# geloescht/mxnet-maintenance

Hardware: AMD Instinct MI355X
Metric: images/sec (whole node) ResNet-50 fp16 batch 256/GPU at 1/2/4/8 MI355X (higher is better)
Workload: dtype fp16; 1 GPU; model=ResNet-50 v1b, global_batch=256, per_gpu_batch=256, image_size=224, parallelism=dp1, layout=NHWC, optimizer=mp-SGD momentum 0.9, lr 0.1 (linear warm-up 40 steps), hip_graph=True, deterministic=True

## Files before the change

### mxnet_maintenance_amd/_state.py

```python
import threading


class _State(threading.local):
    def __init__(self):
        super().__init__()
        self.recording = False
        self.training = False
        self.np_shape = False
        self.np_array = False
        self.tape_leaves = {}


STATE = _State()

DIRECT_GRAD = [0]


def is_recording():
    return STATE.recording


def is_training():
    return STATE.training

GRAPH_RNG = [None]


GRAD_TOUCHED = set()
```

### mxnet_maintenance_amd/autograd.py

```python
from contextlib import contextmanager


import torch

from . import _state
from .base import MXNetError

__all__ = ['record', 'pause', 'train_mode', 'predict_mode', 'is_recording', 'is_training',
           'set_recording', 'set_training', 'mark_variables', 'backward', 'grad', 'Function',
           'get_symbol']


def set_recording(is_recording):
    prev = _state.STATE.recording
    _state.STATE.recording = bool(is_recording)
    return prev


def set_training(train_mode):
    prev = _state.STATE.training
    _state.STATE.training = bool(train_mode)
    return prev


# ... 41 lines not shown
def predict_mode():
    return _RecordingStateScope(None, False)


def mark_variables(variables, gradients, grad_reqs='write'):
    from .ndarray.ndarray import NDArray
    if isinstance(variables, NDArray):
        variables, gradients = [variables], [gradients]
    if isinstance(grad_reqs, str):
        grad_reqs = [grad_reqs] * len(variables)
    for v, g, r in zip(variables, gradients, grad_reqs):
        if r == 'null':
            v._grad_req = None
            continue
        if not v._data.is_floating_point() or getattr(v, '_idt', None) is not None:
            import torch
            idt = getattr(v, '_idt', None) or v._data.dtype
            if not v._data.is_floating_point():
                v._data = v._data.detach().to(torch.float64)
                v._idt = idt
            if not g._data.is_floating_point():
                gidt = g._data.dtype
                g._data = g._data.to(torch.float64)
                g._idt = gidt
        v._set_grad_buffer(g._data, r)
        v._grad = g


_RELEASED_ATTR = '_mxamd_graph_released'


def _collect_leaves(retain):
    leaves = list(_state.STATE.tape_leaves.values())
    if not retain:
        _state.STATE.tape_leaves = {}
    return leaves


def _add_touch_hook(v, t):
    import weakref
    ref = weakref.ref(v)

    def touched(_t, ref=ref):
        a = ref()
        if a is not None:
            _state.GRAD_TOUCHED.add(id(a))
    t.register_post_accumulate_grad_hook(touched)
    t._mxamd_touch_hook = True


def _zero_marked_grads():
    leaves = _collect_leaves(False)
    _prepare_leaves(leaves)
    for v in leaves:
        if v._grad is not None:
            v._fresh_grad = True


def _prepare_leaves(leaves):
    zero = []
    arenas = {}
    for v in leaves:
        t = v._data
        if not t.requires_grad or v._grad is None:
            continue
        if not getattr(t, '_mxamd_touch_hook', False):
            _add_touch_hook(v, t)
        gbuf = v._grad._data
        if t.grad is not gbuf:
            t.grad = gbuf
        if v._grad_req == 'write':
            a = v._arena
            if a is not None and a.all_write:
                arenas.setdefault(id(a), (a, []))[1].append(gbuf)
            else:
                zero.append(gbuf)
    with torch.no_grad():
        for a, bufs in arenas.values():
            if len(bufs) == len(a.params):
                a.g.zero_()
            else:
                zero.extend(bufs)
        if zero:
            torch._foreach_zero_(zero)


def _finish_leaves(leaves):
    touched = _state.GRAD_TOUCHED
    for v in leaves:
        t = v._data
        if v._grad is None:
            continue
        g = t.grad
        if g is not None and g is not v._grad._data:
            v._grad._data = g
            t.grad = g
        if id(v) in touched or not getattr(t, '_mxamd_touch_hook', False):
            v._fresh_grad = True
        else:
            _state.STATE.tape_leaves.setdefault(id(v), v)
    touched.clear()


def _head_grad(g, t):
    if g.shape == t.shape:
        return g
    if g.numel() == t.numel() or (g.numel() > t.numel() and g.dim() == t.dim()
                                  and g.shape[1:] == t.shape[1:]):
        return g.reshape(-1)[:t.numel()].reshape(t.shape)
    try:
        return g.expand(t.shape)
    except RuntimeError:
        pass
    raise MXNetError(f'head gradient of shape {tuple(g.shape)} does not match output shape {tuple(t.shape)}')


def backward(heads, head_grads=None, retain_graph=False, train_mode=True, create_graph=False):
    from .ndarray.ndarray import NDArray
    if isinstance(heads, NDArray):
        heads = [heads]
    if head_grads is not None and isinstance(head_grads, NDArray):
        head_grads = [head_grads]
    tensors, grads = [], []
    for i, h in enumerate(heads):
        t = h._data
        if not t.requires_grad:
            continue
        tensors.append(t)
        hg = None if head_grads is None else head_grads[i]
        grads.append(torch.ones_like(t) if hg is None else _head_grad(hg._data.to(t.dtype), t))
    if not tensors and heads and all(getattr(h, '_recorded', False) for h in heads):
        _zero_marked_grads()
        return
    if not tensors:
        raise MXNetError('Cannot differentiate node because it is not in a computational graph. '
                         'You need to set is_recording to true or use autograd.record() to save '
                         'computational graphs for backward.')
    for h in heads:
        if getattr(getattr(h, '_data', None), _RELEASED_ATTR, False):
            raise MXNetError('Check failed: the graph of this output was already freed by a backward pass '
                             'without retain_graph=True; record it again or pass retain_graph=True')
    if not (retain_graph or create_graph):
        for h in heads:
            if getattr(h, '_data', None) is not None and h._data.grad_fn is not None:
                setattr(h._data, _RELEASED_ATTR, True)
    leaves = _collect_leaves(retain_graph)
    _prepare_leaves(leaves)
    prev_train = set_training(train_mode)
    prev_rec = set_recording(False)
    direct = not create_graph
    if direct:
        _state.DIRECT_GRAD[0] += 1
    try:
        with torch.enable_grad() if create_graph else torch.no_grad():
            torch.autograd.backward(tensors, grads, retain_graph=retain_graph or create_graph,
                                    create_graph=create_graph)
    finally:
        set_training(prev_train)
        set_recording(prev_rec)
        if direct:
            _state.DIRECT_GRAD[0] -= 1
    _finish_leaves(leaves)


def grad(heads, variables, head_grads=None, retain_graph=None, create_graph=False, train_mode=True):
    from .ndarray.ndarray import NDArray
    if isinstance(heads, NDArray):
        heads = [heads]
    if isinstance(variables, NDArray):
        variables = [variables]
    if head_grads is not None and isinstance(head_grads, NDArray):
        head_grads = [head_grads]
    hts = [h._data for h in heads]
    if head_grads is None:
        hgs = [torch.ones_like(h) for h in hts]
    else:
        hgs = [torch.ones_like(h) if g is None else g._data for h, g in zip(hts, head_grads)]
    if retain_graph is None:
        retain_graph = create_graph
    live = [(h, g) for h, g in zip(hts, hgs) if h.requires_grad]
    gs = [None] * len(variables)
    if live:
        prev_train = set_training(train_mode)
        prev_rec = set_recording(create_graph)
        try:
            with torch.enable_grad():
                gs = torch.autograd.grad([h for h, _ in live], [v._data for v in variables],
                                         grad_outputs=[g for _, g in live], retain_graph=retain_graph,
                                         create_graph=create_graph, allow_unused=True)
        finally:
            set_training(prev_train)
            set_recording(prev_rec)

    def dense(g, v):
        if g is None or g._is_zerotensor():
            return torch.zeros_like(v._data)
        return g
    return [NDArray(dense(g, v)) for g, v in zip(gs, variables)]


def get_symbol(x):
    sym = getattr(x, '_symbol', None)
    if isinstance(sym, tuple):
        block, i = sym
        return block._recorded_symbols()[i]
    if sym is not None:
        return sym
    if getattr(x, '_hist', None) is None:
        raise MXNetError('get_symbol: the array was not produced by a recorded operator')
    from .symbol.symbol import _op_func, var
    memo, nvars = {}, [0]

    def build(a):
        key = id(a)
        if key in memo:
            return memo[key]
        h = getattr(a, '_hist', None)
        if h is None:
            s = var('var%d' % nvars[0])
            nvars[0] += 1
        else:
            (opname, attrs, ins), i = h
            kw = {k: v for k, v in attrs.items() if v is not None}
            node = _op_func(opname)(*[build(b) for b in ins if b is not None], **kw)
            s = node[i] if len(node.list_outputs()) > 1 else node
        memo[key] = s
        return s
    return build(x)


class Function:

    def __init__(self):
        self._saved = ()
        self._used = False

    def save_for_backward(self, *args):
        self._saved = args

    @property
    def saved_tensors(self):
        return self._saved

    def __call__(self, *inputs):
        from .ndarray.ndarray import NDArray
        if self._used:
            raise MXNetError('Each Function instance can only be called once.')
        self._used = True
        fself = self
        nin = len(inputs)

        class _Bridge(torch.autograd.Function):
            @staticmethod
            def forward(ctx, *tins):
                with pause():
                    outs = fself.forward(*[NDArray(t.detach()) for t in tins])
                single = isinstance(outs, NDArray)
                ctx.single = single
                outs = [outs] if single else list(outs)
                return tuple(o._data for o in outs)

            @staticmethod
            def backward(ctx, *gouts):
                with pause():
                    gins = fself.backward(*[NDArray(g) for g in gouts])
                if isinstance(gins, NDArray):
                    gins = [gins]
                return tuple(None if g is None else g._data for g in gins)

        from .ndarray.register import _note_leaves
        _note_leaves(inputs)
        tins = [x._data for x in inputs]
        if _state.STATE.recording:
            with torch.enable_grad():
                res = _Bridge.apply(*tins)
        else:
            with torch.no_grad():
                res = _Bridge.apply(*tins)
        outs = [NDArray(r) for r in res]
        return outs[0] if len(outs) == 1 else outs

    def forward(self, *inputs):
        raise NotImplementedError

    def backward(self, *output_grads):
        raise NotImplementedError
```

### mxnet_maintenance_amd/executor.py

```python
import os

import numpy as np
import torch

from . import _state
from . import profiler as _profiler
from .ops import amp_dispatch as _amp
from .base import MXNetError, AsyncOpError
from .ops import registry


def _call_monitor(cb, name, arr):
    from .base import _HANDLES, NDArrayHandle
    key = id(arr)
    _HANDLES[key] = arr
    try:
        cb(name, NDArrayHandle(key))
    finally:
        _HANDLES.pop(key, None)


class GraphProgram:

    def __init__(self, sym):
# ... 372 lines not shown
            return []
        if not out_shapes or any(s is None for s in out_shapes):
            return []
        return [nd.zeros(tuple(s), ctx=self._ctx, dtype=t if t is not None else 'float32')
                for s, t in zip(out_shapes, out_types or [None] * len(out_shapes))]

    @property
    def arg_dict(self):
        return dict(zip(self._symbol.list_arguments(), self.arg_arrays))

    @property
    def grad_dict(self):
        return dict(zip(self._symbol.list_arguments(), self.grad_arrays))

    @property
    def aux_dict(self):
        return dict(zip(self._symbol.list_auxiliary_states(), self.aux_arrays))

    @property
    def output_dict(self):
        return dict(zip(self._symbol.list_outputs(), self.outputs))

    def forward(self, is_train=False, **kwargs):
        from .ndarray.ndarray import NDArray
        for k, v in kwargs.items():
            ad = self.arg_dict
            if k not in ad:
                raise MXNetError('forward: unknown argument %s' % k)
            src = v._data if isinstance(v, NDArray) else torch.as_tensor(np.asarray(v))
            with torch.no_grad():
                ad[k]._data.copy_(src.reshape(ad[k].shape))
        need_grad = is_train and any(r != 'null' for r in self._grad_req.values())
        self._last_is_train = bool(is_train)
        return self._run(is_train, need_grad)

    def _run(self, is_train, need_grad):
        from . import engine as _eng
        _eng.join_workers()
        from .ndarray.ndarray import NDArray
        arg_names = self._symbol.list_arguments()
        feed = {}
        leaves = []
        int_dtypes = None
        for n, a in zip(arg_names, self.arg_arrays):
            t = a._data.detach()
            if need_grad and self._grad_req[n] != 'null':
                if not (t.is_floating_point() or t.is_complex()):
                    int_dtypes = int_dtypes or {}
                    int_dtypes[n] = t.dtype
                    t = t.to(torch.float64)
                t = t.requires_grad_(True)
                leaves.append((n, t))
            feed[n] = t
        for n, a in zip(self._symbol.list_auxiliary_states(), self.aux_arrays):
            feed[n] = a._data
        prev_train = _state.STATE.training
        _state.STATE.training = bool(is_train)
        try:
            mon = None
            if self._monitor_cb is not None:
                cb = self._monitor_cb

                def mon(name, t):
                    _call_monitor(cb, name, NDArray(t.detach()))
            record = [] if (mon is not None and need_grad) else None
            with torch.set_grad_enabled(need_grad):
                outs = self._prog.run(feed, mon, self._monitor_all, record, int_dtypes=int_dtypes)
            self._mon_record = record
            self._mon_grads = {}
            if record:
                for _name, args in record:
                    for t in args:
                        if isinstance(t, torch.Tensor) and t.requires_grad and id(t) not in self._mon_grads:
                            self._mon_grads[id(t)] = None

                            def hook(g, key=id(t)):
                                self._mon_grads[key] = g.detach()
                            t.register_hook(hook)
        finally:
            _state.STATE.training = prev_train
        self._leaves = leaves
        self._out_tensors = outs
        idts = getattr(self._prog, 'out_idts', None) or [None] * len(outs)
        vals = [o.detach().to(d) if d is not None else o.detach() for o, d in zip(outs, idts)]
        if len(self.outputs) == len(vals) and all(
                b.shape == tuple(o.shape) and b._data.dtype == o.dtype for b, o in zip(self.outputs, vals)):
            with torch.no_grad():
                for b, o in zip(self.outputs, vals):
                    b._data.copy_(o)
        else:
            self.outputs = [NDArray(o) for o in vals]
        st = self._output_stypes()
        if st is not None:
            from .ndarray import sparse
            self.outputs = [sparse.cast_storage(o, t) if t != 'default' else o for o, t in zip(self.outputs, st)]
        self._failure = getattr(self._prog, 'failure', None)
        self._failure_box = None
        if self._failure is not None:
            from . import engine
            box = self._failure_box = engine.record_failure(self._failure)
            for o in self.outputs:
                o._exc = box
        return self.outputs

    def _output_stypes(self):
        cached = getattr(self, '_stype_cache', False)
        if cached is not False:
            return cached
        from .ndarray.register import _kept_stype, _check_storage
        args = dict(zip(self._symbol.list_arguments(), self.arg_arrays))
        if all(getattr(a, 'stype', 'default') == 'default' for a in args.values()):
            self._stype_cache = None
            return None

        class _S:
            __slots__ = ('stype',)

            def __init__(self, st):
                self.stype = st
        memo = {}
        for n in self._symbol._topo():
            if n.op is None:
                memo[(id(n), 0)] = getattr(args.get(n.name), 'stype', 'default')
                continue
            ins = [memo.get((id(i), j), 'default') for i, j in n.inputs]
            attrs = registry_parse(n)
            _check_storage(n.op, ins, attrs)
            st = _binary_stype(n.op, ins)
            if st is None:
                st = _kept_stype(n.op, [_S(t) for t in ins], attrs) if ins else None

            memo[(id(n), 0)] = st or 'default'
        self._stype_cache = [memo.get((id(n), i), 'default') for n, i in self._symbol._outputs]
        return self._stype_cache

    def backward(self, out_grads=None, is_train=True):
        from .ndarray.ndarray import NDArray
        if not self._leaves:
            if not any(r != 'null' for r in self._grad_req.values()) or not self.grad_arrays:
                return
            self._run(getattr(self, '_last_is_train', False), True)
        if out_grads is None:
            out_grads = [None] * len(self._out_tensors)
        elif isinstance(out_grads, NDArray):
            out_grads = [out_grads]
        heads, hgs = [], []
        for o, g in zip(self._out_tensors, out_grads):
            if not o.requires_grad:
                continue
            heads.append(o)
            hgs.append(torch.ones_like(o) if g is None else g._data.to(o.dtype).reshape(o.shape))
        names = [n for n, _ in self._leaves]
        ts = [t for _, t in self._leaves]
        grads = (torch.autograd.grad(heads, ts, hgs, allow_unused=True, retain_graph=False)
                 if heads and ts else [None] * len(ts))
        gd = self.grad_dict
        with torch.no_grad():
            for n, g in zip(names, grads):
                buf = gd[n]
                if g is None:
                    if self._grad_req[n] == 'write':
                        buf._data.zero_()
                    continue
                if self._grad_req[n] == 'add':
                    buf._data.add_(g.to(buf._data.dtype))
                else:
                    buf._data.copy_(g)
            got = set(names)
            for n, buf in gd.items():
                if n not in got and buf is not None and self._grad_req.get(n) == 'write':
                    buf._data.zero_()
        record = getattr(self, '_mon_record', None)
        if record and self._monitor_cb is not None:
            for name, args in reversed(record):
                for i, t in enumerate(args):
                    if not isinstance(t, torch.Tensor):
                        continue
                    g = self._mon_grads.get(id(t))
                    _call_monitor(self._monitor_cb, '%s_backward_in%d' % (name, i),
                                  NDArray(g if g is not None else torch.zeros_like(t)))
            self._mon_record = None
        box = getattr(self, '_failure_box', None)
        if box is not None and box[0] is not None:
            for n in names:
                gd[n]._exc = box
        self._leaves = None

    def set_monitor_callback(self, callback, monitor_all=False):
        self._monitor_cb = callback
        self._monitor_all = monitor_all

    def copy_params_from(self, arg_params, aux_params=None, allow_extra_params=False):
        for name, array in arg_params.items():
            if name in self.arg_dict:
                self.arg_dict[name][:] = array.as_in_context(self.arg_dict[name].context)
            elif not allow_extra_params:
                raise ValueError('Find name "%s" that is not in the arguments' % name)
        if aux_params is not None:
            for name, array in aux_params.items():
                if name in self.aux_dict:
                    self.aux_dict[name][:] = array.as_in_context(self.aux_dict[name].context)
                elif not allow_extra_params:
                    raise ValueError('Find name %s that is not in the auxiliary states' % name)

    def reshape(self, partial_shaping=False, allow_up_sizing=False, **kwargs):
        from .ndarray.ndarray import NDArray
        from . import ndarray as nd
        sym = self._symbol
        known = {n: a.shape for n, a in zip(sym.list_arguments(), self.arg_arrays)}
        for k in kwargs:
            if k not in known:
                raise MXNetError('reshape: %s is not an argument of the symbol' % k)
        if not partial_shaping:
            known = {k: v for k, v in known.items() if k not in kwargs}
            known.update(kwargs)
        else:
            known.update(kwargs)
        arg_shapes, out_shapes, aux_shapes = sym.infer_shape(**known)

        def fit(old, shape, what):
            if old is None:
                return None
            shape = tuple(shape)
            if shape == tuple(old.shape):
                return old
            n = 1
            for d in shape:
                n *= d
            if n <= old.size:
                return NDArray(old._data.reshape(-1)[:n].view(shape))
            if not allow_up_sizing:
                raise MXNetError('reshape: %s grows from %s to %s; pass allow_up_sizing=True'
                                 % (what, old.shape, shape))
            return nd.zeros(shape, ctx=old.context, dtype=old.dtype)

        names = sym.list_arguments()
        args = [fit(a, s, n) for a, s, n in zip(self.arg_arrays, arg_shapes, names)]
        grads = [fit(g, s, n + '_grad') for g, s, n in zip(self.grad_arrays, arg_shapes, names)]
        auxs = [fit(a, s, n) for a, s, n in zip(self.aux_arrays, aux_shapes, sym.list_auxiliary_states())]
        exe = Executor(sym, self._ctx, args, grads if any(g is not None for g in grads) else None,
                       dict(self._grad_req), auxs)
        if len(self.outputs) == len(out_shapes):
            try:
                exe.outputs = [fit(o, s, 'output') for o, s in zip(self.outputs, out_shapes)]
            except MXNetError:
                pass
        exe._monitor_cb, exe._monitor_all = self._monitor_cb, self._monitor_all
        return exe

    def get_optimized_symbol(self):
        return self._opt_symbol

    def debug_str(self):
        from .symbol import passes as _passes
        names = self._symbol.list_arguments()
        wanting = [n for n in names if self._grad_req.get(n, 'null') != 'null']
        grad = bool(_passes.grad_reachable(self._opt_symbol, set(wanting)))
        shapes = {n: a.shape for n, a in zip(names, self.arg_arrays)}
        dtypes = {n: a.dtype for n, a in zip(names, self.arg_arrays)}
        nbytes = _passes.memory_plan(self._opt_symbol, shapes, dtypes, grad)
        return '%s\nTotal %d MB allocated\n' % (self._opt_symbol.debug_str(), nbytes // (1 << 20))
```

### mxnet_maintenance_amd/gluon/graph_step.py

```python
import gc
import os

import torch

from .. import _state
from ..ndarray.ndarray import NDArray

__all__ = ['GraphStep']


def _tensor_of(x):
    return x._data if isinstance(x, NDArray) else x


class GraphStep:

    def __init__(self, fn, trainer=None, warmup=3, fallback=False):
        if warmup < 1:
            raise ValueError('GraphStep needs at least one eager warm-up call')
        self._fn = fn
        self._trainer = trainer
        self._warmup = int(warmup)
        self._calls = 0
        self._graph = None
        self._static_in = None
        self._static_out = None
        self._stream = None
        self._rng = None
        self._fallback = fallback
        self._eager_only = False

    @property
    def captured(self):
        return self._graph is not None

    def _side_stream(self, device):
        if self._stream is None:
            self._stream = torch.cuda.Stream(device=device)
        return self._stream

    @staticmethod
    def _device(inputs):
        dev = next((_tensor_of(x).device for x in inputs if torch.is_tensor(_tensor_of(x))), None)
        if dev is None and torch.cuda.is_available():
            dev = torch.device('cuda', torch.cuda.current_device())
        return dev

    def _run_eager(self, inputs):
        dev = self._device(inputs)
        if dev is None or dev.type != 'cuda':
            return self._fn(*inputs)
        s = self._side_stream(dev)
        s.wait_stream(torch.cuda.current_stream(dev))
        with torch.cuda.stream(s):
            out = self._fn(*inputs)
        torch.cuda.current_stream(dev).wait_stream(s)
        return out

    def _capture(self, inputs):
        tin = [_tensor_of(x) for x in inputs]
        dev = self._device(inputs)
        if dev is None or dev.type != 'cuda':
            raise RuntimeError('GraphStep captures HIP work: inputs must live on a GPU context')
        self._static_in = [NDArray(t.clone()) if isinstance(x, NDArray) else (t.clone() if torch.is_tensor(t) else x)
                           for x, t in zip(inputs, tin)]
        self._rng = torch.zeros(1, dtype=torch.int64, device=dev)
        if self._trainer is not None:
            self._trainer._enter_graph_mode()
        s = self._side_stream(dev)
        if os.environ.get('MXAMD_GRAPH_GC', '1') == '1':
            gc.collect()
        torch.cuda.synchronize(dev)
        graph = torch.cuda.CUDAGraph()
        _state.GRAPH_RNG[0] = self._rng
        try:
            with torch.cuda.graph(graph, stream=s):
                self._static_out = self._fn(*self._static_in)
        except Exception:
            if self._trainer is not None:
                self._trainer._exit_graph_mode()
            raise
        finally:
            _state.GRAPH_RNG[0] = None
        self._graph = graph

    def _load_inputs(self, inputs):
        if len(inputs) != len(self._static_in):
            raise ValueError('GraphStep: expected %d inputs, got %d' % (len(self._static_in), len(inputs)))
        for dst, src in zip(self._static_in, inputs):
            d, t = _tensor_of(dst), _tensor_of(src)
            if not torch.is_tensor(d):
                if d != t:
                    raise ValueError('GraphStep: non-tensor argument %r differs from the captured %r' % (t, d))
                continue
            if d.shape != t.shape or d.dtype != t.dtype:
                raise ValueError('GraphStep: input %s/%s differs from the captured %s/%s'
                                 % (tuple(t.shape), t.dtype, tuple(d.shape), d.dtype))
            if d.data_ptr() != t.data_ptr():
                d.copy_(t, non_blocking=True)

    @property
    def static_inputs(self):
        return self._static_in

    def __call__(self, *inputs):
        self._calls += 1
        if self._eager_only:
            return self._run_eager(inputs)
        if self._graph is None:
            if self._calls <= self._warmup:
                return self._run_eager(inputs)
            err = None
            try:
                self._capture(inputs)
            except Exception as e:
                err = e
            if not self._all_ranks_ok(err is None):
                if self._graph is not None:
                    self._drop_graph()
                if not self._fallback:
                    raise err if err is not None else RuntimeError('GraphStep: capture failed on another rank')
                import warnings
                warnings.warn('GraphStep: capture failed (%s); running the step eagerly on every rank'
                              % (err if err is not None else 'on another rank'))
                self._eager_only = True
                if torch.cuda.is_available():
                    torch.cuda.synchronize()
                return self._run_eager(inputs)
        else:
            self._load_inputs(inputs)
        if self._trainer is not None:
            self._trainer._stage_hyper()
        self._rng.add_(1)
        self._graph.replay()
        return self._static_out

    @staticmethod
    def _all_ranks_ok(ok):
        from ..parallel import dist
        if dist.world_size() <= 1:
            return ok
        t = torch.tensor([1 if ok else 0], dtype=torch.int32)
        dist.all_reduce(t, op='min')
        return bool(t.item())

    def _drop_graph(self):
        if self._trainer is not None:
            self._trainer._exit_graph_mode()
        self._graph = None
        self._static_out = None

    def reset(self):
        if self._trainer is not None and self._graph is not None:
            self._trainer._exit_graph_mode()
        self._graph = None
        self._static_out = None
        self._static_in = None
        self._calls = self._warmup
```

### mxnet_maintenance_amd/ops/kernel_fns.py

```python
import os

import torch

from . import kernels as _K
from .. import _state
from ..utils import env as _env

__all__ = ['BatchNormNHWC', 'BatchNormDualTailNHWC', 'SoftmaxCE', 'GlobalAvgPoolNHWC', 'flat_sgd']

_DT = {torch.float32: 0, torch.float16: 1, torch.bfloat16: 2}


def _stream():
    return torch.cuda.current_stream().cuda_stream


def _p(t):
    return 0 if t is None else t.data_ptr()


def _f32(t):
    if t.dtype == torch.float32 and t.is_contiguous():
        return t
    m = getattr(t, '_mxamd_master', None)
# ... 115 lines not shown
            ctx.pool = (N, H, W, C, Ho, Wo, kh, kw, sh, sw, ph, pw, 1)
            lib.pool_nhwc_forward_bnrelu(_DT[x.dtype], x.data_ptr(), y.data_ptr(), arg.data_ptr(), *ctx.pool,
                                         _stream(), scale.data_ptr(), shift.data_ptr())
            mask = arg
        relu_mode = 0 if not relu else (1 if not _RELU_FROM_X[0] else (3 if addend is not None else 2))
        if pool is not None:
            relu_mode = 2
        ctx.save_for_backward(x, y if relu_mode == 1 else mask, g, mean, invstd,
                              scale if relu_mode == 2 else None, shift if relu_mode == 2 else None)
        ctx.cfg = (relu_mode, bool(training), addend is not None, gamma.dtype, beta.dtype)
        ctx.tee_key = getattr(addend, '_mxamd_tee_key', None) if (addend is not None and relu_mode == 3) else None
        ctx.bn_token = None
        if training and relu_mode in (0, 2, 3) and _BN_BWD_FUSE[0] and pool is None:
            ctx.bn_token = _BnToken()
            y._mxamd_bn_src = (x, mean, scale if relu_mode == 2 else None, shift if relu_mode == 2 else None,
                               mask if relu_mode == 3 else None, relu_mode, ctx.bn_token)
        ctx.refs = (gamma, beta)
        ctx.add_src = None
        if relu_mode == 3 and training and _BN_BWD_FUSE[0] and _BN_TAIL_DS[0]:
            src = getattr(addend, '_mxamd_bn_src', None)
            if (src is not None and src[5] == 0 and tuple(src[0].shape) == tuple(x.shape)
                    and src[0].dtype == x.dtype and src[0].is_contiguous()):
                ctx.add_src = src
        third = invstd if (invstd_out and training) else var
        ctx.mark_non_differentiable(mean, third)
        ctx.set_materialize_grads(False)
        return y, mean, third

    @staticmethod
    def backward(ctx, gy, _gm, _gv):
        lib = _K.lib()
        x, y, g, mean, invstd, fscale, fshift = ctx.saved_tensors
        relu_mode, training, has_add, gdt, bdt = ctx.cfg
        gamma_ref, beta_ref = ctx.refs
        if gy is None:
            return (None,) * 12
        gy = gy.contiguous()
        C = x.shape[-1]
        R = x.numel() // C
        dev = x.device
        fused_pool = False
        if ctx.pool is not None:
            fused_pool = (x.dtype in (torch.float16, torch.bfloat16) and 256 % (C // 8) == 0
                          and hasattr(lib, 'bn_pool_backward') and _BN_POOL_BWD[0])
            if not fused_pool:
                gyd = torch.empty_like(x)
                lib.pool_nhwc_backward(_DT[x.dtype], 1, gy.data_ptr(), y.data_ptr(), gyd.data_ptr(), *ctx.pool,
                                       _stream())
                gy, y = gyd, None
        lazy_mask = None
        tok = ctx.bn_token
        if tok is not None and tok.lazy is not None:
            dy_l, mask_l, ver_l = tok.lazy
            tok.lazy = None
            if gy is dy_l and gy._version == ver_l and relu_mode == 0 and not has_add and ctx.pool is None:
                lazy_mask = mask_l
            else:
                gy = (gy - dy_l + _materialize_dz(dy_l, mask_l)).contiguous()
        dx = torch.empty_like(x)
        dz = torch.empty_like(x) if has_add else None
        ext = getattr(gy, '_mxamd_bn_bwd', None)
        ext_nblk = 0
        if (ext is not None and ctx.bn_token is not None and ext[2] is ctx.bn_token
                and ext[3] == gy._version):
            part, ext_nblk = ext[0], ext[1]
        else:
            nblk = lib.bn_partials_rows(R, C)
            part = torch.empty(2 * nblk * C, dtype=torch.float32, device=dev)
        out = torch.empty(5, C, dtype=torch.float32, device=dev)
        need_g, need_b = ctx.needs_input_grad[1], ctx.needs_input_grad[2]
        tg = _leaf_grad(gamma_ref, C) if need_g else None
        tb = _leaf_grad(beta_ref, C) if need_b else None
        direct = tb is not None and (tg is not None or not need_g) and (tg is not None or tb is not None)
        if direct:
            dg_buf = tg if tg is not None else torch.zeros(C, dtype=torch.float32, device=dev)
            dg_ptr, db_ptr, accum = dg_buf.data_ptr(), tb.data_ptr(), 1
        else:
            dg_ptr, db_ptr, accum = out[0].data_ptr(), out[1].data_ptr(), 0
        if fused_pool:
            N_, H_, W_, C_, Ho_, Wo_, kh, kw, sh, sw, ph, pw, _ = ctx.pool
            ppart = torch.empty(2 * lib.bn_pool_bwd_blocks() * C, dtype=torch.float32, device=dev)
            lib.bn_pool_backward(_DT[x.dtype], x.data_ptr(), gy.data_ptr(), y.data_ptr(), dx.data_ptr(), g.data_ptr(),
                                 mean.data_ptr(), invstd.data_ptr(), fscale.data_ptr(), fshift.data_ptr(),
                                 ppart.data_ptr(), dg_ptr, db_ptr, out[2].data_ptr(), N_, H_, W_, C_, Ho_, Wo_, kh, kw,
                                 sh, sw, ph, pw, 0, int(training), accum, _stream())
            if direct:
                return dx, None, None, None, None, None, None, None, None, None, None, None
            return (dx, out[0].to(gdt) if need_g else None, out[1].to(bdt) if need_b else None,
                    None, None, None, None, None, None, None, None, None)
        ymask = y if relu_mode == 3 else None
        y = y if relu_mode == 1 else None
        ds = ctx.add_src if dz is not None else None
        lazy = (dz is not None and ds is None and ymask is not None and ctx.tee_key is not None
                and lazy_shortcut_ok(ctx.tee_key))
        lazy_ds = (dz is not None and ds is not None and ymask is not None and _LAZY_DZ[0]
                   and isinstance(ds[6], _BnToken))
        if lazy or lazy_ds:
            dz = None
        kmode = relu_mode
        if lazy_mask is not None:
            kmode, ymask = 3, lazy_mask
        dkw = {}
        if ds is not None:
            ds_nblk = lib.bn_tail_ds_rows(R, C)
            ds_part = torch.empty(2 * ds_nblk * C, dtype=torch.float32, device=dev)
            dkw = dict(ds_z=ds[0].data_ptr(), ds_mean=ds[1].data_ptr(), ds_part=ds_part.data_ptr())
        lib.bn_nhwc_backward(_DT[x.dtype], x.data_ptr(), gy.data_ptr(), _p(y), _p(ymask), dx.data_ptr(), _p(dz),
                             g.data_ptr(),
                             mean.data_ptr(), invstd.data_ptr(), _p(fscale), _p(fshift), part.data_ptr(), dg_ptr,
                             db_ptr, out[2].data_ptr(), R, C, kmode, 0, int(training), accum, _stream(),
                             ext_nblk, **dkw)
        if ds is not None:
            if lazy_ds:
                gy._mxamd_bn_bwd = (ds_part, ds_nblk, ds[6], gy._version)
                ds[6].lazy = (gy, ymask, gy._version)
                dz = gy
            else:
                dz._mxamd_bn_bwd = (ds_part, ds_nblk, ds[6], dz._version)
        if lazy:
            gy._mxamd_lazy_mask = (ymask, gy._version)
            dz = gy
        if direct:
            dgamma = None
            dbeta = None
        else:
            dgamma = out[0].to(gdt) if need_g else None
            dbeta = out[1].to(bdt) if need_b else None
        return dx, dgamma, dbeta, dz, None, None, None, None, None, None, None, None


_DUAL_TAIL_USED = [0]


def _bn_param_grad_dst(gamma_ref, beta_ref, need_g, need_b, out, C, dev):
    tg = _leaf_grad(gamma_ref, C) if need_g else None
    tb = _leaf_grad(beta_ref, C) if need_b else None
    if tb is not None and (tg is not None or not need_g):
        dg_buf = tg if tg is not None else torch.zeros(C, dtype=torch.float32, device=dev)
        return dg_buf.data_ptr(), tb.data_ptr(), 1, True, dg_buf
    return out[0].data_ptr(), out[1].data_ptr(), 0, False, None


class BatchNormDualTailNHWC(torch.autograd.Function):

    @staticmethod
    def forward(ctx, x, z, gamma, beta, zgamma, zbeta, eps, training, moving_mean, moving_var, zmoving_mean,
                zmoving_var, momentum=None):
        lib = _K.lib()
        assert z.shape == x.shape and z.dtype == x.dtype and z.is_contiguous()
        dev = x.device
        dt = _DT[x.dtype]
        zg, zmean, zinvstd, _zvar, zscale, zshift, zargs, zhost = _bn_fwd_stats(
            lib, z, zgamma, zbeta, zmoving_mean, zmoving_var, eps, training, momentum)
        if training:
            lib.bn_nhwc_forward(dt, z.data_ptr(), 0, 0, 0, *zargs(False))
        g, mean, invstd, var, scale, shift, args, host = _bn_fwd_stats(
            lib, x, gamma, beta, moving_mean, moving_var, eps, training, momentum)
        y = torch.empty_like(x)
        mask = torch.empty(x.numel() // 8, dtype=torch.uint8, device=dev)
        lib.bn_nhwc_forward(dt, x.data_ptr(), z.data_ptr(), y.data_ptr(), mask.data_ptr(), *args(True),
                            zscale.data_ptr(), zshift.data_ptr())
        for h in (zhost, host):
            if h is not None:
                h()
        _DUAL_TAIL_USED[0] += 1
        ctx.save_for_backward(x, z, mask, g, mean, invstd, zg, zmean, zinvstd)
        ctx.cfg = (bool(training), gamma.dtype, beta.dtype, zgamma.dtype, zbeta.dtype)
        ctx.refs = (gamma, beta, zgamma, zbeta)
        ctx.bn_token = None
        if training and _BN_BWD_FUSE[0]:
            ctx.bn_token = _BnToken()
            y._mxamd_bn_src = (x, mean, None, None, mask, 3, ctx.bn_token)
        ctx.mark_non_differentiable(mean, var)
        ctx.set_materialize_grads(False)
        return y, mean, var

    @staticmethod
    def backward(ctx, gy, _gm, _gv):
        lib = _K.lib()
        x, z, mask, g, mean, invstd, zg, zmean, zinvstd = ctx.saved_tensors
        training, gdt, bdt, zgdt, zbdt = ctx.cfg
        gamma_ref, beta_ref, zgamma_ref, zbeta_ref = ctx.refs
        if gy is None:
            return (None,) * 13
        gy = gy.contiguous()
        C = x.shape[-1]
        R = x.numel() // C
        dev = x.device
        dt = _DT[x.dtype]
        need = ctx.needs_input_grad
        dx = torch.empty_like(x)
        dzs = torch.empty_like(z)
        ext = getattr(gy, '_mxamd_bn_bwd', None)
        ext_nblk = 0
        if ext is not None and ctx.bn_token is not None and ext[2] is ctx.bn_token and ext[3] == gy._version:
            part, ext_nblk = ext[0], ext[1]
        else:
            part = torch.empty(2 * lib.bn_partials_rows(R, C) * C, dtype=torch.float32, device=dev)
        out = torch.empty(5, C, dtype=torch.float32, device=dev)
        zout = torch.empty(5, C, dtype=torch.float32, device=dev)
        dg_ptr, db_ptr, accum, direct, _k1 = _bn_param_grad_dst(gamma_ref, beta_ref, need[2], need[3], out, C, dev)
        zdg_ptr, zdb_ptr, zaccum, zdirect, _k2 = _bn_param_grad_dst(zgamma_ref, zbeta_ref, need[4], need[5], zout, C,
                                                                    dev)
        ride = training and _BN_TAIL_DS[0]
        dkw, zpart, znblk = {}, None, 0
        if ride:
            znblk = lib.bn_tail_ds_rows(R, C)
            zpart = torch.empty(2 * znblk * C, dtype=torch.float32, device=dev)
            dkw = dict(ds_z=z.data_ptr(), ds_mean=zmean.data_ptr(), ds_part=zpart.data_ptr())
        else:
            zpart = torch.empty(2 * lib.bn_partials_rows(R, C) * C, dtype=torch.float32, device=dev)
        lib.bn_nhwc_backward(dt, x.data_ptr(), gy.data_ptr(), 0, mask.data_ptr(), dx.data_ptr(), 0, g.data_ptr(),
                             mean.data_ptr(), invstd.data_ptr(), 0, 0, part.data_ptr(), dg_ptr, db_ptr,
                             out[2].data_ptr(), R, C, 3, 0, int(training), accum, _stream(), ext_nblk, **dkw)
        lib.bn_nhwc_backward(dt, z.data_ptr(), gy.data_ptr(), 0, mask.data_ptr(), dzs.data_ptr(), 0, zg.data_ptr(),
                             zmean.data_ptr(), zinvstd.data_ptr(), 0, 0, zpart.data_ptr(), zdg_ptr, zdb_ptr,
                             zout[2].data_ptr(), R, C, 3, 0, int(training), zaccum, _stream(), znblk)
        dgamma = None if direct or not need[2] else out[0].to(gdt)
        dbeta = None if direct or not need[3] else out[1].to(bdt)
        zdgamma = None if zdirect or not need[4] else zout[0].to(zgdt)
        zdbeta = None if zdirect or not need[5] else zout[1].to(zbdt)
        return dx, dzs, dgamma, dbeta, zdgamma, zdbeta, None, None, None, None, None, None, None


def bnrelu_pool_ok(x, kernel, stride, pad):
    return (bn_ok(x) and tuple(kernel) == (3, 3) and pool_ok(x, kernel, stride, pad)
            and x.numel() + 256 * 32 * 256 * 8 < 2 ** 31 and hasattr(_K.lib(), 'pool_nhwc_forward_bnrelu'))


class SoftmaxCE(torch.autograd.Function):

    @staticmethod
    def forward(ctx, logits, label):
        lib = _K.lib()
        N, K = logits.shape
        lab = label.reshape(-1)
        is_int = not lab.is_floating_point()
        lab = lab.to(torch.int64).contiguous() if is_int else lab.float().contiguous()
        loss = torch.empty(N, dtype=torch.float32, device=logits.device)
        lse = torch.empty(N, dtype=torch.float32, device=logits.device)
        lib.softmax_ce_forward(_DT[logits.dtype], int(is_int), logits.data_ptr(), lab.data_ptr(), loss.data_ptr(),
                               lse.data_ptr(), N, K, _stream())
        ctx.save_for_backward(logits, lab, lse)
        ctx.is_int = is_int
        return loss

    @staticmethod
    def backward(ctx, gout):
        lib = _K.lib()
        logits, lab, lse = ctx.saved_tensors
        N, K = logits.shape
        g = gout.float().contiguous()
        dl = torch.empty_like(logits)
        lib.softmax_ce_backward(_DT[logits.dtype], int(ctx.is_int), logits.data_ptr(), lab.data_ptr(),
                                lse.data_ptr(), g.data_ptr(), dl.data_ptr(), N, K, _stream())
        return dl, None


class GlobalAvgPoolNHWC(torch.autograd.Function):
    @staticmethod
    def forward(ctx, x):
        lib = _K.lib()
        x = x.contiguous()
        N, C = x.shape[0], x.shape[-1]
        HW = x.numel() // (N * C)
        y = torch.empty((N,) + (1,) * (x.dim() - 2) + (C,), dtype=x.dtype, device=x.device)
        lib.gap_nhwc_forward(_DT[x.dtype], x.data_ptr(), y.data_ptr(), N, HW, C, _stream())
        ctx.shape = x.shape
        return y

    @staticmethod
    def backward(ctx, gy):
        lib = _K.lib()
        shape = ctx.shape
        N, C = shape[0], shape[-1]
        HW = int(torch.tensor(shape[1:-1]).prod())
        gy = gy.contiguous()
        dx = torch.empty(shape, dtype=gy.dtype, device=gy.device)
        lib.gap_nhwc_backward(_DT[gy.dtype], gy.data_ptr(), dx.data_ptr(), N, HW, C, _stream())
        return dx


def gap_ok(x):
    return x.dtype in _DT and x.is_contiguous() and x.shape[-1] % 8 == 0


class ReluHip(torch.autograd.Function):

    @staticmethod
    def forward(ctx, x):
        x = x.contiguous()
        y = torch.empty_like(x)
        _K.lib().relu_forward(_DT[x.dtype], x.data_ptr(), y.data_ptr(), x.numel(), _stream())
        ctx.save_for_backward(y)
        return y

    @staticmethod
    def backward(ctx, gy):
        y, = ctx.saved_tensors
        gy = gy.contiguous()
        dx = torch.empty_like(y)
        _K.lib().relu_backward(_DT[y.dtype], y.data_ptr(), gy.data_ptr(), dx.data_ptr(), y.numel(), _stream())
        return dx


def relu_ok(x):
    return x.dtype in _DT and x.is_cuda and x.numel() > 0 and x.data_ptr() % 16 == 0 and x.is_contiguous()


_PW_OPS = {'add': 0, 'sub': 1, 'mul': 2, 'div': 3, 'maximum': 4, 'minimum': 5}


def _bcast_strides(t, shape):
    lead = len(shape) - t.dim()
# ... 226 lines not shown
        if bn_bwd is not None:
            z, bmean, bscale, bshift, bmask, bmode, token = bn_bwd
            assert z.shape == y.shape and z.dtype == y.dtype and z.is_contiguous()
            bnp = lib.conv_nhwc_fwd_big_bwd_nparts(N, H, W, R, S, stride[0], stride[1], pad[0], pad[1], v)
            bpart = torch.empty(2 * K * bnp, dtype=torch.float32, device=x.device)
            bkw = dict(bn_z=z.data_ptr(), bn_mean=bmean.data_ptr(), bn_scale=_p(bscale), bn_shift=_p(bshift),
                       bn_mask=_p(bmask), bn_mode=int(bmode), bn_part=bpart.data_ptr(), bn_nparts=bnp)
        lib.conv_nhwc_fwd_big(_DT[x.dtype], x.data_ptr(), w.data_ptr(), _p(b), y.data_ptr(),
                              _zero_page(x.device).data_ptr(), N, H, W, C, K, R, S, stride[0], stride[1],
                              pad[0], pad[1], v, _p(part), nparts, _p(addend), _stream(), up=int(up), dh=dil[0],
                              dw=dil[1], **bkw)
        if bkw:
            y._mxamd_bn_bwd = (bpart, bnp, bn_bwd[6], y._version)
        if part is not None:
            y._mxamd_bn_part = (part, nparts)
        return y
    if variant in (5, 6):
        lib = _K.lib()
        bco = 128 if variant == 5 else 64
        bkw = _glds_bnb(bn_bwd, y, lib.conv_glds_bwd_nparts(N * Ho * Wo, bco))
        part = bkw.pop('_part', None)
        lib.conv_nhwc_fwd_glds(_DT[x.dtype], x.data_ptr(), w.data_ptr(), _p(b), y.data_ptr(),
                               _zero_page(x.device).data_ptr(), N, H, W, C, K, R, S, stride[0], stride[1],
                               pad[0], pad[1], bco, _stream(), **bkw)
        if part is not None:
            y._mxamd_bn_bwd = (part, bkw['bn_nparts'], bn_bwd[6], y._version)
        return y
    _K.lib().conv_nhwc_fwd(_DT[x.dtype], x.data_ptr(), w.data_ptr(), _p(b), y.data_ptr(), N, H, W, C, K, R, S,
                           stride[0], stride[1], pad[0], pad[1], int(variant), _stream())
    return y


def halo_ok(x, w, stride, pad):
    K, R, S, C = w.shape
    return (_CONV_HIP and x.is_cuda and x.dtype in (torch.float16, torch.bfloat16) and x.dim() == 4
            and x.is_contiguous() and w.is_contiguous() and x.data_ptr() % 16 == 0 and w.data_ptr() % 16 == 0
            and hasattr(_K.lib(), 'conv3x3_halo')
            and bool(_K.lib().conv3x3_halo_ok(C, K, R, S, stride[0], stride[1], pad[0], pad[1], x.shape[2])))


def conv_halo(x, w, bn_stats=False, bn_bwd=None):
    N, H, W, C = x.shape
    K = w.shape[0]
    lib = _K.lib()
    y = torch.empty((N, H, W, K), dtype=x.dtype, device=x.device)
    nparts = lib.conv3x3_halo_nparts(N, H)
    part = torch.empty(2 * K * nparts, dtype=torch.float32, device=x.device) if (bn_stats or bn_bwd) else None
    kw = {}
    if bn_bwd is not None:
        z, bmean, bscale, bshift, _bmask, bmode, _token = bn_bwd
        assert int(bmode) in (0, 2) and z.shape == y.shape and z.dtype == y.dtype and z.is_contiguous()
        kw = dict(bn_z=z.data_ptr(), bn_mean=bmean.data_ptr(), bn_scale=_p(bscale), bn_shift=_p(bshift),
                  bn_mode=int(bmode), bn_part=part.data_ptr())
    lib.conv3x3_halo(_DT[x.dtype], x.data_ptr(), w.data_ptr(), y.data_ptr(), _zero_page(x.device).data_ptr(), N, H,
                     W, C, K, _p(part) if bn_bwd is None else 0, nparts if bn_bwd is None else 0, s=_stream(), **kw)
    if bn_bwd is not None:
        y._mxamd_bn_bwd = (part, nparts, bn_bwd[6], y._version)
    elif part is not None:
        y._mxamd_bn_part = (part, nparts)
    return y


def glds_bnb_ok(bn_src):
    return bn_src is not None and int(bn_src[5]) in (0, 2) and hasattr(_K.lib(), 'conv_glds_bwd_nparts')


def _glds_bnb(bn_bwd, y, nparts):
    if bn_bwd is None:
        return {}
    z, bmean, bscale, bshift, _bmask, bmode, _token = bn_bwd
    assert int(bmode) in (0, 2) and z.shape == y.shape and z.dtype == y.dtype and z.is_contiguous()
    part = torch.empty(2 * y.shape[-1] * nparts, dtype=torch.float32, device=y.device)
    return dict(bn_z=z.data_ptr(), bn_mean=bmean.data_ptr(), bn_scale=_p(bscale), bn_shift=_p(bshift),
                bn_part=part.data_ptr(), bn_nparts=nparts, _part=part)


_ZERO = {}


def _zero_page(dev):
    z = _ZERO.get(dev)
    if z is None:
        z = _ZERO[dev] = torch.zeros(128, dtype=torch.float16, device=dev)
    return z


def _fwd_variants(C, K, bias=False, ktot=None):
    v = []
    if C % 64 == 0 and not bias:
        v.extend(b for b, (bco, _bpix) in sorted(_RING_VARIANTS.items()) if K % bco == 0)
    if C % 64 == 0:
        v.extend(b for b, (bco, _bpix) in sorted(_BIG_VARIANTS.items())
                 if K % bco == 0 and (b not in _BIG_SKINNY or (_SKINNY_ON and ktot == 64)))
    if C % 64 == 0 and K % 128 == 0:
        v.append(5)
    if C % 64 == 0:
        v.append(6)
    if K % 128 == 0 and C % 64 == 0:
        v.append(1)
    if K % 128 == 0:
        v.append(2)
    if C % 64 == 0:
        v.append(3)
    v.append(4)
    return v


def conv_wgrad_ok(x, w):
    return (_CONV_HIP and x.dim() == 4 and w.dim() == 4 and x.dtype in (torch.float16, torch.bfloat16)
            and x.is_contiguous() and x.shape[3] % 64 == 0 and w.shape[0] % 64 == 0 and w.shape[3] == x.shape[3]
            and x.numel() < 2 ** 31 and x.data_ptr() % 16 == 0)


def conv_wgrad(x, dy, wshape, stride, pad, out=None, accum=False, dma=True, ring=0, dil=(1, 1)):
    N, H, W, C = x.shape
    K, R, S, _ = wshape
    dy = dy.contiguous()
    assert dy.dtype == x.dtype and dy.shape[0] == N and dy.shape[3] == K
    dh, dw = dil
    Ho = (H + 2 * pad[0] - dh * (R - 1) - 1) // stride[0] + 1
    Wo = (W + 2 * pad[1] - dw * (S - 1) - 1) // stride[1] + 1
    assert tuple(dy.shape[1:3]) == (Ho, Wo), 'conv_wgrad: dy shape does not match the conv geometry'
    assert dy.numel() < 2 ** 31 and dy.data_ptr() % 16 == 0
    lib = _K.lib()
    if ring:
        ws = lib.conv_nhwc_wgrad_ring_workspace(N, H, W, C, K, R, S, stride[0], stride[1], pad[0], pad[1], ring,
                                                dh=dh, dw=dw)
    else:
        ws = lib.conv_nhwc_wgrad_workspace(N, H, W, C, K, R, S, stride[0], stride[1], pad[0], pad[1], dh=dh, dw=dw)
    slab = torch.empty(ws, dtype=torch.float32, device=x.device)
    if out is None:
        out = torch.empty((K, R, S, C), dtype=x.dtype, device=x.device)
        accum = False
    assert out.is_contiguous() and out.numel() == K * R * S * C and out.dtype in _DT
    if ring:
        lib.conv_nhwc_wgrad_ring(_DT[x.dtype], x.data_ptr(), dy.data_ptr(), slab.data_ptr(), _DT[out.dtype],
                                 out.data_ptr(), int(bool(accum)), N, H, W, C, K, R, S, stride[0], stride[1], pad[0],
                                 pad[1], _zero_page(x.device).data_ptr(), int(ring), _stream(), dh=dh, dw=dw)
        return out
    lib.conv_nhwc_wgrad(_DT[x.dtype], x.data_ptr(), dy.data_ptr(), slab.data_ptr(), _DT[out.dtype], out.data_ptr(),
                        int(bool(accum)), N, H, W, C, K, R, S, stride[0], stride[1], pad[0], pad[1],
                        _zero_page(x.device).data_ptr() if dma else 0, _stream(), dh=dh, dw=dw)
    return out


def _taps_t(w, out, src, base, rstride):
    K, R, S, C = w.shape
    for i in range(0, len(src), 32):
        _K.lib().weight_taps_t(w.element_size(), w.data_ptr(), out.data_ptr(), K, R * S, C, src[i:i + 32],
                               base[i:i + 32], rstride[i:i + 32], _stream())
    return out


def _dgrad_weight(w):
    K, R, S, C = w.shape
    if not (w.is_cuda and w.is_contiguous() and w.element_size() in (2, 4) and _K.available()):
        return w.flip(1, 2).permute(3, 1, 2, 0).contiguous()
    T = R * S
    out = torch.empty((C, R, S, K), dtype=w.dtype, device=w.device)
    return _taps_t(w, out, [T - 1 - t for t in range(T)], [t * K for t in range(T)], [T * K] * T)


def transpose2d(w):
    R, C = w.shape
    if w.is_cuda and w.is_contiguous() and w.element_size() in (2, 4) and R % 8 == 0 and C % 8 == 0:
        return _dgrad_weight(w.view(R, 1, 1, C)).view(C, R)
    return w.t().contiguous()


def _phase_taps(R, P, s, ph):
    return sorted(((ph + P - r) // s, r) for r in range(R) if (ph + P - r) % s == 0)


def conv_dgrad_strided_ok(dy, w, stride, pad, xshape, bco=128):
    K, R, S, C = w.shape
    s = tuple(stride)
    return (_CONV_HIP and s != (1, 1) and s[0] == s[1] and s[0] <= 2 and dy.dtype in (torch.float16, torch.bfloat16)
            and dy.dim() == 4 and K % 64 == 0 and C % bco == 0 and xshape[1] % s[0] == 0 and xshape[2] % s[1] == 0
            and dy.is_cuda and all(0 <= p < k for p, k in zip(pad, (R, S))))


_PHASE_PLANS = {}


def _phase_plan(wshape, stride, pad, device):
    key = (tuple(wshape), tuple(stride), tuple(pad), device)
    plan = _PHASE_PLANS.get(key)
    if plan is not None:
        return plan
    K, R, S, C = wshape
    st = stride[0]
    phases, empty, idx, off = [], [], [], 0
    for ph in range(st):
        th = _phase_taps(R, pad[0], st, ph)
        for pw in range(st):
            tw = _phase_taps(S, pad[1], st, pw)
            if not th or not tw:
                empty.append((ph, pw))
                continue
            dh = [d for d, _ in th]
            dw = [d for d, _ in tw]
            if dh != list(range(dh[0], dh[0] + len(dh))) or dw != list(range(dw[0], dw[0] + len(dw))):
                raise ValueError('conv_dgrad_strided: non-contiguous phase taps')
            nt = len(th) * len(tw)
            for i, (_, r) in enumerate(th):
                for j, (_, c) in enumerate(tw):
                    idx.append((r * S + c, off + (i * len(tw) + j) * K, nt * K))
            phases.append((ph, pw, len(th), len(tw), -dh[0], -dw[0], off))
            off += C * nt * K
    plan = (phases, empty, (idx, off))
    _PHASE_PLANS[key] = plan
    return plan


def conv_dgrad_strided(dy, w, stride, pad, xshape, bco=128, bn_bwd=None):
    K, R, S, C = w.shape
    N, H, W, _ = xshape
    st = stride[0]
    Ho, Wo = H // st, W // st
    dy = dy.contiguous()
    phases, empty, gidx = _phase_plan(w.shape, stride, pad, w.device)
    if len(phases) > 4:
        raise ValueError('conv_dgrad_strided: at most 4 phases per launch')
    dx = torch.empty((N, H, W, C), dtype=dy.dtype, device=dy.device)
    if len(empty) > 3:
        raise ValueError('conv_dgrad_strided: at most 3 phases without taps')
    slots, total = gidx
    wsub = _taps_t(w.contiguous(), torch.empty(total, dtype=w.dtype, device=w.device), [t[0] for t in slots],
                   [t[1] for t in slots], [t[2] for t in slots])
    cols = list(zip(*phases))
    lib = _K.lib()
    bkw = _glds_bnb(bn_bwd, dx, len(phases) * lib.conv_glds_bwd_nparts(N * Ho * Wo, bco)) if bn_bwd else {}
    part = bkw.pop('_part', None)
    lib.conv_nhwc_dgrad_phases_glds(_DT[dy.dtype], dy.data_ptr(), wsub.data_ptr(), dx.data_ptr(),
                                    _zero_page(dy.device).data_ptr(), N, dy.shape[1], dy.shape[2], K, C, Ho, Wo,
                                    st, list(cols[0]), list(cols[1]), list(cols[2]), list(cols[3]),
                                    list(cols[4]), list(cols[5]), list(cols[6]), [e[0] for e in empty],
                                    [e[1] for e in empty], bco, _stream(), **bkw)
    if part is not None:
        dx._mxamd_bn_bwd = (part, bkw['bn_nparts'], bn_bwd[6], dx._version)
    return dx


def _conv_bwd_torch(dy, x, w, stride, pad, mask):
    xc = x.permute(0, 3, 1, 2)
    wc = w.permute(0, 3, 1, 2)
    dyc = dy.permute(0, 3, 1, 2)
    dx, dw, _ = torch.ops.aten.convolution_backward(dyc, xc, wc, None, list(stride), list(pad), [1, 1], False,
                                                    [0, 0], 1, [mask[0], mask[1], False])
    if dx is not None:
        dx = dx.permute(0, 2, 3, 1)
    if dw is not None:
        dw = dw.permute(0, 2, 3, 1)
    return dx, dw



_AUTOTUNE = _env.get('MXNET_CUDNN_AUTOTUNE_DEFAULT') > 0
_ALGO = {}
_TIMES = {}


_REJECTED = {}


def _rel_err(a, b):
    a = a.float()
    b = b.float()
    return float((a - b).abs().max() / (b.abs().max() + 1e-6))


_VENDOR = ('mm', 'miopen')
_VENDOR_PREFIX = ('splitk', 'blaslt', 'sk')
_VENDOR_MARGIN = float(os.environ.get('MXAMD_VENDOR_MARGIN', '0.03'))


def _is_vendor(name):
    return name in _VENDOR or name.startswith(_VENDOR_PREFIX)
_TUNE_ROUNDS = int(os.environ.get('MXAMD_TUNE_ROUNDS', '2'))


def _time_candidates(cands, reps=3, key=None, tol=2e-2):
    ref = None
    ref_name = next((n for n, _ in cands if n in ('mm', 'miopen')), None)
    if ref_name is not None:
        ref = dict(cands)[ref_name]()
        if isinstance(ref, torch.Tensor):
            ref = ref.detach().clone()
        else:
            ref = None
    ok = []
    for name, fn in cands:
        if ref is not None and name != ref_name:
            r = fn()
            if isinstance(r, torch.Tensor) and r.shape == ref.shape:
                err = _rel_err(r, ref)
                if not err <= tol:
                    _REJECTED.setdefault(key, {})[name] = err
                    continue
        ok.append((name, fn))
    times, outs = {}, {}
    for _ in range(_TUNE_ROUNDS):
        for name, fn in ok:
            fn()
            t, r = _measure(fn, reps)
            if name not in times or t < times[name]:
                times[name] = t
                outs[name] = r
    names = [n for n, _ in cands]
    agreed = _agree_times([times.get(n, float('inf')) for n in names])
    best, best_t = None, None
    for name, t in zip(names, agreed):
        if t == float('inf'):
            continue
        if key is not None:
            _TIMES.setdefault(key, {})[name] = t / reps
        if _is_vendor(name):
            t *= 1.0 + _VENDOR_MARGIN
        if best_t is None or t < best_t:
            best, best_t = name, t
    if best is not None and best not in outs:
        best = None
    return best, (outs[best] if best is not None else None)


def _measure(fn, reps):
    if torch.cuda.is_available():
        s, e = torch.cuda.Event(enable_timing=True), torch.cuda.Event(enable_timing=True)
        s.record()
        for _ in range(reps):
            r = fn()
        e.record()
        e.synchronize()
        return s.elapsed_time(e), r
    import time
    t0 = time.perf_counter()
    for _ in range(reps):
        r = fn()
    return (time.perf_counter() - t0) * 1e3, r


def _agree_times(vals):
    from ..parallel import dist
    if dist.world_size() <= 1 or not vals:
        return vals
    t = torch.tensor(vals, dtype=torch.float64)
    dist.all_reduce(t, op='max')
    return [float(v) for v in t.tolist()]


_DETERMINISTIC = [_env.get('MXNET_ENFORCE_DETERMINISM') != 0]
_NONDET = ('mm', 'miopen', 'sk', 'splitk', 'bmm', 'blaslt')


def _apply_torch_determinism(flag):
    torch.backends.cudnn.deterministic = bool(flag)
    if flag:
        torch.backends.cudnn.benchmark = False
    try:
        torch.use_deterministic_algorithms(bool(flag), warn_only=True)
    except Exception:
        pass


def set_deterministic(flag):
    _DETERMINISTIC[0] = bool(flag)
    _apply_torch_determinism(flag)


def deterministic():
    return _DETERMINISTIC[0]


if _DETERMINISTIC[0]:
    _apply_torch_determinism(True)


def _det_filter(cands):
    if not _DETERMINISTIC[0] or cands is None:
        return cands
    keep = [(n, f) for n, f in cands if not n.startswith(_NONDET)]
    return keep or cands


def _akey(key):
    return key + ('det',) if _DETERMINISTIC[0] else key


_FILE_ALGO = {}
_FILE_STATE = {'loaded': False}


def _tuning_file():
    return os.environ.get('MXAMD_AUTOTUNE_FILE', '')


def _load_tuning_file():
    if _FILE_STATE['loaded']:
        return
    _FILE_STATE['loaded'] = True
    path = _tuning_file()
    if path and os.path.exists(path):
        import json
        try:
            with open(path) as f:
                _FILE_ALGO.update(json.load(f))
        except (OSError, ValueError):
            pass


def _save_tuning_file(key, name):
    path = _tuning_file()
    if not path or name is None:
        return
    from ..parallel import dist
    if dist.rank() != 0:
        return
    import json
    _FILE_ALGO[repr(key)] = name
    tmp = path + '.tmp'
    try:
        with open(tmp, 'w') as f:
            json.dump(_FILE_ALGO, f, indent=0, sort_keys=True)
        os.replace(tmp, path)
    except OSError:
        pass


def _select(key, cands, default, timing=None):
    key = _akey(key)
    cands = _det_filter(cands)
    timing = _det_filter(timing)
    _load_tuning_file()
    name = _ALGO.get(key)
    if name is None:
# ... 681 lines not shown
```

### src/kernels/bindings.cc

```cpp
#include <hip/hip_runtime.h>
#include <pybind11/pybind11.h>
#include <pybind11/stl.h>

#include <cstdint>
#include <stdexcept>
#include <vector>

namespace py = pybind11;

namespace mxamd {
void bn_nhwc_forward(int dtype, const void* x, const void* addend, void* y, uint8_t* mask, const float* gamma,
                     const float* beta,
                     const float* center, float* part, float* mean, float* invstd, float* var, float* scale,
                     float* shift, int64_t R, int C, float eps, int training, int relu, int fix_gamma,
                     float momentum, float* mm_upd, float* mv_upd, int ext_nblk, hipStream_t s, const float* ascale,
                     const float* ashift);
void bn_nhwc_backward(int dtype, const void* x, const void* dy, const void* y, const uint8_t* mask, void* dx,
                      void* dz,
                      const float* gamma, const float* mean, const float* invstd, const float* fscale,
                      const float* fshift, float* part, float* dgamma, float* dbeta, float* coef, int64_t R, int C,
                      int relu_mode, int fix_gamma, int training, int accum, hipStream_t s, int ext_nblk, const void* ds_z, const float* ds_mean, float* ds_part);
int bn_partials_rows(int64_t R, int C);
int bn_tail_ds_rows(int64_t R, int C);
void gemm_nt(int dtype, const void* a, const void* b, const void* bias, const void* addend, void* c, int out_f32,
             int M, int N, int K, int lda, int ldb, int ldc, int act, int cfg, int splits, float* ws, hipStream_t s,
             int bias_lowp);
int gemm_nt_tile_n(int cfg);
int gemm_nt_tile_m(int cfg);
void int8_gemm(const int8_t* A, const int8_t* B, int32_t* C, int M, int N, int K, hipStream_t s);
void csr_dot_dense(int dtype, const int64_t* indptr, const int64_t* indices, const void* vals, const void* rhs,
                   void* out, int64_t M, int64_t K, int N, hipStream_t s);
void csrT_dot_dense(int dtype, const int64_t* indptr, const int64_t* indices, const void* vals, const void* rhs,
                    const int64_t* slot, float* out32, int64_t M, int64_t K, int N, hipStream_t s);
void embedding_forward(int dtype, int itype, const void* idx, const void* w, void* y, int64_t n, int V, int C,
                       hipStream_t s);
void embedding_backward(int dtype, int itype, const void* idx, const void* dy, float* acc, uint8_t* touched,
                        int out_dtype, void* grad, int accum, int64_t n, int V, int C, hipStream_t s);
int bn_nhwc_stats(int dtype, const void* x, const float* center, float* part, int64_t R, int C, hipStream_t s,
                  int total_blocks);
int64_t colsum_partials(int64_t R, int C);
void colsum_rows(int dtype, const void* x, const float* zeros, float* part, int64_t R, int C, int out_dtype,
                 void* out, int accum, hipStream_t s);
void softmax_ce_forward(int dtype, int label_is_int, const void* logits, const void* label, float* loss, float* lse,
                        int N, int K, hipStream_t s);
void softmax_ce_backward(int dtype, int label_is_int, const void* logits, const void* label, const float* lse,
                         const float* gout, void* dlogits, int N, int K, hipStream_t s);
void gap_nhwc_forward(int dtype, const void* x, void* y, int N, int HW, int C, hipStream_t s);
void relu_forward(int dtype, const void* x, void* y, int64_t n, hipStream_t s);
void relu_backward(int dtype, const void* y, const void* dy, void* dx, int64_t n, hipStream_t s);
void pointwise_binary(int dtype, int op, const void* a, const void* b, void* out, int64_t n, int mode, int64_t row,
                      int ndim, const int64_t* shape, const int64_t* astride, const int64_t* bstride, hipStream_t s);
void gap_nhwc_backward(int dtype, const void* dy, void* dx, int N, int HW, int C, hipStream_t s);
void flat_sgd(int dtype, void* w, const void* g, float* mom, float* w32, int64_t n, float lr, float wd,
              float momentum, float rescale, float clip, const float* hp, hipStream_t s);
void conv_nhwc_fwd(int dtype, const void* x, const void* w, const float* bias, void* y, int N, int H, int W, int C,
                   int K, int R, int S, int sh, int sw, int ph, int pw, int variant, hipStream_t s);
int conv_nhwc_fwd_big_nparts(int N, int H, int W, int R, int S, int sh, int sw, int ph, int pw, int variant);
void conv_nhwc_fwd_big(int dtype, const void* x, const void* w, const float* bias, void* y, const void* zero, int N,
                       int H, int W, int C, int K, int R, int S, int sh, int sw, int ph, int pw, int variant,
                       float* part, int nparts, const void* addend, hipStream_t s, const void* bn_z,
                       const float* bn_mean, const float* bn_scale, const float* bn_shift, const uint8_t* bn_mask,
                       int bn_mode, float* bn_part, int bn_nparts, int up, int dh, int dw);
int conv_nhwc_fwd_big_bwd_nparts(int N, int H, int W, int R, int S, int sh, int sw, int ph, int pw, int variant);
void conv_nhwc_fwd_glds(int dtype, const void* x, const void* w, const float* bias, void* y, const void* zero, int N,
                        int H, int W, int C, int K, int R, int S, int sh, int sw, int ph, int pw, int bco,
                        hipStream_t s, const void* bn_z, const float* bn_mean, const float* bn_scale,
                        const float* bn_shift, float* bn_part, int bn_nparts);
int conv_glds_bwd_nparts(int M, int bco);
void conv_nhwc_dgrad_phases_glds(int dtype, const void* dy, const void* w, void* dx, const void* zero, int N, int Hi,
                                 int Wi, int Cin, int Cout, int Ho, int Wo, int stride, int nph, const int* ph,
                                 const int* pw, const int* R, const int* S, const int* pad_h, const int* pad_w,
                                 const int64_t* w_off, int nzero, const int* zph, const int* zpw, int bco,
                                 hipStream_t s, const void* bn_z, const float* bn_mean, const float* bn_scale,
                                 const float* bn_shift, float* bn_part, int bn_nparts);
int conv_nhwc_fwd_ring_nparts(int N, int H, int W, int R, int S, int sh, int sw, int ph, int pw, int variant);
void conv_nhwc_fwd_ring(int dtype, const void* x, const void* w, void* y, const void* zero, int N, int H, int W, int C,
                        int K, int R, int S, int sh, int sw, int ph, int pw, int variant, float* part, int nparts,
                        hipStream_t s);
bool conv3x3_halo_ok(int C, int K, int R, int S, int sh, int sw, int ph, int pw, int W);
int conv3x3_halo_nparts(int N, int H);
void conv3x3_halo(int dtype, const void* x, const void* w, void* y, const void* zero, int N, int H, int W, int C, int K,
                  float* part, int nparts, const void* bn_z, const float* bn_mean, const float* bn_scale,
                  const float* bn_shift, int bn_mode, float* bn_part, hipStream_t s);
int conv_nhwc_wgrad_ring_ok(int C, int K, int R, int S, int variant);
int64_t conv_nhwc_wgrad_ring_workspace(int N, int H, int W, int C, int K, int R, int S, int sh, int sw, int ph, int pw,
                                       int variant, int dh, int dw);
void conv_nhwc_wgrad_ring(int dtype, const void* x, const void* dy, float* slab, int out_dtype, void* out, int accum,
                          int N, int H, int W, int C, int K, int R, int S, int sh, int sw, int ph, int pw,
                          const void* zero, int variant, hipStream_t s, int dh, int dw);
int64_t conv_nhwc_wgrad_workspace(int N, int H, int W, int C, int K, int R, int S, int sh, int sw, int ph, int pw,
                                  int dh, int dw);
void conv_nhwc_wgrad(int dtype, const void* x, const void* dy, float* slab, int out_dtype, void* out, int accum, int N,
                     int H, int W, int C, int K, int R, int S, int sh, int sw, int ph, int pw, const void* zero,
                     hipStream_t s, int dh, int dw);
int conv_stem_grid(int N, int H, int W, int R, int S, int ph, int pw);
void conv_stem_fwd(int dtype, const void* x, const void* w, void* y, int N, int H, int W, int C, int K, int R, int S,
                   int sh, int sw, int ph, int pw, float* part, int nparts, hipStream_t s);
int64_t conv_stem_wgrad_workspace(int N, int H, int W, int R, int S, int ph, int pw);
void conv_stem_wgrad(int dtype, const void* x, const void* dy, float* slab, int out_dtype, void* out, int accum, int N,
                     int H, int W, int C, int K, int R, int S, int sh, int sw, int ph, int pw, hipStream_t s);
int layernorm_bwd_partials(int M);
void layernorm_forward(int dtype, const void* x, const void* gamma, const void* beta, int pt, void* y, float* mean,
                       float* rstd, int M, int D, float eps, hipStream_t s);
void layernorm_backward(int dtype, const void* x, const void* dy, const void* gamma, int pt, const float* mean,
                        const float* rstd, void* dx, float* part, void* dgamma, void* dbeta, int gdtype, int accum,
                        int M, int D, hipStream_t s);
void add_dropout_ln_forward(int dtype, const void* x, const void* h, const void* gamma, const void* beta, int pt,
                            void* y, void* s_out, uint8_t* mask, float* mean, float* rstd, int M, int D, float eps,
                            float p, uint64_t seed, const uint64_t* seed_base, hipStream_t s);
void add_dropout_ln_backward(int dtype, const void* s_in, const void* dy, const void* gamma, int pt, const float* mean,
                             const float* rstd, const uint8_t* mask, float p, void* ds, void* dh, float* part,
                             float* hpart, void* dgamma, void* dbeta, int gdtype, int accum, int M, int D,
                             hipStream_t s);
void column_sum_partials(int gdtype, const float* part, int nb, int ncol, void* out, int accum, hipStream_t s);
void gelu_forward(int dtype, const void* x, void* y, int64_t n, hipStream_t s);
void gelu_backward(int dtype, const void* x, const void* dy, void* dx, int64_t n, hipStream_t s);
void gelu_backward_colpart(int dtype, const void* x, const void* dy, void* dx, float* part, int M, int N,
                           hipStream_t s);
int gelu_colpart_blocks(int M, int N);
void softmax_forward(int dtype, int log, const void* x, void* y, int M, int L, float scale, hipStream_t s);
void softmax_backward(int dtype, int log, const void* y, const void* dy, void* dx, int M, int L, float scale,
                      hipStream_t s);
void dropout_forward(int dtype, const void* x, void* y, uint8_t* mask, int64_t n, float p, uint64_t seed,
                     const uint64_t* seed_base, hipStream_t s);
void dropout_backward(int dtype, const void* dy, const uint8_t* mask, void* dx, int64_t n, float p, hipStream_t s);
int attention_max_seq();
void attention_forward(int dtype, const void* qkv, const float* kmask, void* out, float* lse, int S, int B, int H,
                       int D, float scale, float p, uint64_t seed, const uint64_t* seed_base, hipStream_t s);
void attention_backward(int dtype, const void* qkv, const float* kmask, const void* out, const void* dout,
                        const float* lse, float* delta, void* dqkv, int S, int B, int H, int D, float scale, float p,
                        uint64_t seed, const uint64_t* seed_base, hipStream_t s);
void flat_adam(int dtype, int mode, void* w, const void* g, float* mean, float* var, float* w32, int64_t n, float lr,
               float beta1, float beta2, float eps, float wd, float eta, float rescale, float clip, const float* hp,
               hipStream_t s);
void lamb_update(int dtype, void* w, const void* g, float* mean, float* var, float* w32, float* upd,
                 const void* chunks, int nchunks, float* nrm, int nseg, float lr, float beta1, float beta2, float eps,
                 float bc1, float bc2, float wd, float rescale, float clip, float lb, float ub, const float* hp,
                 hipStream_t s);
void seg_sumsq(int dtype, const void* x, const void* chunks, int nchunks, float* out, int nseg, hipStream_t s);
void all_finite(int dtype, const void* x, int64_t n, float scale, int* flag, int init, hipStream_t s);
void pool_nhwc_forward(int dtype, int is_max, const void* x, void* y, uint8_t* arg, int N, int H, int W, int C,
                       int Ho, int Wo, int kh, int kw, int sh, int sw, int ph, int pw, int cip, hipStream_t s,
                       const float* scale, const float* shift);
int bn_pool_bwd_blocks();
void bn_pool_backward(int dtype, const void* x, const void* dy, const uint8_t* arg, void* dx, const float* gamma,
                      const float* mean, const float* invstd, const float* fscale, const float* fshift, float* part,
                      float* dgamma, float* dbeta, float* coef, int N, int H, int W, int C, int Ho, int Wo, int kh,
                      int kw, int sh, int sw, int ph, int pw, int fix_gamma, int training, int accum,
                      hipStream_t s);
void pool_nhwc_backward(int dtype, int is_max, const void* dy, const uint8_t* arg, void* dx, int N, int H, int W,
                        int C, int Ho, int Wo, int kh, int kw, int sh, int sw, int ph, int pw, int cip,
                        hipStream_t s);
void deform_im2col(int dtype, const void* x, const void* off, const void* msk, void* cols, int N, int C, int H, int W,
                   int Ho, int Wo, int kh, int kw, int sh, int sw, int ph, int pw, int dh, int dw, int dg,
                   int rows, hipStream_t s);
void deform_col2im(int dtype, const void* off, const void* msk, const void* gcols, float* gx, int N, int C, int H,
                   int W, int Ho, int Wo, int kh, int kw, int sh, int sw, int ph, int pw, int dh, int dw, int dg,
                   int rows, hipStream_t s);
void deform_col2im_coord(int dtype, const void* x, const void* off, const void* msk, const void* gcols, void* goff,
                         void* gmsk, int N, int C, int H, int W, int Ho, int Wo, int kh, int kw, int sh, int sw,
                         int ph, int pw, int dh, int dw, int dg, int rows, hipStream_t s);
void deform_im2col_nhwc(int dtype, const void* x, const void* off, const void* msk, void* cols, const int* g,
                        int ld_off, int ld_msk, hipStream_t s);
void deform_bwd_nhwc(int dtype, const void* x, const void* off, const void* msk, const void* gcols, float* gx,
                     void* goff, void* gmsk, const int* g, int ld_off, int ld_msk, hipStream_t s);
void conv_dw_fwd(int dtype, const void* x, const void* wt, const float* bias, void* y, const int* gm, hipStream_t s);
void conv_dw_dgrad(int dtype, const void* dy, const void* wt, void* dx, const int* gm, hipStream_t s);
void conv_dw_wgrad(int dtype, const void* x, const void* dy, float* slab, int nslice, int out_dtype, void* out,
                   int accum, const int* gm, hipStream_t s);
int ssd_loss_blocks(int rows);
void ssd_loss_fwd(int dtype, const void* cls, const void* loc, const float* cls_t, const float* loc_t,
                  const float* loc_m, int rows, int C1, float lambd, float* part, float* out, hipStream_t s);
void ssd_loss_bwd(int dtype, const void* cls, const void* loc, const float* cls_t, const float* loc_t,
                  const float* loc_m, const float* stats, const float* gout, int rows, int C1, float lambd, void* dcls,
                  void* dloc, hipStream_t s);
void multibox_target(int dtype, const float* anchors, const float* labels, const void* cls_pred, float* loc_target,
                     float* loc_mask, float* cls_target, float* match_iou, int* match_gt, uint32_t* key, int B, int A,
                     int L, int W, int C, float thr, float ignore_label, float neg_ratio, float neg_thresh,
                     int min_neg, float v0, float v1, float v2, float v3, hipStream_t s);
void slab_reduce(int out_dtype, float* slab, int splits, int64_t n, void* out, int accum, hipStream_t s);
void twobit_quantize(int dtype, const void* g, float* res, void* packed, int64_t n, float thr, hipStream_t s);
void twobit_dequantize_sum(const void* packed, int64_t row_bytes, int nrows, int64_t n, float thr, float* out,
                           hipStream_t s);
int conv_pw_stream_ok(int kin, int nout);
int conv_pw_stream_grid(int M, int kin, int nout, int ncu, int add);
int conv_pw_stream_slices(int kin, int nout);
void weight_taps_t(int elem_bytes, const void* w, void* out, int K, int RS, int C, int n, const int* src,
                   const int64_t* base, const int64_t* rstride, hipStream_t s);
void conv_pw_stream(int dtype, const void* x, const void* w, void* y, const void* zero, int M, int kin, int nout,
                    float* part, int grid, hipStream_t s, const void* addend, int wt, const void* bn_z,
                    const uint8_t* bn_mask, const float* bn_mean, const float* bn_scale, const float* bn_shift,
                    int bn_mode, const uint8_t* addend_mask);
int conv_pw_stream_bnb_ok(int kin, int nout, int add, int mode);
void conv_gen(int dtype, int mode, const void* src, const void* wsrc, const float* bias, void* dst, const int* geom,
              int splits, hipStream_t s);
void rnn_fwd_seq(int dtype, int mode, const float* gx, const void* h0, const float* c0, const void* whh,
                 const float* bhh, void* out, int ldo, float* cseq, float* save, int Tn, int N, int H, int reverse,
                 hipStream_t s);
void rnn_bwd_seq(int dtype, int mode, const void* whhT, const void* dy, int ldy, const float* dhT,
                 const float* save, const float* cseq, const float* c0, const void* h0, const void* out, int ldo,
                 void* dgh, void* dgx, float* dc, float* dhd, float* dh0, int Tn, int N, int H, int reverse,
                 hipStream_t s);
}

using namespace mxamd;

template <typename T>
static inline T* P(uintptr_t p) {
  return reinterpret_cast<T*>(p);
}
static inline hipStream_t S(uintptr_t s) { return reinterpret_cast<hipStream_t>(s); }
static inline hipStream_t S_(uintptr_t s) { return reinterpret_cast<hipStream_t>(s); }

static void check_launch(const char* name) {
  hipError_t e = hipGetLastError();
  if (e != hipSuccess) throw std::runtime_error(std::string(name) + ": " + hipGetErrorString(e));
}

PYBIND11_MODULE(_hip_kernels, m) {
  m.doc() = "gfx950 HIP kernels for mxnet_maintenance_amd";
  m.attr("arch") = "gfx950";

  m.def("bn_partials_rows", &bn_partials_rows);
  m.def("bn_tail_ds_rows", &bn_tail_ds_rows);
  m.def("bn_nhwc_stats", [](int dt, uintptr_t x, uintptr_t center, uintptr_t part, int64_t R, int C, uintptr_t s) {
    int nblk = bn_nhwc_stats(dt, P<const void>(x), P<const float>(center), P<float>(part), R, C, S(s), 512);
    check_launch("bn_nhwc_stats");
    return nblk;
  });
  m.def("embedding_forward", [](int dt, int it, uintptr_t idx, uintptr_t w, uintptr_t y, int64_t n, int V, int C,
                                uintptr_t s) {
    embedding_forward(dt, it, P<const void>(idx), P<const void>(w), P<void>(y), n, V, C, S(s));
    check_launch("embedding_forward");
  });
  m.def("embedding_backward", [](int dt, int it, uintptr_t idx, uintptr_t dy, uintptr_t acc, uintptr_t touched,
                                 int odt, uintptr_t grad, int accum, int64_t n, int V, int C, uintptr_t s) {
    embedding_backward(dt, it, P<const void>(idx), P<const void>(dy), P<float>(acc), P<uint8_t>(touched), odt,
                       P<void>(grad), accum, n, V, C, S(s));
    check_launch("embedding_backward");
  });
  m.def("csr_dot_dense", [](int dt, uintptr_t indptr, uintptr_t indices, uintptr_t vals, uintptr_t rhs, uintptr_t out,
                            int64_t M, int64_t K, int N, uintptr_t s) {
    csr_dot_dense(dt, P<const int64_t>(indptr), P<const int64_t>(indices), P<const void>(vals), P<const void>(rhs),
                  P<void>(out), M, K, N, S(s));
    check_launch("csr_dot_dense");
  });
  m.def("csrT_dot_dense", [](int dt, uintptr_t indptr, uintptr_t indices, uintptr_t vals, uintptr_t rhs,
                             uintptr_t slot, uintptr_t out32, int64_t M, int64_t K, int N, uintptr_t s) {
    csrT_dot_dense(dt, P<const int64_t>(indptr), P<const int64_t>(indices), P<const void>(vals), P<const void>(rhs),
                   P<const int64_t>(slot), P<float>(out32), M, K, N, S(s));
    check_launch("csrT_dot_dense");
  });
  m.def("int8_gemm", [](uintptr_t a, uintptr_t b, uintptr_t c, int M, int N, int K, uintptr_t s) {
    int8_gemm(P<const int8_t>(a), P<const int8_t>(b), P<int32_t>(c), M, N, K, S(s));
    check_launch("int8_gemm");
  });
  m.def("colsum_partials", [](int64_t R, int C) { return colsum_partials(R, C); });
  m.def("colsum_rows", [](int dt, uintptr_t x, uintptr_t zeros, uintptr_t part, int64_t R, int C, int odt,
                          uintptr_t out, int accum, uintptr_t s) {
    colsum_rows(dt, P<const void>(x), P<const float>(zeros), P<float>(part), R, C, odt, P<void>(out), accum, S(s));
    check_launch("colsum_rows");
  });
  m.def("twobit_quantize", [](int dt, uintptr_t g, uintptr_t res, uintptr_t packed, int64_t n, float thr,
                              uintptr_t s) {
    twobit_quantize(dt, P<void>(g), P<float>(res), P<void>(packed), n, thr, S(s));
    check_launch("twobit_quantize");
  });
  m.def("twobit_dequantize_sum", [](uintptr_t packed, int64_t row_bytes, int nrows, int64_t n, float thr,
                                    uintptr_t out, uintptr_t s) {
    twobit_dequantize_sum(P<void>(packed), row_bytes, nrows, n, thr, P<float>(out), S(s));
    check_launch("twobit_dequantize_sum");
  });
  m.def("gemm_nt", [](int dt, uintptr_t a, uintptr_t b, uintptr_t bias, uintptr_t addend, uintptr_t c, int out_f32,
                      int M, int N, int K, int lda, int ldb, int ldc, int act, int cfg, int splits, uintptr_t ws,
                      uintptr_t s, int bias_lowp) {
    gemm_nt(dt, P<void>(a), P<void>(b), P<void>(bias), P<void>(addend), P<void>(c), out_f32, M, N, K, lda, ldb, ldc,
            act, cfg, splits, P<float>(ws), S(s), bias_lowp);
    check_launch("gemm_nt");
  }, py::arg("dt"), py::arg("a"), py::arg("b"), py::arg("bias"), py::arg("addend"), py::arg("c"), py::arg("out_f32"),
     py::arg("M"), py::arg("N"), py::arg("K"), py::arg("lda"), py::arg("ldb"), py::arg("ldc"), py::arg("act"),
     py::arg("cfg"), py::arg("splits"), py::arg("ws"), py::arg("s"), py::arg("bias_lowp") = 0);
  m.def("weight_taps_t", [](int eb, uintptr_t w, uintptr_t out, int K, int RS, int C, std::vector<int> src,
                            std::vector<int64_t> base, std::vector<int64_t> rstride, uintptr_t s) {
    if (src.size() != base.size() || src.size() != rstride.size()) throw std::runtime_error("weight_taps_t: table sizes");
    weight_taps_t(eb, P<const void>(w), P<void>(out), K, RS, C, static_cast<int>(src.size()), src.data(), base.data(),
                  rstride.data(), S(s));
    check_launch("weight_taps_t");
  });
  m.def("conv_pw_stream_ok", &conv_pw_stream_ok);
  m.def("conv_pw_stream_slices", &conv_pw_stream_slices);
  m.def("conv_pw_stream_grid", [](int M, int kin, int nout, int ncu, int add) {
    return conv_pw_stream_grid(M, kin, nout, ncu, add);
  }, pybind11::arg("M"), pybind11::arg("kin"), pybind11::arg("nout"), pybind11::arg("ncu"), pybind11::arg("add") = 0);
  m.def("conv_pw_stream", [](int dt, uintptr_t x, uintptr_t w, uintptr_t y, uintptr_t zero, int M, int kin, int nout,
                             uintptr_t part, int grid, uintptr_t s, uintptr_t addend, int wt, uintptr_t bn_z,
                             uintptr_t bn_mask, uintptr_t bn_mean, uintptr_t bn_scale, uintptr_t bn_shift, int bn_mode,
                             uintptr_t addend_mask) {
    conv_pw_stream(dt, P<const void>(x), P<const void>(w), P<void>(y), P<const void>(zero), M, kin, nout,
                   P<float>(part), grid, S(s), P<const void>(addend), wt, P<const void>(bn_z), P<const uint8_t>(bn_mask),
                   P<const float>(bn_mean), P<const float>(bn_scale), P<const float>(bn_shift), bn_mode,
                   P<const uint8_t>(addend_mask));
    check_launch("conv_pw_stream");
  }, pybind11::arg("dt"), pybind11::arg("x"), pybind11::arg("w"), pybind11::arg("y"), pybind11::arg("zero"),
     pybind11::arg("M"), pybind11::arg("kin"), pybind11::arg("nout"), pybind11::arg("part"), pybind11::arg("grid"),
     pybind11::arg("s"), pybind11::arg("addend"), pybind11::arg("wt") = 0, pybind11::arg("bn_z") = 0,
     pybind11::arg("bn_mask") = 0, pybind11::arg("bn_mean") = 0, pybind11::arg("bn_scale") = 0,
     pybind11::arg("bn_shift") = 0, pybind11::arg("bn_mode") = 0, pybind11::arg("addend_mask") = 0);
  m.def("conv_pw_stream_bnb_ok", &conv_pw_stream_bnb_ok);
  m.def("conv_gen", [](int dt, int mode, uintptr_t src, uintptr_t wsrc, uintptr_t bias, uintptr_t dst,
                       std::vector<int> geom, int splits, uintptr_t s) {
    if (geom.size() != 22) throw std::runtime_error("conv_gen: geometry needs 22 ints");
    conv_gen(dt, mode, P<const void>(src), P<const void>(wsrc), P<const float>(bias), P<void>(dst), geom.data(),
             splits, S(s));
    check_launch("conv_gen");
  });
  m.def("rnn_fwd_seq", [](int dt, int mode, uintptr_t gx, uintptr_t h0, uintptr_t c0, uintptr_t whh, uintptr_t bhh,
                          uintptr_t out, int ldo, uintptr_t cseq, uintptr_t save, int T, int N, int H, int reverse,
                          uintptr_t s) {
    rnn_fwd_seq(dt, mode, P<const float>(gx), P<const void>(h0), P<const float>(c0), P<const void>(whh),
                P<const float>(bhh), P<void>(out), ldo, P<float>(cseq), P<float>(save), T, N, H, reverse, S(s));
    check_launch("rnn_fwd_seq");
  });
  m.def("rnn_bwd_seq", [](int dt, int mode, uintptr_t whhT, uintptr_t dy, int ldy, uintptr_t dhT, uintptr_t save,
                          uintptr_t cseq, uintptr_t c0, uintptr_t h0, uintptr_t out, int ldo, uintptr_t dgh,
                          uintptr_t dgx, uintptr_t dc, uintptr_t dhd, uintptr_t dh0, int T, int N, int H, int reverse,
                          uintptr_t s) {
    rnn_bwd_seq(dt, mode, P<const void>(whhT), P<const void>(dy), ldy, P<const float>(dhT), P<const float>(save),
                P<const float>(cseq), P<const float>(c0), P<const void>(h0), P<const void>(out), ldo, P<void>(dgh),
                P<void>(dgx), P<float>(dc), P<float>(dhd), P<float>(dh0), T, N, H, reverse, S(s));
    check_launch("rnn_bwd_seq");
  });
  m.def("gemm_nt_tile_n", &gemm_nt_tile_n);
  m.def("gemm_nt_tile_m", &gemm_nt_tile_m);
  m.def("slab_reduce", [](int odt, uintptr_t slab, int splits, int64_t n, uintptr_t out, int accum, uintptr_t s) {
    slab_reduce(odt, P<float>(slab), splits, n, P<void>(out), accum, S(s));
    check_launch("slab_reduce");
  });
  m.def("deform_im2col", [](int dt, uintptr_t x, uintptr_t off, uintptr_t msk, uintptr_t cols, std::vector<int> g,
                            uintptr_t s) {
    if (g.size() != 15 && g.size() != 16) throw std::runtime_error("deform_im2col: geometry needs 15 or 16 ints");
    const int rows = g.size() == 16 ? g[15] : 0;
    deform_im2col(dt, P<void>(x), P<void>(off), P<void>(msk), P<void>(cols), g[0], g[1], g[2], g[3], g[4], g[5], g[6],
                  g[7], g[8], g[9], g[10], g[11], g[12], g[13], g[14], rows, S(s));
    check_launch("deform_im2col");
  });
  m.def("deform_col2im", [](int dt, uintptr_t off, uintptr_t msk, uintptr_t gcols, uintptr_t gx, std::vector<int> g,
                            uintptr_t s) {
    if (g.size() != 15 && g.size() != 16) throw std::runtime_error("deform_col2im: geometry needs 15 or 16 ints");
    const int rows = g.size() == 16 ? g[15] : 0;
    deform_col2im(dt, P<void>(off), P<void>(msk), P<void>(gcols), P<float>(gx), g[0], g[1], g[2], g[3], g[4], g[5],
                  g[6], g[7], g[8], g[9], g[10], g[11], g[12], g[13], g[14], rows, S(s));
    check_launch("deform_col2im");
  });
  m.def("deform_col2im_coord", [](int dt, uintptr_t x, uintptr_t off, uintptr_t msk, uintptr_t gcols, uintptr_t goff,
                                  uintptr_t gmsk, std::vector<int> g, uintptr_t s) {
    if (g.size() != 15 && g.size() != 16) throw std::runtime_error("deform_col2im_coord: geometry needs 15 or 16 ints");
    const int rows = g.size() == 16 ? g[15] : 0;
    deform_col2im_coord(dt, P<void>(x), P<void>(off), P<void>(msk), P<void>(gcols), P<void>(goff), P<void>(gmsk),
                        g[0], g[1], g[2], g[3], g[4], g[5], g[6], g[7], g[8], g[9], g[10], g[11], g[12], g[13], g[14],
                        rows, S(s));
    check_launch("deform_col2im_coord");
  });
  m.def("deform_im2col_nhwc", [](int dt, uintptr_t x, uintptr_t off, uintptr_t msk, uintptr_t cols, std::vector<int> g,
                                 int ld_off, int ld_msk, uintptr_t s) {
    if (g.size() != 15) throw std::runtime_error("deform_im2col_nhwc: geometry needs 15 ints");
    deform_im2col_nhwc(dt, P<void>(x), P<void>(off), P<void>(msk), P<void>(cols), g.data(), ld_off, ld_msk, S(s));
    check_launch("deform_im2col_nhwc");
  });
  m.def("deform_bwd_nhwc", [](int dt, uintptr_t x, uintptr_t off, uintptr_t msk, uintptr_t gcols, uintptr_t gx,
                              uintptr_t goff, uintptr_t gmsk, std::vector<int> g, int ld_off, int ld_msk, uintptr_t s) {
    if (g.size() != 15) throw std::runtime_error("deform_bwd_nhwc: geometry needs 15 ints");
    deform_bwd_nhwc(dt, P<void>(x), P<void>(off), P<void>(msk), P<void>(gcols), P<float>(gx), P<void>(goff),
                    P<void>(gmsk), g.data(), ld_off, ld_msk, S(s));
    check_launch("deform_bwd_nhwc");
  });
  m.def("conv_dw_fwd", [](int dt, uintptr_t x, uintptr_t wt, uintptr_t bias, uintptr_t y, std::vector<int> g,
                          uintptr_t s) {
    if (g.size() != 14) throw std::runtime_error("conv_dw_fwd: geometry needs 14 ints");
    conv_dw_fwd(dt, P<void>(x), P<void>(wt), P<float>(bias), P<void>(y), g.data(), S(s));
    check_launch("conv_dw_fwd");
  });
  m.def("conv_dw_dgrad", [](int dt, uintptr_t dy, uintptr_t wt, uintptr_t dx, std::vector<int> g, uintptr_t s) {
    if (g.size() != 14) throw std::runtime_error("conv_dw_dgrad: geometry needs 14 ints");
    conv_dw_dgrad(dt, P<void>(dy), P<void>(wt), P<void>(dx), g.data(), S(s));
    check_launch("conv_dw_dgrad");
  });
  m.def("conv_dw_wgrad", [](int dt, uintptr_t x, uintptr_t dy, uintptr_t slab, int nslice, int out_dt, uintptr_t out,
                            int accum, std::vector<int> g, uintptr_t s) {
    if (g.size() != 14) throw std::runtime_error("conv_dw_wgrad: geometry needs 14 ints");
    conv_dw_wgrad(dt, P<void>(x), P<void>(dy), P<float>(slab), nslice, out_dt, P<void>(out), accum, g.data(), S(s));
    check_launch("conv_dw_wgrad");
  });
  m.def("ssd_loss_blocks", &ssd_loss_blocks);
  m.def("ssd_loss_fwd", [](int dt, uintptr_t cls, uintptr_t loc, uintptr_t ct, uintptr_t lt, uintptr_t lm, int rows,
                           int C1, float lambd, uintptr_t part, uintptr_t out, uintptr_t s) {
    ssd_loss_fwd(dt, P<void>(cls), P<void>(loc), P<float>(ct), P<float>(lt), P<float>(lm), rows, C1, lambd,
                 P<float>(part), P<float>(out), S(s));
    check_launch("ssd_loss_fwd");
  });
  m.def("ssd_loss_bwd", [](int dt, uintptr_t cls, uintptr_t loc, uintptr_t ct, uintptr_t lt, uintptr_t lm,
                           uintptr_t stats, uintptr_t gout, int rows, int C1, float lambd, uintptr_t dcls, uintptr_t dloc,
                           uintptr_t s) {
    ssd_loss_bwd(dt, P<void>(cls), P<void>(loc), P<float>(ct), P<float>(lt), P<float>(lm), P<float>(stats),
                 P<float>(gout), rows, C1, lambd, P<void>(dcls), P<void>(dloc), S(s));
    check_launch("ssd_loss_bwd");
  });
  m.def("multibox_target", [](int dt, uintptr_t anchors, uintptr_t labels, uintptr_t cls_pred, uintptr_t loc_target,
                              uintptr_t loc_mask, uintptr_t cls_target, uintptr_t match_iou, uintptr_t match_gt,
                              uintptr_t key, int B, int A, int L, int W, int C, float thr, float ignore_label,
                              float neg_ratio, float neg_thresh, int min_neg, float v0, float v1, float v2, float v3,
                              uintptr_t s) {
    multibox_target(dt, P<float>(anchors), P<float>(labels), P<void>(cls_pred), P<float>(loc_target),
                    P<float>(loc_mask), P<float>(cls_target), P<float>(match_iou), P<int>(match_gt),
                    P<uint32_t>(key), B, A, L, W, C, thr, ignore_label, neg_ratio, neg_thresh, min_neg, v0, v1, v2,
                    v3, S(s));
    check_launch("multibox_target");
  });
  m.def("bn_nhwc_forward", [](int dt, uintptr_t x, uintptr_t add, uintptr_t y, uintptr_t mask, uintptr_t g, uintptr_t b,
                              uintptr_t center, uintptr_t part, uintptr_t mean, uintptr_t inv, uintptr_t var,
                              uintptr_t scale, uintptr_t shift, int64_t R, int C, float eps, int training, int relu,
                              int fix_gamma, float momentum, uintptr_t mm_upd, uintptr_t mv_upd, int ext_nblk,
                              uintptr_t s, uintptr_t ascale, uintptr_t ashift) {
    bn_nhwc_forward(dt, P<void>(x), P<void>(add), P<void>(y), P<uint8_t>(mask), P<float>(g), P<float>(b), P<float>(center),
                    P<float>(part), P<float>(mean), P<float>(inv), P<float>(var), P<float>(scale), P<float>(shift), R,
                    C, eps, training, relu, fix_gamma, momentum, P<float>(mm_upd), P<float>(mv_upd), ext_nblk, S(s),
                    P<const float>(ascale), P<const float>(ashift));
    check_launch("bn_nhwc_forward");
  }, py::arg("dt"), py::arg("x"), py::arg("add"), py::arg("y"), py::arg("mask"), py::arg("g"), py::arg("b"),
     py::arg("center"), py::arg("part"), py::arg("mean"), py::arg("inv"), py::arg("var"), py::arg("scale"),
     py::arg("shift"), py::arg("R"), py::arg("C"), py::arg("eps"), py::arg("training"), py::arg("relu"),
     py::arg("fix_gamma"), py::arg("momentum"), py::arg("mm_upd"), py::arg("mv_upd"), py::arg("ext_nblk"),
     py::arg("stream"), py::arg("ascale") = 0, py::arg("ashift") = 0);
  m.def("bn_nhwc_backward", [](int dt, uintptr_t x, uintptr_t dy, uintptr_t y, uintptr_t mask, uintptr_t dx,
                               uintptr_t dz,
                               uintptr_t g, uintptr_t mean, uintptr_t inv, uintptr_t fscale, uintptr_t fshift,
                               uintptr_t part, uintptr_t dgamma, uintptr_t dbeta, uintptr_t coef, int64_t R, int C,
                               int relu_mode, int fix_gamma, int training, int accum, uintptr_t s, int ext_nblk,
                               uintptr_t ds_z, uintptr_t ds_mean, uintptr_t ds_part) {
    bn_nhwc_backward(dt, P<void>(x), P<void>(dy), P<void>(y), P<uint8_t>(mask), P<void>(dx), P<void>(dz), P<float>(g), P<float>(mean),
                     P<float>(inv), P<float>(fscale), P<float>(fshift), P<float>(part), P<float>(dgamma),
                     P<float>(dbeta), P<float>(coef), R, C, relu_mode, fix_gamma, training, accum, S(s), ext_nblk,
                     P<const void>(ds_z), P<const float>(ds_mean), P<float>(ds_part));
    check_launch("bn_nhwc_backward");
  }, py::arg("dt"), py::arg("x"), py::arg("dy"), py::arg("y"), py::arg("mask"), py::arg("dx"), py::arg("dz"),
     py::arg("g"), py::arg("mean"), py::arg("inv"), py::arg("fscale"), py::arg("fshift"), py::arg("part"),
     py::arg("dgamma"), py::arg("dbeta"), py::arg("coef"), py::arg("R"), py::arg("C"), py::arg("relu_mode"),
     py::arg("fix_gamma"), py::arg("training"), py::arg("accum"), py::arg("stream"), py::arg("ext_nblk") = 0,
     py::arg("ds_z") = 0, py::arg("ds_mean") = 0, py::arg("ds_part") = 0);
  m.def("softmax_ce_forward", [](int dt, int li, uintptr_t logits, uintptr_t label, uintptr_t loss, uintptr_t lse,
                                 int N, int K, uintptr_t s) {
    softmax_ce_forward(dt, li, P<void>(logits), P<void>(label), P<float>(loss), P<float>(lse), N, K, S(s));
    check_launch("softmax_ce_forward");
  });
  m.def("softmax_ce_backward", [](int dt, int li, uintptr_t logits, uintptr_t label, uintptr_t lse, uintptr_t gout,
                                  uintptr_t dlogits, int N, int K, uintptr_t s) {
    softmax_ce_backward(dt, li, P<void>(logits), P<void>(label), P<float>(lse), P<float>(gout), P<void>(dlogits), N,
                        K, S(s));
    check_launch("softmax_ce_backward");
  });
  m.def("relu_forward", [](int dt, uintptr_t x, uintptr_t y, int64_t n, uintptr_t s) {
    relu_forward(dt, P<void>(x), P<void>(y), n, S(s));
    check_launch("relu_forward");
  });
  m.def("relu_backward", [](int dt, uintptr_t y, uintptr_t dy, uintptr_t dx, int64_t n, uintptr_t s) {
    relu_backward(dt, P<void>(y), P<void>(dy), P<void>(dx), n, S(s));
    check_launch("relu_backward");
  });
  m.def("pointwise_binary", [](int dt, int op, uintptr_t a, uintptr_t b, uintptr_t out, int64_t n, int mode,
                               int64_t row, std::vector<int64_t> shape, std::vector<int64_t> sa,
                               std::vector<int64_t> sb, uintptr_t s) {
    if (shape.size() != sa.size() || shape.size() != sb.size()) throw std::runtime_error("pointwise_binary: rank");
    pointwise_binary(dt, op, P<void>(a), P<void>(b), P<void>(out), n, mode, row, static_cast<int>(shape.size()),
                     shape.data(), sa.data(), sb.data(), S(s));
    check_launch("pointwise_binary");
  });
  m.def("gap_nhwc_forward", [](int dt, uintptr_t x, uintptr_t y, int N, int HW, int C, uintptr_t s) {
    gap_nhwc_forward(dt, P<void>(x), P<void>(y), N, HW, C, S(s));
    check_launch("gap_nhwc_forward");
  });
  m.def("gap_nhwc_backward", [](int dt, uintptr_t dy, uintptr_t dx, int N, int HW, int C, uintptr_t s) {
    gap_nhwc_backward(dt, P<void>(dy), P<void>(dx), N, HW, C, S(s));
    check_launch("gap_nhwc_backward");
  });
  m.def("flat_sgd", [](int dt, uintptr_t w, uintptr_t g, uintptr_t mom, uintptr_t w32, int64_t n, float lr,
                       float wd, float momentum, float rescale, float clip, uintptr_t s) {
    flat_sgd(dt, P<void>(w), P<void>(g), P<float>(mom), P<float>(w32), n, lr, wd, momentum, rescale, clip, nullptr,
             S(s));
    check_launch("flat_sgd");
  });
  m.def("flat_sgd", [](int dt, uintptr_t w, uintptr_t g, uintptr_t mom, uintptr_t w32, int64_t n, float lr,
                       float wd, float momentum, float rescale, float clip, uintptr_t s, uintptr_t hp) {
    flat_sgd(dt, P<void>(w), P<void>(g), P<float>(mom), P<float>(w32), n, lr, wd, momentum, rescale, clip,
             P<float>(hp), S(s));
    check_launch("flat_sgd");
  });
  m.def("conv_nhwc_fwd", [](int dt, uintptr_t x, uintptr_t w, uintptr_t bias, uintptr_t y, int N, int H, int W,
                            int C, int K, int R, int Sf, int sh, int sw, int ph, int pw, int variant, uintptr_t s) {
    conv_nhwc_fwd(dt, P<void>(x), P<void>(w), P<float>(bias), P<void>(y), N, H, W, C, K, R, Sf, sh, sw, ph, pw,
                  variant, S(s));
    check_launch("conv_nhwc_fwd");
  });
  m.def("conv_nhwc_fwd_glds", [](int dt, uintptr_t x, uintptr_t w, uintptr_t bias, uintptr_t y, uintptr_t zero, int N,
                                 int H, int W, int C, int K, int R, int Sf, int sh, int sw, int ph, int pw, int bco,
                                 uintptr_t s, uintptr_t bn_z, uintptr_t bn_mean, uintptr_t bn_scale,
                                 uintptr_t bn_shift, uintptr_t bn_part, int bn_nparts) {
    conv_nhwc_fwd_glds(dt, P<void>(x), P<void>(w), P<float>(bias), P<void>(y), P<void>(zero), N, H, W, C, K, R, Sf,
                       sh, sw, ph, pw, bco, S(s), P<void>(bn_z), P<float>(bn_mean), P<float>(bn_scale),
                       P<float>(bn_shift), P<float>(bn_part), bn_nparts);
    check_launch("conv_nhwc_fwd_glds");
  }, py::arg("dtype"), py::arg("x"), py::arg("w"), py::arg("bias"), py::arg("y"), py::arg("zero"), py::arg("N"),
     py::arg("H"), py::arg("W"), py::arg("C"), py::arg("K"), py::arg("R"), py::arg("S"), py::arg("sh"),
     py::arg("sw"), py::arg("ph"), py::arg("pw"), py::arg("bco"), py::arg("stream"), py::arg("bn_z") = 0,
     py::arg("bn_mean") = 0, py::arg("bn_scale") = 0, py::arg("bn_shift") = 0, py::arg("bn_part") = 0,
     py::arg("bn_nparts") = 0);
  m.def("conv_glds_bwd_nparts", &conv_glds_bwd_nparts);
  m.def("conv_nhwc_dgrad_phases_glds",
        [](int dt, uintptr_t dy, uintptr_t w, uintptr_t dx, uintptr_t zero, int N, int Hi, int Wi, int Cin, int Cout,
           int Ho, int Wo, int stride, std::vector<int> ph, std::vector<int> pw, std::vector<int> R,
           std::vector<int> Sf, std::vector<int> pad_h, std::vector<int> pad_w, std::vector<int64_t> w_off,
           std::vector<int> zph, std::vector<int> zpw, int bco, uintptr_t s, uintptr_t bn_z, uintptr_t bn_mean,
           uintptr_t bn_scale, uintptr_t bn_shift, uintptr_t bn_part, int bn_nparts) {
          const size_t n = ph.size();
          if (pw.size() != n || R.size() != n || Sf.size() != n || pad_h.size() != n || pad_w.size() != n ||
              w_off.size() != n || zph.size() != zpw.size())
            throw std::runtime_error("conv_nhwc_dgrad_phases_glds: per-phase lists differ in length");
          conv_nhwc_dgrad_phases_glds(dt, P<void>(dy), P<void>(w), P<void>(dx), P<void>(zero), N, Hi, Wi, Cin, Cout,
                                      Ho, Wo, stride, (int)n, ph.data(), pw.data(), R.data(), Sf.data(),
                                      pad_h.data(), pad_w.data(), w_off.data(), (int)zph.size(), zph.data(),
                                      zpw.data(), bco, S(s), P<void>(bn_z), P<float>(bn_mean), P<float>(bn_scale),
                                      P<float>(bn_shift), P<float>(bn_part), bn_nparts);
          check_launch("conv_nhwc_dgrad_phases_glds");
        },
        py::arg("dtype"), py::arg("dy"), py::arg("w"), py::arg("dx"), py::arg("zero"), py::arg("N"), py::arg("Hi"),
        py::arg("Wi"), py::arg("Cin"), py::arg("Cout"), py::arg("Ho"), py::arg("Wo"), py::arg("stride"),
        py::arg("ph"), py::arg("pw"), py::arg("R"), py::arg("S"), py::arg("pad_h"), py::arg("pad_w"),
        py::arg("w_off"), py::arg("zph"), py::arg("zpw"), py::arg("bco"), py::arg("stream"), py::arg("bn_z") = 0,
        py::arg("bn_mean") = 0, py::arg("bn_scale") = 0, py::arg("bn_shift") = 0, py::arg("bn_part") = 0,
        py::arg("bn_nparts") = 0);
  m.def("conv_stem_grid", &conv_stem_grid);
  m.def("conv_stem_wgrad_workspace", &conv_stem_wgrad_workspace);
  m.def("conv_stem_fwd", [](int dt, uintptr_t x, uintptr_t w, uintptr_t y, int N, int H, int W, int C, int K, int R,
                            int Sf, int sh, int sw, int ph, int pw, uintptr_t part, int nparts, uintptr_t s) {
    conv_stem_fwd(dt, P<void>(x), P<void>(w), P<void>(y), N, H, W, C, K, R, Sf, sh, sw, ph, pw, P<float>(part),
                  nparts, S(s));
    check_launch("conv_stem_fwd");
  });
  m.def("conv_stem_wgrad", [](int dt, uintptr_t x, uintptr_t dy, uintptr_t slab, int odt, uintptr_t out, int accum,
                              int N, int H, int W, int C, int K, int R, int Sf, int sh, int sw, int ph, int pw,
                              uintptr_t s) {
    conv_stem_wgrad(dt, P<void>(x), P<void>(dy), P<float>(slab), odt, P<void>(out), accum, N, H, W, C, K, R, Sf, sh,
                    sw, ph, pw, S(s));
    check_launch("conv_stem_wgrad");
  });
  m.def("conv_nhwc_fwd_big_nparts", &conv_nhwc_fwd_big_nparts);
  m.def("conv_nhwc_fwd_big_bwd_nparts", &conv_nhwc_fwd_big_bwd_nparts);
  m.def("conv_nhwc_fwd_big", [](int dt, uintptr_t x, uintptr_t w, uintptr_t bias, uintptr_t y, uintptr_t zero, int N,
                                int H, int W, int C, int K, int R, int Sf, int sh, int sw, int ph, int pw, int variant,
                                uintptr_t part, int nparts, uintptr_t addend, uintptr_t s, uintptr_t bz,
                                uintptr_t bmean, uintptr_t bscale, uintptr_t bshift, uintptr_t bmask, int bmode,
                                uintptr_t bpart, int bnparts, int up, int dh, int dw) {
    conv_nhwc_fwd_big(dt, P<void>(x), P<void>(w), P<float>(bias), P<void>(y), P<void>(zero), N, H, W, C, K, R, Sf, sh,
                      sw, ph, pw, variant, P<float>(part), nparts, P<void>(addend), S(s), P<void>(bz), P<float>(bmean),
                      P<float>(bscale), P<float>(bshift), P<uint8_t>(bmask), bmode, P<float>(bpart), bnparts, up, dh,
                      dw);
    check_launch("conv_nhwc_fwd_big");
  }, py::arg("dt"), py::arg("x"), py::arg("w"), py::arg("bias"), py::arg("y"), py::arg("zero"), py::arg("N"),
     py::arg("H"), py::arg("W"), py::arg("C"), py::arg("K"), py::arg("R"), py::arg("S"), py::arg("sh"),
     py::arg("sw"), py::arg("ph"), py::arg("pw"), py::arg("variant"), py::arg("part"), py::arg("nparts"),
     py::arg("addend"), py::arg("stream"), py::arg("bn_z") = 0, py::arg("bn_mean") = 0, py::arg("bn_scale") = 0,
     py::arg("bn_shift") = 0, py::arg("bn_mask") = 0, py::arg("bn_mode") = 0, py::arg("bn_part") = 0,
     py::arg("bn_nparts") = 0, py::arg("up") = 0, py::arg("dh") = 1, py::arg("dw") = 1);
  m.def("conv_nhwc_fwd_ring_nparts", &conv_nhwc_fwd_ring_nparts);
  m.def("conv_nhwc_fwd_ring", [](int dt, uintptr_t x, uintptr_t w, uintptr_t y, uintptr_t zero, int N, int H, int W,
                                 int C, int K, int R, int Sf, int sh, int sw, int ph, int pw, int variant, uintptr_t part,
                                 int nparts, uintptr_t s) {
    conv_nhwc_fwd_ring(dt, P<void>(x), P<void>(w), P<void>(y), P<void>(zero), N, H, W, C, K, R, Sf, sh, sw, ph, pw,
                       variant, P<float>(part), nparts, S(s));
    check_launch("conv_nhwc_fwd_ring");
  });
  m.def("conv3x3_halo_ok", &conv3x3_halo_ok);
  m.def("conv3x3_halo_nparts", &conv3x3_halo_nparts);
  m.def("conv3x3_halo", [](int dt, uintptr_t x, uintptr_t w, uintptr_t y, uintptr_t zero, int N, int H, int W, int C,
                           int K, uintptr_t part, int nparts, uintptr_t bn_z, uintptr_t bn_mean, uintptr_t bn_scale,
                           uintptr_t bn_shift, int bn_mode, uintptr_t bn_part, uintptr_t s) {
    conv3x3_halo(dt, P<void>(x), P<void>(w), P<void>(y), P<void>(zero), N, H, W, C, K, P<float>(part), nparts,
// ... 199 lines not shown
```

### src/kernels/bn_nhwc.hip

```cpp
#include <cstdlib>
#include <stdexcept>

#include <algorithm>

#include "common.h"

namespace mxamd {

constexpr int kBnThreads = 256;

struct BnGeom {
  int tpr;
  int cb;
  int rpi;
};

static inline BnGeom bn_geom(int C) {
  BnGeom g;
  int v = C / 8;
  g.tpr = v;
  if (v > kBnThreads)
    for (g.tpr = kBnThreads; v % g.tpr != 0; --g.tpr) {
    }
  g.cb = g.tpr * 8;
  g.rpi = kBnThreads / g.tpr;
  return g;
}

constexpr int kReluNone = 0;
constexpr int kReluFromY = 1;
constexpr int kReluFromX = 2;
constexpr int kReluFromMask = 3;

template <typename T, int MODE, int RELU>
__global__ void __launch_bounds__(kBnThreads) bn_reduce_kernel(
    const T* __restrict__ x, const T* __restrict__ dy, const T* __restrict__ y, const uint8_t* __restrict__ mask,
    const float* __restrict__ center, const float* __restrict__ fscale, const float* __restrict__ fshift,
    float* __restrict__ part1, float* __restrict__ part2, int64_t R, int C, int tpr, int rpi,
    int64_t rows_per_block) {
  const int tid = threadIdx.x;
  const int lane_c = tid % tpr;
  const int lane_r = tid / tpr;
  const int cbase = blockIdx.y * tpr * 8 + lane_c * 8;
  float s1[8], s2[8], k[8], fs[8], fh[8];
#pragma unroll
  for (int i = 0; i < 8; ++i) {
    s1[i] = 0.f;
    s2[i] = 0.f;
    k[i] = center[cbase + i];
    if (RELU == kReluFromX) {
      fs[i] = fscale[cbase + i];
      fh[i] = fshift[cbase + i];
    }
  }
  const int64_t r0 = static_cast<int64_t>(blockIdx.x) * rows_per_block;
  int64_t r1 = r0 + rows_per_block;
  if (r1 > R) r1 = R;
  const bool spare = lane_r >= rpi;
  if (spare) r1 = r0;
  constexpr int UNR = 4;
  auto accum = [&](const Vec8<T>& vx, const Vec8<T>& vdy, const Vec8<T>& vy, uint32_t mb) {
#pragma unroll
    for (int i = 0; i < 8; ++i) {
      if (MODE == 0) {
        float d = vx.get(i) - k[i];
        s1[i] += d;
        s2[i] += d * d;
      } else {
        float dz = vdy.get(i);
        const float xi = vx.get(i);
        if (RELU == kReluFromY) dz = vy.get(i) > 0.f ? dz : 0.f;
        if (RELU == kReluFromX) dz = fmaf(xi, fs[i], fh[i]) > 0.f ? dz : 0.f;
        if (RELU == kReluFromMask) dz = ((mb >> i) & 1u) ? dz : 0.f;
        s1[i] += dz;
        s2[i] += dz * (xi - k[i]);
      }
    }
  };
  int64_t r = r0 + lane_r;
  for (; r + (UNR - 1) * rpi < r1; r += UNR * rpi) {
    Vec8<T> vx[UNR], vdy[UNR], vy[UNR];
    uint32_t vm[UNR];
#pragma unroll
    for (int u = 0; u < UNR; ++u) {
      const int64_t off = (r + u * rpi) * C + cbase;
      vx[u].load(x + off);
      if (MODE == 1) vdy[u].load(dy + off);
      if (MODE == 1 && RELU == kReluFromY) vy[u].load(y + off);
      vm[u] = (MODE == 1 && RELU == kReluFromMask) ? mask[off >> 3] : 0u;
    }
#pragma unroll
    for (int u = 0; u < UNR; ++u) accum(vx[u], vdy[u], vy[u], vm[u]);
  }
  for (; r < r1; r += rpi) {
    const int64_t off = r * C + cbase;
    Vec8<T> vx, vdy, vy;
    vx.load(x + off);
    if (MODE == 1) vdy.load(dy + off);
    if (MODE == 1 && RELU == kReluFromY) vy.load(y + off);
    accum(vx, vdy, vy, (MODE == 1 && RELU == kReluFromMask) ? mask[off >> 3] : 0u);
  }
  __shared__ float sh1[kBnThreads * 8];
  __shared__ float sh2[kBnThreads * 8];
  const int cb = tpr * 8;
  if (!spare) {
#pragma unroll
    for (int i = 0; i < 8; ++i) {
      sh1[lane_r * cb + lane_c * 8 + i] = s1[i];
      sh2[lane_r * cb + lane_c * 8 + i] = s2[i];
    }
  }
  __syncthreads();
  for (int c = tid; c < cb; c += kBnThreads) {
    float a = 0.f, b = 0.f;
    for (int rr = 0; rr < rpi; ++rr) {
      a += sh1[rr * cb + c];
      b += sh2[rr * cb + c];
    }
    const int64_t o = static_cast<int64_t>(blockIdx.y * cb + c) * gridDim.x + blockIdx.x;
    part1[o] = a;
    part2[o] = b;
  }
}

constexpr int kFinThreads = 256;
constexpr int kFinPerBlock = kFinThreads / 64;
template <int MODE>
__global__ void __launch_bounds__(kFinThreads) bn_finalize_kernel(
    const float* __restrict__ part1, const float* __restrict__ part2, int nblk, int C, int64_t R,
    const float* __restrict__ center, const float* __restrict__ gamma, const float* __restrict__ beta,
    const float* __restrict__ invstd_in, float eps, float* __restrict__ o0, float* __restrict__ o1,
    float* __restrict__ o2, float* __restrict__ o3, float* __restrict__ o4, float* __restrict__ o5,
    int fix_gamma, int training, float momentum, float* __restrict__ mm_upd, float* __restrict__ mv_upd,
    int accum) {
  const int lane = threadIdx.x & 63;
  const int c = blockIdx.x * kFinPerBlock + (threadIdx.x >> 6);
  if (c >= C) return;
  const float* p1 = part1 + static_cast<int64_t>(c) * nblk;
  const float* p2 = part2 + static_cast<int64_t>(c) * nblk;
  double a = 0.0, b = 0.0;
  const int nv = ((reinterpret_cast<uintptr_t>(p1) | reinterpret_cast<uintptr_t>(p2)) & 15) == 0 ? nblk / 4 : 0;
  for (int i = lane; i < nv; i += 64) {
    const float4 x = reinterpret_cast<const float4*>(p1)[i];
    const float4 y = reinterpret_cast<const float4*>(p2)[i];
    a += static_cast<double>(x.x) + static_cast<double>(x.y) + static_cast<double>(x.z) + static_cast<double>(x.w);
    b += static_cast<double>(y.x) + static_cast<double>(y.y) + static_cast<double>(y.z) + static_cast<double>(y.w);
  }
  for (int i = nv * 4 + lane; i < nblk; i += 64) {
    a += p1[i];
    b += p2[i];
  }
#pragma unroll
  for (int o = 32; o > 0; o >>= 1) {
    a += __shfl_xor(a, o, 64);
    b += __shfl_xor(b, o, 64);
  }
  if (lane != 0) return;
  const double n = static_cast<double>(R);
  const float g = fix_gamma ? 1.f : gamma[c];
  if (MODE == 0) {
    double m1 = a / n;
    double var = b / n - m1 * m1;
    if (var < 0) var = 0;
    double mean = center[c] + m1;
    float inv = static_cast<float>(1.0 / sqrt(var + eps));
    o0[c] = static_cast<float>(mean);
    o1[c] = inv;
    o2[c] = static_cast<float>(var);
    float sc = g * inv;
    o3[c] = sc;
    o4[c] = beta[c] - static_cast<float>(mean) * sc;
    if (mm_upd) mm_upd[c] = mm_upd[c] * momentum + static_cast<float>(mean) * (1.f - momentum);
    if (mv_upd) mv_upd[c] = mv_upd[c] * momentum + static_cast<float>(var) * (1.f - momentum);
  } else {
    const float inv = invstd_in[c];
    const double dbeta = a;
    const double dgamma = b * inv;
    if (accum) {
      o0[c] += static_cast<float>(dgamma);
      o1[c] += static_cast<float>(dbeta);
    } else {
      o0[c] = static_cast<float>(dgamma);
      o1[c] = static_cast<float>(dbeta);
    }
    const double A = static_cast<double>(g) * inv;
    const double B = training ? -A * inv * dgamma / n : 0.0;
    const double Cc = training ? A * (static_cast<double>(center[c]) * inv * dgamma / n - dbeta / n) : 0.0;
    o2[c] = static_cast<float>(A);
    o3[c] = static_cast<float>(B);
    o4[c] = static_cast<float>(Cc);
  }
}

typedef unsigned int bn_u32x4 __attribute__((ext_vector_type(4)));

template <typename T>
__device__ __forceinline__ void vload(Vec8<T>& v, const T* p, int nt) {
  if constexpr (sizeof(T) == 2) {
    if (nt) {
      const bn_u32x4 r = __builtin_nontemporal_load(reinterpret_cast<const bn_u32x4*>(p));
      v.raw = make_uint4(r.x, r.y, r.z, r.w);
      return;
    }
  }
  v.load(p);
}

template <typename T>
__device__ __forceinline__ void vstore(const Vec8<T>& v, T* p, int nt) {
  if constexpr (sizeof(T) == 2) {
    if (nt > 1) {
      const bn_u32x4 r = {v.raw.x, v.raw.y, v.raw.z, v.raw.w};
      __builtin_nontemporal_store(r, reinterpret_cast<bn_u32x4*>(p));
      return;
    }
  }
  v.store(p);
}

__device__ __forceinline__ void load8f(const float* __restrict__ p, float* o) {
  const float4 a = *reinterpret_cast<const float4*>(p);
  const float4 b = *reinterpret_cast<const float4*>(p + 4);
  o[0] = a.x; o[1] = a.y; o[2] = a.z; o[3] = a.w; o[4] = b.x; o[5] = b.y; o[6] = b.z; o[7] = b.w;
}


template <typename T, bool ADD, bool RELU, bool MASK, bool AFF = false>
__global__ void __launch_bounds__(kBnThreads) bn_apply_kernel(
    const T* __restrict__ x, const T* __restrict__ addend, const float* __restrict__ scale,
    const float* __restrict__ shift, T* __restrict__ y, uint8_t* __restrict__ mask, int64_t nvec, int C, int nt,
    const float* __restrict__ ascale, const float* __restrict__ ashift) {
  static_assert(ADD || !AFF, "an affine addend needs the add");
  const int64_t stride = static_cast<int64_t>(gridDim.x) * blockDim.x;
  int64_t v = static_cast<int64_t>(blockIdx.x) * blockDim.x + threadIdx.x;
  int c = static_cast<int>((v * 8) % C);
  const int cstep = static_cast<int>((stride * 8) % C);
  float sc[8], sh[8], asc[8], ash[8];
  auto coef = [&](int cc) {
    load8f(scale + cc, sc);
    load8f(shift + cc, sh);
    if (AFF) {
      load8f(ascale + cc, asc);
      load8f(ashift + cc, ash);
    }
  };
  auto compute = [&](const Vec8<T>& vx, Vec8<T> va, int64_t vv) {
    Vec8<T> out;
    uint32_t bits = 0;
    if (AFF) {
#pragma unroll
      for (int i = 0; i < 8; ++i) va.set(i, va.get(i) * asc[i] + ash[i]);
    }
#pragma unroll
    for (int i = 0; i < 8; ++i) {
      float r = vx.get(i) * sc[i] + sh[i];
      if (ADD) r += va.get(i);
      if (MASK) bits |= (r > 0.f ? 1u : 0u) << i;
      if (RELU) r = r > 0.f ? r : 0.f;
      out.set(i, r);
    }
    vstore(out, y + vv * 8, nt == 2 ? 2 : 0);
    if (MASK) mask[vv] = static_cast<uint8_t>(bits);
  };
  if (cstep == 0) {
    coef(c);
    for (; v + stride < nvec; v += 2 * stride) {
      Vec8<T> vx0, vx1, va0, va1;
      vload(vx0, x + v * 8, nt);
      vload(vx1, x + (v + stride) * 8, nt);
      if (ADD) {
        vload(va0, addend + v * 8, nt);
        vload(va1, addend + (v + stride) * 8, nt);
      }
      compute(vx0, va0, v);
      compute(vx1, va1, v + stride);
    }
    if (v < nvec) {
      Vec8<T> vx, va;
      vload(vx, x + v * 8, nt);
      if (ADD) vload(va, addend + v * 8, nt);
      compute(vx, va, v);
    }
    return;
  }
  for (; v < nvec; v += stride, c = (c + cstep >= C) ? c + cstep - C : c + cstep) {
    Vec8<T> vx, va;
    vload(vx, x + v * 8, nt);
    if (ADD) vload(va, addend + v * 8, nt);
    coef(c);
    compute(vx, va, v);
  }
}

template <typename T, int RELU, bool WRITE_DZ>
__global__ void __launch_bounds__(kBnThreads) bn_bwd_apply_kernel(
    const T* __restrict__ x, const T* __restrict__ dy, const T* __restrict__ y, const uint8_t* __restrict__ mask,
    const float* __restrict__ A, const float* __restrict__ B, const float* __restrict__ Cc,
    const float* __restrict__ fscale, const float* __restrict__ fshift,
    T* __restrict__ dx, T* __restrict__ dz_out, int64_t nvec, int C, int nt) {
  const int64_t stride = static_cast<int64_t>(gridDim.x) * blockDim.x;
  int64_t v = static_cast<int64_t>(blockIdx.x) * blockDim.x + threadIdx.x;
  int c = static_cast<int>((v * 8) % C);
  const int cstep = static_cast<int>((stride * 8) % C);
  float fs[8], fh[8], ka[8], kb[8], kc[8];
  auto coef = [&](int cc) {
    if (RELU == kReluFromX) {
      load8f(fscale + cc, fs);
      load8f(fshift + cc, fh);
    }
    load8f(A + cc, ka);
    load8f(B + cc, kb);
    load8f(Cc + cc, kc);
  };
  struct In {
    Vec8<T> x, dy, y;
    uint32_t mb;
  };
  auto load = [&](In& in, int64_t vv) {
    vload(in.x, x + vv * 8, nt);
    vload(in.dy, dy + vv * 8, nt);
    if (RELU == kReluFromY) vload(in.y, y + vv * 8, nt);
    in.mb = RELU == kReluFromMask ? mask[vv] : 0u;
  };
  auto compute = [&](const In& in, int64_t vv) {
    Vec8<T> out, dz;
#pragma unroll
    for (int i = 0; i < 8; ++i) {
      float d = in.dy.get(i);
      if (RELU == kReluFromY) d = in.y.get(i) > 0.f ? d : 0.f;
      if (RELU == kReluFromX) d = fmaf(in.x.get(i), fs[i], fh[i]) > 0.f ? d : 0.f;
      if (RELU == kReluFromMask) d = ((in.mb >> i) & 1u) ? d : 0.f;
      if (WRITE_DZ) dz.set(i, d);
      out.set(i, ka[i] * d + kb[i] * in.x.get(i) + kc[i]);
    }
    vstore(out, dx + vv * 8, nt == 2 ? 2 : 0);
    if (WRITE_DZ) vstore(dz, dz_out + vv * 8, nt >= 2 ? 2 : 0);
  };
  if (cstep == 0) {
    coef(c);
    for (; v + stride < nvec; v += 2 * stride) {
      In i0, i1;
      load(i0, v);
      load(i1, v + stride);
      compute(i0, v);
      compute(i1, v + stride);
    }
    if (v < nvec) {
      In i0;
      load(i0, v);
      compute(i0, v);
    }
    return;
  }
  for (; v < nvec; v += stride, c = (c + cstep >= C) ? c + cstep - C : c + cstep) {
    In i0;
    load(i0, v);
    coef(c);
    compute(i0, v);
  }
}

template <typename T>
__global__ void __launch_bounds__(kBnThreads) bn_tail_bwd_ds_kernel(
    const T* __restrict__ x, const T* __restrict__ dy, const uint8_t* __restrict__ mask,
    const float* __restrict__ A, const float* __restrict__ B, const float* __restrict__ Cc, T* __restrict__ dx,
    T* __restrict__ dz_out, const T* __restrict__ zds, const float* __restrict__ mean_ds, float* __restrict__ part1,
    float* __restrict__ part2, int64_t R, int C, int tpr, int rpi, int64_t rows_per_block, int nt) {
  const int tid = threadIdx.x;
  const int lane_c = tid % tpr;
  const int lane_r = tid / tpr;
  const int cbase = blockIdx.y * tpr * 8 + lane_c * 8;
  float s1[8], s2[8], ka[8], kb[8], kc[8], km[8];
#pragma unroll
  for (int i = 0; i < 8; ++i) {
    s1[i] = 0.f;
    s2[i] = 0.f;
    ka[i] = A[cbase + i];
    kb[i] = B[cbase + i];
    kc[i] = Cc[cbase + i];
    km[i] = mean_ds[cbase + i];
  }
  const int64_t r0 = static_cast<int64_t>(blockIdx.x) * rows_per_block;
  int64_t r1 = r0 + rows_per_block;
  if (r1 > R) r1 = R;
  const bool spare = lane_r >= rpi;
  if (spare) r1 = r0;
  constexpr int UNR = 2;
  auto body = [&](const Vec8<T>& vx, const Vec8<T>& vdy, const Vec8<T>& vz, uint32_t mb, int64_t off) {
    Vec8<T> out, dz;
#pragma unroll
    for (int i = 0; i < 8; ++i) {
      const float d = ((mb >> i) & 1u) ? vdy.get(i) : 0.f;
      dz.set(i, d);
      out.set(i, ka[i] * d + kb[i] * vx.get(i) + kc[i]);
      s1[i] += d;
      s2[i] += d * (vz.get(i) - km[i]);
    }
    out.store(dx + off);
    if (dz_out != nullptr) vstore(dz, dz_out + off, nt >= 2 ? 2 : 0);
  };
  int64_t r = r0 + lane_r;
  for (; r + (UNR - 1) * rpi < r1; r += UNR * rpi) {
    Vec8<T> vx[UNR], vdy[UNR], vz[UNR];
    uint32_t vm[UNR];
#pragma unroll
    for (int u = 0; u < UNR; ++u) {
      const int64_t off = (r + u * rpi) * C + cbase;
      vload(vx[u], x + off, nt);
      vload(vdy[u], dy + off, nt);
      vload(vz[u], zds + off, nt);
      vm[u] = mask[off >> 3];
    }
#pragma unroll
    for (int u = 0; u < UNR; ++u) body(vx[u], vdy[u], vz[u], vm[u], (r + u * rpi) * C + cbase);
  }
  for (; r < r1; r += rpi) {
    const int64_t off = r * C + cbase;
    Vec8<T> vx, vdy, vz;
    vload(vx, x + off, nt);
    vload(vdy, dy + off, nt);
    vload(vz, zds + off, nt);
    body(vx, vdy, vz, mask[off >> 3], off);
  }
  __shared__ float sh1[kBnThreads * 8];
  __shared__ float sh2[kBnThreads * 8];
  const int cb = tpr * 8;
  if (!spare) {
#pragma unroll
    for (int i = 0; i < 8; ++i) {
      sh1[lane_r * cb + lane_c * 8 + i] = s1[i];
      sh2[lane_r * cb + lane_c * 8 + i] = s2[i];
    }
  }
  __syncthreads();
  for (int c = tid; c < cb; c += kBnThreads) {
    float a = 0.f, b = 0.f;
    for (int rr = 0; rr < rpi; ++rr) {
      a += sh1[rr * cb + c];
      b += sh2[rr * cb + c];
    }
    const int64_t o = static_cast<int64_t>(blockIdx.y * cb + c) * gridDim.x + blockIdx.x;
    part1[o] = a;
    part2[o] = b;
  }
}


static int bn_nt() { return 1; }

static int bn_total_blocks() { return 512; }

static inline int64_t bn_rows_per_block(int64_t R, int C, const BnGeom& g, int* nblk,
                                        int total_blocks = bn_total_blocks(), int min_rows = 0) {
  const int cblocks = C / g.cb;
  int64_t target = total_blocks / cblocks;
  if (target < 8) target = 8;
  int64_t rpb = (R + target - 1) / target;
  rpb = (rpb + g.rpi - 1) / g.rpi * g.rpi;
  if (rpb < g.rpi * 4) rpb = g.rpi * 4;
  if (rpb < min_rows) rpb = (min_rows + g.rpi - 1) / g.rpi * g.rpi;
  *nblk = static_cast<int>((R + rpb - 1) / rpb);
  return rpb;
}

static int bn_tail_blocks() { return 1024; }

int bn_tail_ds_rows(int64_t R, int C) {
  BnGeom g = bn_geom(C);
  int nblk;
  bn_rows_per_block(R, C, g, &nblk, bn_tail_blocks(), 64);
  return nblk;
}

int bn_partials_rows(int64_t R, int C) {
  BnGeom g = bn_geom(C);
  int nblk;
  bn_rows_per_block(R, C, g, &nblk);
  return nblk;
}

template <typename T>
static void bn_forward_impl(const void* x, const void* addend, void* y, uint8_t* mask, const float* gamma,
                            const float* beta, const float* center, float* part, float* mean, float* invstd,
                            float* var, float* scale, float* shift, int64_t R, int C, float eps, int training,
                            int relu, int fix_gamma, float momentum, float* mm_upd, float* mv_upd, int ext_nblk,
                            hipStream_t s, const float* ascale, const float* ashift) {
  MXAMD_HOST_CHECK(C % 8 == 0, "bn_nhwc: channels must be a multiple of 8");
  BnGeom g = bn_geom(C);
  MXAMD_HOST_CHECK(C % g.cb == 0, "bn_nhwc: unsupported channel count");
  if (training) {
    int nblk;
    float* p1 = part;
    if (ext_nblk > 0) {
      nblk = ext_nblk;
    } else {
      int64_t rpb = bn_rows_per_block(R, C, g, &nblk);
      dim3 grid(nblk, C / g.cb);
      float* p2r = part + static_cast<int64_t>(nblk) * C;
      hipLaunchKernelGGL((bn_reduce_kernel<T, 0, kReluNone>), grid, dim3(kBnThreads), 0, s,
                         static_cast<const T*>(x), nullptr, nullptr, nullptr, center, nullptr, nullptr, p1, p2r, R, C,
                         g.tpr, g.rpi, rpb);
    }
    float* p2 = part + static_cast<int64_t>(nblk) * C;
    hipLaunchKernelGGL((bn_finalize_kernel<0>), dim3((C + kFinPerBlock - 1) / kFinPerBlock), dim3(kFinThreads), 0, s, p1, p2, nblk, C, R, center, gamma,
                       beta, nullptr, eps, mean, invstd, var, scale, shift, nullptr, fix_gamma, 1, momentum, mm_upd,
                       mv_upd, 0);
  }
  if (y == nullptr) return;
  const int64_t nvec = R * C / 8;
  int blocks = static_cast<int>((nvec + kBnThreads - 1) / kBnThreads);
  if (blocks > 256 * 16) blocks = 256 * 16;
  const T* xa = static_cast<const T*>(x);
  const T* aa = static_cast<const T*>(addend);
  T* ya = static_cast<T*>(y);
  const float* no_coef = nullptr;
#define APPLY(ADD, RELU, MASK)                                                                              \
  hipLaunchKernelGGL((bn_apply_kernel<T, ADD, RELU, MASK>), dim3(blocks), dim3(kBnThreads), 0, s, xa, aa, scale, \
                     shift, ya, mask, nvec, C, bn_nt(), no_coef, no_coef)
  MXAMD_HOST_CHECK(mask == nullptr || (addend && relu), "bn_nhwc_forward: mask output only for add+relu");
  MXAMD_HOST_CHECK((ascale == nullptr) == (ashift == nullptr) && (ascale == nullptr || addend),
                   "bn_nhwc_forward: an affine addend needs the addend and both of its coefficient vectors");
  if (ascale) {
#define APPLY_AFF(RELU, MASK)                                                                                 \
  hipLaunchKernelGGL((bn_apply_kernel<T, true, RELU, MASK, true>), dim3(blocks), dim3(kBnThreads), 0, s, xa, aa, \
                     scale, shift, ya, mask, nvec, C, bn_nt(), ascale, ashift)
    if (relu) {
      if (mask) APPLY_AFF(true, true); else APPLY_AFF(true, false);
    } else {
      APPLY_AFF(false, false);
    }
#undef APPLY_AFF
  } else if (addend) {
    if (relu) {
      if (mask) APPLY(true, true, true); else APPLY(true, true, false);
    } else {
      APPLY(true, false, false);
    }
  } else {
    if (relu) APPLY(false, true, false); else APPLY(false, false, false);
  }
#undef APPLY
}

template <typename T>
static void bn_backward_impl(const void* x, const void* dy, const void* y, const uint8_t* mask, void* dx, void* dz,
                             const float* gamma, const float* mean, const float* invstd, const float* fscale,
                             const float* fshift, float* part, float* dgamma, float* dbeta, float* coef, int64_t R,
                             int C, int relu_mode, int fix_gamma, int training, int accum, hipStream_t s,
                             int ext_nblk, const void* ds_z, const float* ds_mean, float* ds_part) {
  BnGeom g = bn_geom(C);
  int nblk;
  int64_t rpb = bn_rows_per_block(R, C, g, &nblk);
  if (ext_nblk > 0) nblk = ext_nblk;
  dim3 grid(nblk, C / g.cb);
  float* p1 = part;
  float* p2 = part + static_cast<int64_t>(nblk) * C;
  const T* xa = static_cast<const T*>(x);
  const T* dya = static_cast<const T*>(dy);
  const T* ya = static_cast<const T*>(y);
  MXAMD_HOST_CHECK(relu_mode != kReluFromY || y != nullptr, "bn_nhwc_backward: relu mask from y needs y");
  MXAMD_HOST_CHECK(relu_mode != kReluFromX || (fscale && fshift), "bn_nhwc_backward: relu-from-x needs scale/shift");
  MXAMD_HOST_CHECK(relu_mode != kReluFromMask || mask != nullptr, "bn_nhwc_backward: relu-from-mask needs the mask");
#define RED(RL)                                                                                                \
  hipLaunchKernelGGL((bn_reduce_kernel<T, 1, RL>), grid, dim3(kBnThreads), 0, s, xa, dya, ya, mask, mean, fscale, \
                     fshift,                                                                                         \
                     p1, p2, R, C, g.tpr, g.rpi, rpb)
  if (ext_nblk > 0) {
  } else if (relu_mode == kReluFromY) RED(kReluFromY);
  else if (relu_mode == kReluFromX) RED(kReluFromX);
  else if (relu_mode == kReluFromMask) RED(kReluFromMask);
  else RED(kReluNone);
#undef RED
  float* A = coef;
  float* B = coef + C;
  float* Cc = coef + 2 * C;
  hipLaunchKernelGGL((bn_finalize_kernel<1>), dim3((C + kFinPerBlock - 1) / kFinPerBlock), dim3(kFinThreads), 0, s, p1, p2, nblk, C, R, mean, gamma, nullptr,
                     invstd, 0.f, dgamma, dbeta, A, B, Cc, nullptr, fix_gamma, training, 0.f, nullptr,
                     nullptr, accum);
  const int64_t nvec = R * C / 8;
  int blocks = static_cast<int>((nvec + kBnThreads - 1) / kBnThreads);
  if (blocks > 256 * 16) blocks = 256 * 16;
  T* dxa = static_cast<T*>(dx);
  T* dza = static_cast<T*>(dz);
  if (ds_z) {
    MXAMD_HOST_CHECK(relu_mode == kReluFromMask && ds_mean && ds_part,
                     "bn_nhwc_backward: shortcut statistics need the tail's mask mode and the BN's mean");
    int dnblk;
    const int64_t drpb = bn_rows_per_block(R, C, g, &dnblk, bn_tail_blocks(), 64);
    hipLaunchKernelGGL((bn_tail_bwd_ds_kernel<T>), dim3(dnblk, C / g.cb), dim3(kBnThreads), 0, s, xa, dya, mask, A, B,
                       Cc, dxa, dza, static_cast<const T*>(ds_z), ds_mean, ds_part,
                       ds_part + static_cast<int64_t>(dnblk) * C, R, C, g.tpr, g.rpi, drpb, bn_nt());
    return;
  }
#define BWD(RL, WD)                                                                                      \
  hipLaunchKernelGGL((bn_bwd_apply_kernel<T, RL, WD>), dim3(blocks), dim3(kBnThreads), 0, s, xa, dya, ya, mask, A, B, \
                     Cc, fscale, fshift, dxa, dza, nvec, C, bn_nt())
  if (relu_mode == kReluFromY) {
    if (dz) BWD(kReluFromY, true); else BWD(kReluFromY, false);
  } else if (relu_mode == kReluFromX) {
    if (dz) BWD(kReluFromX, true); else BWD(kReluFromX, false);
  } else if (relu_mode == kReluFromMask) {
    if (dz) BWD(kReluFromMask, true); else BWD(kReluFromMask, false);
  } else {
    if (dz) BWD(kReluNone, true); else BWD(kReluNone, false);
  }
#undef BWD
}

int bn_nhwc_stats(int dtype, const void* x, const float* center, float* part, int64_t R, int C, hipStream_t s,
                  int total_blocks) {
  MXAMD_HOST_CHECK(C % 8 == 0, "bn_nhwc: channels must be a multiple of 8");
  BnGeom g = bn_geom(C);
  MXAMD_HOST_CHECK(C % g.cb == 0, "bn_nhwc: unsupported channel count");
  int nblk;
  int64_t rpb = bn_rows_per_block(R, C, g, &nblk, total_blocks);
  dim3 grid(nblk, C / g.cb);
  float* p2 = part + static_cast<int64_t>(nblk) * C;
#define STATS(T)                                                                                              \
  hipLaunchKernelGGL((bn_reduce_kernel<T, 0, kReluNone>), grid, dim3(kBnThreads), 0, s, static_cast<const T*>(x), \
                     nullptr, nullptr, nullptr, center, nullptr, nullptr, part, p2, R, C, g.tpr, g.rpi, rpb)
  if (dtype == kF16) STATS(__half); else if (dtype == kBF16) STATS(__hip_bfloat16); else STATS(float);
#undef STATS
  return nblk;
}

namespace {
constexpr int kColsumTargetBlocks = 768;

inline void colsum_geom(int64_t R, int C, int* nchunk, int* rows_per) {
  const int strips = (C + 63) / 64;
  int64_t n = (kColsumTargetBlocks + strips - 1) / strips;
  n = std::max<int64_t>(1, std::min<int64_t>(n, (R + 31) / 32));
  int64_t rp = (R + n - 1) / n;
  rp = (rp + 31) / 32 * 32;
  *rows_per = static_cast<int>(rp);
  *nchunk = static_cast<int>((R + rp - 1) / rp);
}

template <typename T>
__global__ void __launch_bounds__(256) colsum_part_kernel(const T* __restrict__ x, int64_t R, int C, int rows_per,
                                                          float* __restrict__ part) {
  __shared__ float red[32][64 + 1];
  const int cv = threadIdx.x & 7, ty = threadIdx.x >> 3;
  const int c0 = (blockIdx.x * 8 + cv) * 8;
  const int64_t r0 = static_cast<int64_t>(blockIdx.y) * rows_per;
  const int64_t r1 = r0 + rows_per < R ? r0 + rows_per : R;
  float a[8] = {0.f, 0.f, 0.f, 0.f, 0.f, 0.f, 0.f, 0.f};
  if (c0 < C) {
    for (int64_t r = r0 + ty; r < r1; r += 32) {
      Vec8<T> v;
      v.load(x + r * C + c0);
#pragma unroll
      for (int i = 0; i < 8; ++i) a[i] += v.get(i);
    }
  }
#pragma unroll
  for (int i = 0; i < 8; ++i) red[ty][cv * 8 + i] = a[i];
  __syncthreads();
  if (threadIdx.x < 64) {
    const int col = threadIdx.x;
    float t = 0.f;
#pragma unroll 8
    for (int j = 0; j < 32; ++j) t += red[j][col];
    const int c = blockIdx.x * 64 + col;
    if (c < C) part[static_cast<int64_t>(blockIdx.y) * C + c] = t;
  }
}

template <typename TO>
__global__ void __launch_bounds__(256) colsum_fin_kernel(const float* __restrict__ part, int nchunk, int C,
                                                         TO* __restrict__ out, int accum) {
  __shared__ float red[16][17];
  const int col = threadIdx.x & 15, l16 = threadIdx.x >> 4;
  const int c = blockIdx.x * 16 + col;
  float t0 = 0.f, t1 = 0.f, t2 = 0.f, t3 = 0.f;
  if (c < C) {
    int i = l16;
    for (; i + 48 < nchunk; i += 64) {
      t0 += part[static_cast<int64_t>(i) * C + c];
      t1 += part[static_cast<int64_t>(i + 16) * C + c];
      t2 += part[static_cast<int64_t>(i + 32) * C + c];
      t3 += part[static_cast<int64_t>(i + 48) * C + c];
    }
    for (; i < nchunk; i += 16) t0 += part[static_cast<int64_t>(i) * C + c];
  }
  red[l16][col] = (t0 + t1) + (t2 + t3);
  __syncthreads();
  if (l16 == 0 && c < C) {
    float t = 0.f;
#pragma unroll
    for (int j = 0; j < 16; ++j) t += red[j][col];
    if (accum) t += static_cast<float>(out[c]);
    out[c] = static_cast<TO>(t);
  }
}
}

int64_t colsum_partials(int64_t R, int C) {
  int nchunk, rows_per;
  colsum_geom(R, C, &nchunk, &rows_per);
  return static_cast<int64_t>(nchunk) * C;
}

void colsum_rows(int dtype, const void* x, const float* zeros, float* part, int64_t R, int C, int out_dtype,
                 void* out, int accum, hipStream_t s) {
  (void)zeros;
  MXAMD_HOST_CHECK(C % 8 == 0, "colsum_rows: columns must be a multiple of 8");
  int nchunk, rows_per;
  colsum_geom(R, C, &nchunk, &rows_per);
  const dim3 grid((C + 63) / 64, nchunk);
  if (dtype == kF16)
    hipLaunchKernelGGL(colsum_part_kernel<__half>, grid, dim3(256), 0, s, static_cast<const __half*>(x), R, C,
                       rows_per, part);
  else if (dtype == kBF16)
    hipLaunchKernelGGL(colsum_part_kernel<__hip_bfloat16>, grid, dim3(256), 0, s,
                       static_cast<const __hip_bfloat16*>(x), R, C, rows_per, part);
  else
    hipLaunchKernelGGL(colsum_part_kernel<float>, grid, dim3(256), 0, s, static_cast<const float*>(x), R, C,
                       rows_per, part);
  const dim3 g2((C + 15) / 16);
  if (out_dtype == kF16)
    hipLaunchKernelGGL(colsum_fin_kernel<__half>, g2, dim3(256), 0, s, part, nchunk, C, static_cast<__half*>(out),
                       accum);
  else if (out_dtype == kBF16)
    hipLaunchKernelGGL(colsum_fin_kernel<__hip_bfloat16>, g2, dim3(256), 0, s, part, nchunk, C,
                       static_cast<__hip_bfloat16*>(out), accum);
  else
    hipLaunchKernelGGL(colsum_fin_kernel<float>, g2, dim3(256), 0, s, part, nchunk, C, static_cast<float*>(out),
                       accum);
}

void bn_nhwc_forward(int dtype, const void* x, const void* addend, void* y, uint8_t* mask, const float* gamma,
                     const float* beta,
                     const float* center, float* part, float* mean, float* invstd, float* var, float* scale,
                     float* shift, int64_t R, int C, float eps, int training, int relu, int fix_gamma,
                     float momentum, float* mm_upd, float* mv_upd, int ext_nblk, hipStream_t s, const float* ascale,
                     const float* ashift) {
  switch (dtype) {
    case kF16:
      bn_forward_impl<__half>(x, addend, y, mask, gamma, beta, center, part, mean, invstd, var, scale, shift, R, C, eps,
                              training, relu, fix_gamma, momentum, mm_upd, mv_upd, ext_nblk, s, ascale, ashift);
      break;
    case kBF16:
      bn_forward_impl<__hip_bfloat16>(x, addend, y, mask, gamma, beta, center, part, mean, invstd, var, scale, shift, R,
                                      C, eps, training, relu, fix_gamma, momentum, mm_upd, mv_upd, ext_nblk, s, ascale,
                                      ashift);
      break;
    default:
      bn_forward_impl<float>(x, addend, y, mask, gamma, beta, center, part, mean, invstd, var, scale, shift, R, C, eps,
                             training, relu, fix_gamma, momentum, mm_upd, mv_upd, ext_nblk, s, ascale, ashift);
  }
}

void bn_finalize_backward(const float* part, int nblk, int C, int64_t R, const float* mean, const float* gamma,
                          const float* invstd, float* dgamma, float* dbeta, float* coef, int fix_gamma, int training,
                          int accum, hipStream_t s) {
  hipLaunchKernelGGL((bn_finalize_kernel<1>), dim3((C + kFinPerBlock - 1) / kFinPerBlock), dim3(kFinThreads), 0, s, part,
                     part + static_cast<int64_t>(nblk) * C, nblk, C, R, mean, gamma, nullptr, invstd, 0.f, dgamma,
                     dbeta, coef, coef + C, coef + 2 * C, nullptr, fix_gamma, training, 0.f, nullptr, nullptr, accum);
}

void bn_nhwc_backward(int dtype, const void* x, const void* dy, const void* y, const uint8_t* mask, void* dx,
                      void* dz,
                      const float* gamma, const float* mean, const float* invstd, const float* fscale,
                      const float* fshift, float* part, float* dgamma, float* dbeta, float* coef, int64_t R, int C,
                      int relu_mode, int fix_gamma, int training, int accum, hipStream_t s, int ext_nblk,
                      const void* ds_z, const float* ds_mean, float* ds_part) {
  switch (dtype) {
    case kF16:
      bn_backward_impl<__half>(x, dy, y, mask, dx, dz, gamma, mean, invstd, fscale, fshift, part, dgamma, dbeta, coef, R,
                               C, relu_mode, fix_gamma, training, accum, s, ext_nblk, ds_z, ds_mean, ds_part);
      break;
    case kBF16:
      bn_backward_impl<__hip_bfloat16>(x, dy, y, mask, dx, dz, gamma, mean, invstd, fscale, fshift, part, dgamma, dbeta,
                                       coef, R, C, relu_mode, fix_gamma, training, accum, s, ext_nblk, ds_z, ds_mean,
                                       ds_part);
      break;
    default:
      bn_backward_impl<float>(x, dy, y, mask, dx, dz, gamma, mean, invstd, fscale, fshift, part, dgamma, dbeta, coef, R,
                              C, relu_mode, fix_gamma, training, accum, s, ext_nblk, ds_z, ds_mean, ds_part);
  }
}

}
```

### src/kernels/pointwise.hip

```cpp
#include <stdexcept>

#include "common.h"

namespace mxamd {

namespace {

constexpr int kPwThreads = 256;
constexpr int kPwMaxDims = 6;

enum PwOp { kAdd = 0, kSub = 1, kMul = 2, kDiv = 3, kMax = 4, kMin = 5 };

template <int OP>
__device__ __forceinline__ float pw_apply(float a, float b) {
  if (OP == kAdd) return a + b;
  if (OP == kSub) return a - b;
  if (OP == kMul) return a * b;
  if (OP == kDiv) return a / b;
  if (OP == kMax) return a >= b ? a : b;
  return a <= b ? a : b;
}

template <typename T>
struct PwVec {
  static constexpr int N = 16 / sizeof(T);
};

template <typename T>
__device__ __forceinline__ float to_f(T v) {
  return static_cast<float>(v);
}
template <>
__device__ __forceinline__ float to_f<__half>(__half v) {
  return __half2float(v);
}
template <>
__device__ __forceinline__ float to_f<__hip_bfloat16>(__hip_bfloat16 v) {
  return __bfloat162float(v);
}

template <typename T>
__device__ __forceinline__ T from_f(float v) {
  return static_cast<T>(v);
}
template <>
__device__ __forceinline__ __half from_f<__half>(float v) {
  return __float2half(v);
}
template <>
__device__ __forceinline__ __hip_bfloat16 from_f<__hip_bfloat16>(float v) {
  return __float2bfloat16(v);
}

template <typename T>
union PwPack {
  uint4 raw;
  T e[PwVec<T>::N];
};

inline unsigned pw_blocks(int64_t work) {
  int64_t b = (work + kPwThreads - 1) / kPwThreads;
  if (b > 256 * 8 * 4) b = 256 * 8 * 4;
  return static_cast<unsigned>(b < 1 ? 1 : b);
}

template <typename T>
__global__ void __launch_bounds__(kPwThreads) relu_fwd_kernel(const T* __restrict__ x, T* __restrict__ y, int64_t n) {
  constexpr int V = PwVec<T>::N;
  const int64_t nv = n / V;
  const int64_t stride = static_cast<int64_t>(gridDim.x) * kPwThreads;
  for (int64_t i = static_cast<int64_t>(blockIdx.x) * kPwThreads + threadIdx.x; i < nv; i += stride) {
    PwPack<T> p;
    p.raw = reinterpret_cast<const uint4*>(x)[i];
#pragma unroll
    for (int k = 0; k < V; ++k) {
      const float v = to_f(p.e[k]);
      p.e[k] = from_f<T>(v > 0.f ? v : 0.f);
    }
    reinterpret_cast<uint4*>(y)[i] = p.raw;
  }
  if (blockIdx.x == 0) {
    for (int64_t i = nv * V + threadIdx.x; i < n; i += kPwThreads) {
      const float v = to_f(x[i]);
      y[i] = from_f<T>(v > 0.f ? v : 0.f);
    }
  }
}

template <typename T>
__global__ void __launch_bounds__(kPwThreads) relu_bwd_kernel(const T* __restrict__ y, const T* __restrict__ dy,
                                                              T* __restrict__ dx, int64_t n) {
  constexpr int V = PwVec<T>::N;
  const int64_t nv = n / V;
  const int64_t stride = static_cast<int64_t>(gridDim.x) * kPwThreads;
  for (int64_t i = static_cast<int64_t>(blockIdx.x) * kPwThreads + threadIdx.x; i < nv; i += stride) {
    PwPack<T> py, pd;
    py.raw = reinterpret_cast<const uint4*>(y)[i];
    pd.raw = reinterpret_cast<const uint4*>(dy)[i];
#pragma unroll
    for (int k = 0; k < V; ++k) pd.e[k] = to_f(py.e[k]) > 0.f ? pd.e[k] : from_f<T>(0.f);
    reinterpret_cast<uint4*>(dx)[i] = pd.raw;
  }
  if (blockIdx.x == 0) {
    for (int64_t i = nv * V + threadIdx.x; i < n; i += kPwThreads) dx[i] = to_f(y[i]) > 0.f ? dy[i] : from_f<T>(0.f);
  }
}

template <typename T, int OP, int ROW, bool SWAP>
__global__ void __launch_bounds__(kPwThreads) binary_vec_kernel(const T* __restrict__ a, const T* __restrict__ b,
                                                                T* __restrict__ out, int64_t n, int64_t row) {
  constexpr int V = PwVec<T>::N;
  const int64_t nv = n / V;
  const int64_t stride = static_cast<int64_t>(gridDim.x) * kPwThreads;
  for (int64_t i = static_cast<int64_t>(blockIdx.x) * kPwThreads + threadIdx.x; i < nv; i += stride) {
    PwPack<T> pa, pb;
    pa.raw = reinterpret_cast<const uint4*>(a)[i];
    const int64_t bi = ROW ? (i * V) % row / V : i;
    pb.raw = reinterpret_cast<const uint4*>(b)[bi];
#pragma unroll
    for (int k = 0; k < V; ++k) {
      const float x = to_f(pa.e[k]), yv = to_f(pb.e[k]);
      pa.e[k] = from_f<T>(SWAP ? pw_apply<OP>(yv, x) : pw_apply<OP>(x, yv));
    }
    reinterpret_cast<uint4*>(out)[i] = pa.raw;
  }
  if (blockIdx.x == 0) {
    for (int64_t i = nv * V + threadIdx.x; i < n; i += kPwThreads) {
      const float x = to_f(a[i]), yv = to_f(b[ROW ? i % row : i]);
      out[i] = from_f<T>(SWAP ? pw_apply<OP>(yv, x) : pw_apply<OP>(x, yv));
    }
  }
}

struct PwGeom {
  int ndim;
  int64_t shape[kPwMaxDims];
  int64_t sa[kPwMaxDims];
  int64_t sb[kPwMaxDims];
};

template <typename T, int OP>
__global__ void __launch_bounds__(kPwThreads) binary_strided_kernel(const T* __restrict__ a, const T* __restrict__ b,
                                                                    T* __restrict__ out, int64_t n, PwGeom g) {
  const int64_t stride = static_cast<int64_t>(gridDim.x) * kPwThreads;
  for (int64_t i = static_cast<int64_t>(blockIdx.x) * kPwThreads + threadIdx.x; i < n; i += stride) {
    int64_t rem = i, oa = 0, ob = 0;
    for (int d = g.ndim - 1; d >= 0; --d) {
      const int64_t q = rem / g.shape[d];
      const int64_t idx = rem - q * g.shape[d];
      rem = q;
      oa += idx * g.sa[d];
      ob += idx * g.sb[d];
    }
    out[i] = from_f<T>(pw_apply<OP>(to_f(a[oa]), to_f(b[ob])));
  }
}

template <typename T, int OP>
void binary_launch(const T* a, const T* b, T* out, int64_t n, int mode, int64_t row, const PwGeom& g,
                   hipStream_t s) {
  constexpr int V = PwVec<T>::N;
  const unsigned vb = pw_blocks(n / V + 1);
  if (mode == 0) {
    hipLaunchKernelGGL((binary_vec_kernel<T, OP, 0, false>), dim3(vb), dim3(kPwThreads), 0, s, a, b, out, n, row);
  } else if (mode == 1) {
    hipLaunchKernelGGL((binary_vec_kernel<T, OP, 1, false>), dim3(vb), dim3(kPwThreads), 0, s, a, b, out, n, row);
  } else if (mode == 2) {
    hipLaunchKernelGGL((binary_vec_kernel<T, OP, 1, true>), dim3(vb), dim3(kPwThreads), 0, s, b, a, out, n, row);
  } else {
    hipLaunchKernelGGL((binary_strided_kernel<T, OP>), dim3(pw_blocks(n)), dim3(kPwThreads), 0, s, a, b, out, n, g);
  }
}

template <typename T>
void binary_dispatch(int op, const T* a, const T* b, T* out, int64_t n, int mode, int64_t row, const PwGeom& g,
                     hipStream_t s) {
  switch (op) {
    case kAdd: binary_launch<T, kAdd>(a, b, out, n, mode, row, g, s); break;
    case kSub: binary_launch<T, kSub>(a, b, out, n, mode, row, g, s); break;
    case kMul: binary_launch<T, kMul>(a, b, out, n, mode, row, g, s); break;
    case kDiv: binary_launch<T, kDiv>(a, b, out, n, mode, row, g, s); break;
    case kMax: binary_launch<T, kMax>(a, b, out, n, mode, row, g, s); break;
    case kMin: binary_launch<T, kMin>(a, b, out, n, mode, row, g, s); break;
    default: throw std::runtime_error("pointwise_binary: unknown op");
  }
}


constexpr int kTapMax = 32;
struct TapTable {
  int src[kTapMax];
  int64_t base[kTapMax];
  int64_t rstride[kTapMax];
};

template <typename E>
__global__ void __launch_bounds__(256) weight_taps_t_kernel(const E* __restrict__ w, E* __restrict__ out, int K, int RS,
                                                            int C, TapTable tt) {
  __shared__ E tile[64][65];
  const int z = blockIdx.z;
  const int k0 = blockIdx.y * 64, c0 = blockIdx.x * 64;
  const int src = tt.src[z];
  for (int i = threadIdx.x; i < 64 * 64; i += 256) {
    const int kk = i >> 6, cc = i & 63;
    const int k = k0 + kk, c = c0 + cc;
    if (k < K && c < C) tile[kk][cc] = w[(static_cast<int64_t>(k) * RS + src) * C + c];
  }
  __syncthreads();
  const int64_t base = tt.base[z], rs = tt.rstride[z];
  for (int i = threadIdx.x; i < 64 * 64; i += 256) {
    const int cc = i >> 6, kk = i & 63;
    const int k = k0 + kk, c = c0 + cc;
    if (k < K && c < C) out[base + static_cast<int64_t>(c) * rs + k] = tile[kk][cc];
  }
}

__global__ void __launch_bounds__(256) weight_taps_t_vec_kernel(const uint16_t* __restrict__ w,
                                                                uint16_t* __restrict__ out, int K, int RS, int C,
                                                                TapTable tt) {
  __shared__ __attribute__((aligned(16))) uint16_t tile[64][72];
  const int z = blockIdx.z;
  const int k0 = blockIdx.y * 64, c0 = blockIdx.x * 64;
  const int src = tt.src[z];
  const int tid = threadIdx.x;
  uint4 r[2];
#pragma unroll
  for (int i = 0; i < 2; ++i) {
    const int v = tid + i * 256;
    const int k = k0 + (v >> 3), c = c0 + (v & 7) * 8;
    r[i] = (k < K && c < C) ? *reinterpret_cast<const uint4*>(w + (static_cast<int64_t>(k) * RS + src) * C + c)
                            : uint4{0u, 0u, 0u, 0u};
  }
#pragma unroll
  for (int i = 0; i < 2; ++i) {
    const int v = tid + i * 256;
    *reinterpret_cast<uint4*>(&tile[v >> 3][(v & 7) * 8]) = r[i];
  }
  __syncthreads();
  const int64_t base = tt.base[z], rs = tt.rstride[z];
#pragma unroll
  for (int i = 0; i < 2; ++i) {
    const int v = tid + i * 256;
    const int cc = v >> 3, kv = (v & 7) * 8;
    const int c = c0 + cc, k = k0 + kv;
    if (c < C && k < K) {
      uint32_t q[4];
#pragma unroll
      for (int j = 0; j < 4; ++j)
        q[j] = static_cast<uint32_t>(tile[kv + 2 * j][cc]) | (static_cast<uint32_t>(tile[kv + 2 * j + 1][cc]) << 16);
      *reinterpret_cast<uint4*>(out + base + static_cast<int64_t>(c) * rs + k) = uint4{q[0], q[1], q[2], q[3]};
    }
  }
}

}

void weight_taps_t(int elem_bytes, const void* w, void* out, int K, int RS, int C, int n, const int* src,
                   const int64_t* base, const int64_t* rstride, hipStream_t s) {
  MXAMD_HOST_CHECK(n >= 1 && n <= kTapMax, "weight_taps_t: 1..32 tap slots");
  TapTable tt{};
  for (int z = 0; z < n; ++z) {
    MXAMD_HOST_CHECK(src[z] >= 0 && src[z] < RS, "weight_taps_t: tap index out of range");
    tt.src[z] = src[z];
    tt.base[z] = base[z];
    tt.rstride[z] = rstride[z];
  }
  const dim3 grid((C + 63) / 64, (K + 63) / 64, n);
  bool vec = elem_bytes == 2 && K % 8 == 0 && C % 8 == 0 && reinterpret_cast<uintptr_t>(w) % 16 == 0 &&
             reinterpret_cast<uintptr_t>(out) % 16 == 0;
  for (int z = 0; z < n && vec; ++z) vec = base[z] % 8 == 0 && rstride[z] % 8 == 0;
  if (vec)
    hipLaunchKernelGGL(weight_taps_t_vec_kernel, grid, dim3(256), 0, s, static_cast<const uint16_t*>(w),
                       static_cast<uint16_t*>(out), K, RS, C, tt);
  else if (elem_bytes == 2)
    hipLaunchKernelGGL(weight_taps_t_kernel<uint16_t>, grid, dim3(256), 0, s, static_cast<const uint16_t*>(w),
                       static_cast<uint16_t*>(out), K, RS, C, tt);
  else if (elem_bytes == 4)
    hipLaunchKernelGGL(weight_taps_t_kernel<uint32_t>, grid, dim3(256), 0, s, static_cast<const uint32_t*>(w),
                       static_cast<uint32_t*>(out), K, RS, C, tt);
  else
    throw std::runtime_error("weight_taps_t: 2- or 4-byte elements");
}

void relu_forward(int dtype, const void* x, void* y, int64_t n, hipStream_t s) {
  const unsigned blocks = pw_blocks(n / 8 + 1);
  if (dtype == kF16)
    hipLaunchKernelGGL(relu_fwd_kernel<__half>, dim3(blocks), dim3(kPwThreads), 0, s, static_cast<const __half*>(x),
                       static_cast<__half*>(y), n);
  else if (dtype == kBF16)
    hipLaunchKernelGGL(relu_fwd_kernel<__hip_bfloat16>, dim3(blocks), dim3(kPwThreads), 0, s,
                       static_cast<const __hip_bfloat16*>(x), static_cast<__hip_bfloat16*>(y), n);
  else
    hipLaunchKernelGGL(relu_fwd_kernel<float>, dim3(blocks), dim3(kPwThreads), 0, s, static_cast<const float*>(x),
                       static_cast<float*>(y), n);
}

void relu_backward(int dtype, const void* y, const void* dy, void* dx, int64_t n, hipStream_t s) {
  const unsigned blocks = pw_blocks(n / 8 + 1);
  if (dtype == kF16)
    hipLaunchKernelGGL(relu_bwd_kernel<__half>, dim3(blocks), dim3(kPwThreads), 0, s, static_cast<const __half*>(y),
                       static_cast<const __half*>(dy), static_cast<__half*>(dx), n);
  else if (dtype == kBF16)
    hipLaunchKernelGGL(relu_bwd_kernel<__hip_bfloat16>, dim3(blocks), dim3(kPwThreads), 0, s,
                       static_cast<const __hip_bfloat16*>(y), static_cast<const __hip_bfloat16*>(dy),
                       static_cast<__hip_bfloat16*>(dx), n);
  else
    hipLaunchKernelGGL(relu_bwd_kernel<float>, dim3(blocks), dim3(kPwThreads), 0, s, static_cast<const float*>(y),
                       static_cast<const float*>(dy), static_cast<float*>(dx), n);
}

void pointwise_binary(int dtype, int op, const void* a, const void* b, void* out, int64_t n, int mode, int64_t row,
                      int ndim, const int64_t* shape, const int64_t* astride, const int64_t* bstride, hipStream_t s) {
  MXAMD_HOST_CHECK(ndim <= kPwMaxDims, "pointwise_binary: at most 6 dimensions");
  MXAMD_HOST_CHECK(mode == 0 || mode == 3 || (row > 0 && row % (dtype == kF32 ? 4 : 8) == 0),
                   "pointwise_binary: row broadcast needs a row length that is a multiple of the vector width");
  PwGeom g{};
  g.ndim = ndim;
  for (int d = 0; d < ndim; ++d) {
    g.shape[d] = shape[d];
    g.sa[d] = astride[d];
    g.sb[d] = bstride[d];
  }
  if (n == 0) return;
  if (dtype == kF16)
    binary_dispatch<__half>(op, static_cast<const __half*>(a), static_cast<const __half*>(b), static_cast<__half*>(out),
                            n, mode, row, g, s);
  else if (dtype == kBF16)
    binary_dispatch<__hip_bfloat16>(op, static_cast<const __hip_bfloat16*>(a), static_cast<const __hip_bfloat16*>(b),
                                    static_cast<__hip_bfloat16*>(out), n, mode, row, g, s);
  else
    binary_dispatch<float>(op, static_cast<const float*>(a), static_cast<const float*>(b), static_cast<float*>(out), n,
                           mode, row, g, s);
}

}
```

Before: 12650 images/sec.

## Batch per-backward weight relayouts into one multi-job launch and fuse dual BN forward

Adds a per-backward-pass relayout plan that collects all dgrad weight flip/transpose jobs seen in the previous backward and launches them together as one table-driven kernel at the start of the next backward, instead of one small kernel per conv. It also fuses the shortcut BatchNorm stats pass and the main BatchNorm forward into a single dual kernel during training. The aim is to cut kernel-launch count and small-kernel tail overhead, particularly inside the captured HIP graph. The cost is added bookkeeping, stream waits, table uploads and graph-lifetime pinning of buffers, with some risk of stale relayouts if weights are reallocated.

```diff
diff --git a/mxnet_maintenance_amd/_state.py b/mxnet_maintenance_amd/_state.py
--- a/mxnet_maintenance_amd/_state.py
+++ b/mxnet_maintenance_amd/_state.py
@@ -16,6 +16,23 @@
 DIRECT_GRAD = [0]
 
 
+BACKWARD_EPOCH = [0]
+BACKWARD_DEPTH = [0]
+
+
+class backward_pass:
+
+    def __enter__(self):
+        if BACKWARD_DEPTH[0] == 0:
+            BACKWARD_EPOCH[0] += 1
+        BACKWARD_DEPTH[0] += 1
+        return self
+
+    def __exit__(self, *exc):
+        BACKWARD_DEPTH[0] -= 1
+        return False
+
+
 def is_recording():
     return STATE.recording
 
@@ -24,6 +41,7 @@
     return STATE.training
 
 GRAPH_RNG = [None]
+GRAPH_KEEP = [None]
 
 
 GRAD_TOUCHED = set()
diff --git a/mxnet_maintenance_amd/autograd.py b/mxnet_maintenance_amd/autograd.py
--- a/mxnet_maintenance_amd/autograd.py
+++ b/mxnet_maintenance_amd/autograd.py
@@ -217,7 +217,7 @@
     if direct:
         _state.DIRECT_GRAD[0] += 1
     try:
-        with torch.enable_grad() if create_graph else torch.no_grad():
+        with (torch.enable_grad() if create_graph else torch.no_grad()), _state.backward_pass():
             torch.autograd.backward(tensors, grads, retain_graph=retain_graph or create_graph,
                                     create_graph=create_graph)
     finally:
@@ -249,7 +249,7 @@
         prev_train = set_training(train_mode)
         prev_rec = set_recording(create_graph)
         try:
-            with torch.enable_grad():
+            with torch.enable_grad(), _state.backward_pass():
                 gs = torch.autograd.grad([h for h, _ in live], [v._data for v in variables],
                                          grad_outputs=[g for _, g in live], retain_graph=retain_graph,
                                          create_graph=create_graph, allow_unused=True)
diff --git a/mxnet_maintenance_amd/executor.py b/mxnet_maintenance_amd/executor.py
--- a/mxnet_maintenance_amd/executor.py
+++ b/mxnet_maintenance_amd/executor.py
@@ -548,8 +548,9 @@
             hgs.append(torch.ones_like(o) if g is None else g._data.to(o.dtype).reshape(o.shape))
         names = [n for n, _ in self._leaves]
         ts = [t for _, t in self._leaves]
-        grads = (torch.autograd.grad(heads, ts, hgs, allow_unused=True, retain_graph=False)
-                 if heads and ts else [None] * len(ts))
+        with _state.backward_pass():
+            grads = (torch.autograd.grad(heads, ts, hgs, allow_unused=True, retain_graph=False)
+                     if heads and ts else [None] * len(ts))
         gd = self.grad_dict
         with torch.no_grad():
             for n, g in zip(names, grads):
diff --git a/mxnet_maintenance_amd/gluon/graph_step.py b/mxnet_maintenance_amd/gluon/graph_step.py
--- a/mxnet_maintenance_amd/gluon/graph_step.py
+++ b/mxnet_maintenance_amd/gluon/graph_step.py
@@ -29,6 +29,7 @@
         self._rng = None
         self._fallback = fallback
         self._eager_only = False
+        self._keep = []
 
     @property
     def captured(self):
@@ -73,6 +74,7 @@
         torch.cuda.synchronize(dev)
         graph = torch.cuda.CUDAGraph()
         _state.GRAPH_RNG[0] = self._rng
+        self._keep = _state.GRAPH_KEEP[0] = []
         try:
             with torch.cuda.graph(graph, stream=s):
                 self._static_out = self._fn(*self._static_in)
@@ -82,6 +84,7 @@
             raise
         finally:
             _state.GRAPH_RNG[0] = None
+            _state.GRAPH_KEEP[0] = None
         self._graph = graph
 
     def _load_inputs(self, inputs):
@@ -149,6 +152,7 @@
             self._trainer._exit_graph_mode()
         self._graph = None
         self._static_out = None
+        self._keep = []
 
     def reset(self):
         if self._trainer is not None and self._graph is not None:
@@ -156,4 +160,5 @@
         self._graph = None
         self._static_out = None
         self._static_in = None
+        self._keep = []
         self._calls = self._warmup
diff --git a/mxnet_maintenance_amd/ops/kernel_fns.py b/mxnet_maintenance_amd/ops/kernel_fns.py
--- a/mxnet_maintenance_amd/ops/kernel_fns.py
+++ b/mxnet_maintenance_amd/ops/kernel_fns.py
@@ -291,14 +291,18 @@
         dt = _DT[x.dtype]
         zg, zmean, zinvstd, _zvar, zscale, zshift, zargs, zhost = _bn_fwd_stats(
             lib, z, zgamma, zbeta, zmoving_mean, zmoving_var, eps, training, momentum)
-        if training:
-            lib.bn_nhwc_forward(dt, z.data_ptr(), 0, 0, 0, *zargs(False))
         g, mean, invstd, var, scale, shift, args, host = _bn_fwd_stats(
             lib, x, gamma, beta, moving_mean, moving_var, eps, training, momentum)
         y = torch.empty_like(x)
         mask = torch.empty(x.numel() // 8, dtype=torch.uint8, device=dev)
-        lib.bn_nhwc_forward(dt, x.data_ptr(), z.data_ptr(), y.data_ptr(), mask.data_ptr(), *args(True),
-                            zscale.data_ptr(), zshift.data_ptr())
+        if training:
+            xa, za = args(True), zargs(False)
+            lib.bn_nhwc_forward_dual(dt, x.data_ptr(), z.data_ptr(), y.data_ptr(), mask.data_ptr(),
+                                     list(xa[:9] + xa[16:18]), xa[18], list(za[:9] + za[16:18]), za[18],
+                                     xa[9], xa[10], xa[11], 0, xa[15], xa[19])
+        else:
+            lib.bn_nhwc_forward(dt, x.data_ptr(), z.data_ptr(), y.data_ptr(), mask.data_ptr(), *args(True),
+                                zscale.data_ptr(), zshift.data_ptr())
         for h in (zhost, host):
             if h is not None:
                 h()
@@ -831,13 +835,101 @@
     return out
 
 
+class _RelayoutJob:
+    __slots__ = ('w', 'out', 'src', 'base', 'rstride', 'seen')
+
+    def __init__(self, w, out, src, base, rstride, seen):
+        self.w, self.out, self.src, self.base, self.rstride, self.seen = w, out, src, base, rstride, seen
+
+
+class _RelayoutPlan:
+    def __init__(self):
+        self.jobs = {}
+        self.epoch = None
+        self.serial = 0
+        self.table = None
+        self.fresh = frozenset()
+        self.stream = None
+        self.launches = 0
+
+    def begin(self, epoch, capturing):
+        prev, self.serial, self.epoch, self.fresh = self.serial, self.serial + 1, epoch, frozenset()
+        if not capturing:
+            for k in [k for k, j in self.jobs.items() if j.seen != prev]:
+                del self.jobs[k]
+        keys = tuple(self.jobs)
+        if not keys:
+            self.table = None
+            return
+        if self.table is None or self.table[2] != keys:
+            if capturing:
+                return
+            self.table = self._upload(keys)
+        table, blocks, _ = self.table
+        _K.lib().weight_taps_t_multi(table.data_ptr(), blocks, _stream())
+        self.launches += 1
+        self.fresh = frozenset(keys)
+        self.stream = (_stream(), torch.cuda.current_stream())
+        if capturing:
+            keep = _state.GRAPH_KEEP[0]
+            (keep if keep is not None else _RELAYOUT_PINNED).append((table, [(j.w, j.out) for j in self.jobs.values()]))
+
+    def _upload(self, keys):
+        jobs = [self.jobs[k] for k in keys]
+        begin, src, base, rstride = [0], [], [], []
+        for j in jobs:
+            src += j.src
+            base += j.base
+            rstride += j.rstride
+            begin.append(len(src))
+        image, blocks = _K.lib().weight_taps_t_multi_table(
+            [j.w.element_size() for j in jobs], [j.w.data_ptr() for j in jobs], [j.out.data_ptr() for j in jobs],
+            [j.out.numel() for j in jobs], [j.w.shape[0] for j in jobs], [j.w.shape[1] * j.w.shape[2] for j in jobs],
+            [j.w.shape[3] for j in jobs], begin, src, base, rstride)
+        table = torch.frombuffer(bytearray(image), dtype=torch.uint8).to(jobs[0].w.device)
+        return table, blocks, keys
+
+    def request(self, kind, w, numel, src, base, rstride):
+        capturing = torch.cuda.is_current_stream_capturing()
+        if self.epoch != _state.BACKWARD_EPOCH[0]:
+            self.begin(_state.BACKWARD_EPOCH[0], capturing)
+        key = (w.data_ptr(), tuple(w.shape), w.dtype, kind)
+        job = self.jobs.get(key)
+        if job is not None:
+            job.seen = self.serial
+            if key in self.fresh:
+                if self.stream[0] != _stream():
+                    torch.cuda.current_stream().wait_stream(self.stream[1])
+                return job.out
+            if not capturing:
+                return _taps_t(w, job.out, src, base, rstride)
+        out = _taps_t(w, torch.empty(numel, dtype=w.dtype, device=w.device), src, base, rstride)
+        if job is None and not capturing:
+            self.jobs[key] = _RelayoutJob(w, out, list(src), list(base), list(rstride), self.serial)
+        return out
+
+
+_RELAYOUT = {}
+_RELAYOUT_PINNED = []
+_RELAYOUT_SUSPEND = [0]
+
+
+def _relayout(kind, w, numel, src, base, rstride):
+    if _state.BACKWARD_DEPTH[0] <= 0 or _RELAYOUT_SUSPEND[0] or not hasattr(_K.lib(), 'weight_taps_t_multi'):
+        return _taps_t(w, torch.empty(numel, dtype=w.dtype, device=w.device), src, base, rstride)
+    plan = _RELAYOUT.get(w.device.index)
+    if plan is None:
+        plan = _RELAYOUT[w.device.index] = _RelayoutPlan()
+    return plan.request(kind, w, numel, src, base, rstride)
+
+
 def _dgrad_weight(w):
     K, R, S, C = w.shape
     if not (w.is_cuda and w.is_contiguous() and w.element_size() in (2, 4) and _K.available()):
         return w.flip(1, 2).permute(3, 1, 2, 0).contiguous()
     T = R * S
-    out = torch.empty((C, R, S, K), dtype=w.dtype, device=w.device)
-    return _taps_t(w, out, [T - 1 - t for t in range(T)], [t * K for t in range(T)], [T * K] * T)
+    return _relayout('dgrad', w, C * T * K, [T - 1 - t for t in range(T)], [t * K for t in range(T)],
+                     [T * K] * T).view(C, R, S, K)
 
 
 def transpose2d(w):
@@ -905,8 +997,8 @@
     if len(empty) > 3:
         raise ValueError('conv_dgrad_strided: at most 3 phases without taps')
     slots, total = gidx
-    wsub = _taps_t(w.contiguous(), torch.empty(total, dtype=w.dtype, device=w.device), [t[0] for t in slots],
-                   [t[1] for t in slots], [t[2] for t in slots])
+    wsub = _relayout(('phases', tuple(stride), tuple(pad)), w.contiguous(), total, [t[0] for t in slots],
+                     [t[1] for t in slots], [t[2] for t in slots])
     cols = list(zip(*phases))
     lib = _K.lib()
     bkw = _glds_bnb(bn_bwd, dx, len(phases) * lib.conv_glds_bwd_nparts(N * Ho * Wo, bco)) if bn_bwd else {}
@@ -960,6 +1052,14 @@
 
 
 def _time_candidates(cands, reps=3, key=None, tol=2e-2):
+    _RELAYOUT_SUSPEND[0] += 1
+    try:
+        return _time_candidates_impl(cands, reps, key, tol)
+    finally:
+        _RELAYOUT_SUSPEND[0] -= 1
+
+
+def _time_candidates_impl(cands, reps, key, tol):
     ref = None
     ref_name = next((n for n, _ in cands if n in ('mm', 'miopen')), None)
     if ref_name is not None:
diff --git a/src/kernels/bindings.cc b/src/kernels/bindings.cc
--- a/src/kernels/bindings.cc
+++ b/src/kernels/bindings.cc
@@ -15,6 +15,9 @@
                      float* shift, int64_t R, int C, float eps, int training, int relu, int fix_gamma,
                      float momentum, float* mm_upd, float* mv_upd, int ext_nblk, hipStream_t s, const float* ascale,
                      const float* ashift);
+void bn_nhwc_forward_dual(int dtype, const void* x, const void* z, void* y, uint8_t* mask, float* const* xs,
+                          int x_ext_nblk, float* const* zs, int z_ext_nblk, int64_t R, int C, float eps,
+                          int fix_gamma, float momentum, hipStream_t s);
 void bn_nhwc_backward(int dtype, const void* x, const void* dy, const void* y, const uint8_t* mask, void* dx,
                       void* dz,
                       const float* gamma, const float* mean, const float* invstd, const float* fscale,
@@ -187,6 +190,11 @@
 int conv_pw_stream_slices(int kin, int nout);
 void weight_taps_t(int elem_bytes, const void* w, void* out, int K, int RS, int C, int n, const int* src,
                    const int64_t* base, const int64_t* rstride, hipStream_t s);
+int weight_taps_t_multi_table(int njobs, const int* elem_bytes, const uintptr_t* w, const uintptr_t* out,
+                              const int64_t* out_elems, const int* K, const int* RS, const int* C,
+                              const int* tap_begin, const int* src, const int64_t* base, const int64_t* rstride,
+                              std::vector<unsigned char>* image);
+void weight_taps_t_multi(const void* table, int total_blocks, hipStream_t s);
 void conv_pw_stream(int dtype, const void* x, const void* w, void* y, const void* zero, int M, int kin, int nout,
                     float* part, int grid, hipStream_t s, const void* addend, int wt, const void* bn_z,
                     const uint8_t* bn_mask, const float* bn_mean, const float* bn_scale, const float* bn_shift,
@@ -287,6 +295,29 @@
                   rstride.data(), S(s));
     check_launch("weight_taps_t");
   });
+  m.def("weight_taps_t_multi_table", [](std::vector<int> eb, std::vector<uintptr_t> w, std::vector<uintptr_t> out,
+                                        std::vector<int64_t> out_elems, std::vector<int> K, std::vector<int> RS,
+                                        std::vector<int> C, std::vector<int> tap_begin, std::vector<int> src,
+                                        std::vector<int64_t> base, std::vector<int64_t> rstride) {
+    const size_t n = eb.size();
+    if (n == 0 || w.size() != n || out.size() != n || out_elems.size() != n || K.size() != n || RS.size() != n ||
+        C.size() != n || tap_begin.size() != n + 1 || tap_begin[0] != 0)
+      throw std::runtime_error("weight_taps_t_multi_table: job list sizes");
+    for (size_t i = 0; i < n; ++i)
+      if (tap_begin[i + 1] < tap_begin[i]) throw std::runtime_error("weight_taps_t_multi_table: tap ranges");
+    const size_t nt = static_cast<size_t>(tap_begin[n]);
+    if (src.size() != nt || base.size() != nt || rstride.size() != nt)
+      throw std::runtime_error("weight_taps_t_multi_table: tap list sizes");
+    std::vector<unsigned char> image;
+    const int blocks = weight_taps_t_multi_table(static_cast<int>(n), eb.data(), w.data(), out.data(),
+                                                 out_elems.data(), K.data(), RS.data(), C.data(), tap_begin.data(),
+                                                 src.data(), base.data(), rstride.data(), &image);
+    return py::make_tuple(py::bytes(reinterpret_cast<const char*>(image.data()), image.size()), blocks);
+  });
+  m.def("weight_taps_t_multi", [](uintptr_t table, int total_blocks, uintptr_t s) {
+    weight_taps_t_multi(P<const void>(table), total_blocks, S(s));
+    check_launch("weight_taps_t_multi");
+  });
   m.def("conv_pw_stream_ok", &conv_pw_stream_ok);
   m.def("conv_pw_stream_slices", &conv_pw_stream_slices);
   m.def("conv_pw_stream_grid", [](int M, int kin, int nout, int ncu, int add) {
@@ -431,6 +462,21 @@
      py::arg("shift"), py::arg("R"), py::arg("C"), py::arg("eps"), py::arg("training"), py::arg("relu"),
      py::arg("fix_gamma"), py::arg("momentum"), py::arg("mm_upd"), py::arg("mv_upd"), py::arg("ext_nblk"),
      py::arg("stream"), py::arg("ascale") = 0, py::arg("ashift") = 0);
+  m.def("bn_nhwc_forward_dual", [](int dt, uintptr_t x, uintptr_t z, uintptr_t y, uintptr_t mask,
+                                   std::vector<uintptr_t> xs, int x_ext_nblk, std::vector<uintptr_t> zs,
+                                   int z_ext_nblk, int64_t R, int C, float eps, int fix_gamma, float momentum,
+                                   uintptr_t s) {
+    if (xs.size() != 11 || zs.size() != 11) throw std::runtime_error("bn_nhwc_forward_dual: 11 buffers per BatchNorm");
+    float* xp[11];
+    float* zp[11];
+    for (int i = 0; i < 11; ++i) {
+      xp[i] = P<float>(xs[i]);
+      zp[i] = P<float>(zs[i]);
+    }
+    bn_nhwc_forward_dual(dt, P<void>(x), P<void>(z), P<void>(y), P<uint8_t>(mask), xp, x_ext_nblk, zp, z_ext_nblk, R, C,
+                         eps, fix_gamma, momentum, S(s));
+    check_launch("bn_nhwc_forward_dual");
+  });
   m.def("bn_nhwc_backward", [](int dt, uintptr_t x, uintptr_t dy, uintptr_t y, uintptr_t mask, uintptr_t dx,
                                uintptr_t dz,
                                uintptr_t g, uintptr_t mean, uintptr_t inv, uintptr_t fscale, uintptr_t fshift,
diff --git a/src/kernels/bn_nhwc.hip b/src/kernels/bn_nhwc.hip
--- a/src/kernels/bn_nhwc.hip
+++ b/src/kernels/bn_nhwc.hip
@@ -126,16 +126,10 @@
 constexpr int kFinThreads = 256;
 constexpr int kFinPerBlock = kFinThreads / 64;
 template <int MODE>
-__global__ void __launch_bounds__(kFinThreads) bn_finalize_kernel(
-    const float* __restrict__ part1, const float* __restrict__ part2, int nblk, int C, int64_t R,
-    const float* __restrict__ center, const float* __restrict__ gamma, const float* __restrict__ beta,
-    const float* __restrict__ invstd_in, float eps, float* __restrict__ o0, float* __restrict__ o1,
-    float* __restrict__ o2, float* __restrict__ o3, float* __restrict__ o4, float* __restrict__ o5,
-    int fix_gamma, int training, float momentum, float* __restrict__ mm_upd, float* __restrict__ mv_upd,
-    int accum) {
-  const int lane = threadIdx.x & 63;
-  const int c = blockIdx.x * kFinPerBlock + (threadIdx.x >> 6);
-  if (c >= C) return;
+__device__ __forceinline__ void bn_finalize_channel(
+    int c, int lane, const float* part1, const float* part2, int nblk, int64_t R, const float* center,
+    const float* gamma, const float* beta, const float* invstd_in, float eps, float* o0, float* o1, float* o2,
+    float* o3, float* o4, int fix_gamma, int training, float momentum, float* mm_upd, float* mv_upd, int accum) {
   const float* p1 = part1 + static_cast<int64_t>(c) * nblk;
   const float* p2 = part2 + static_cast<int64_t>(c) * nblk;
   double a = 0.0, b = 0.0;
@@ -192,6 +186,49 @@
   }
 }
 
+template <int MODE>
+__global__ void __launch_bounds__(kFinThreads) bn_finalize_kernel(
+    const float* __restrict__ part1, const float* __restrict__ part2, int nblk, int C, int64_t R,
+    const float* __restrict__ center, const float* __restrict__ gamma, const float* __restrict__ beta,
+    const float* __restrict__ invstd_in, float eps, float* __restrict__ o0, float* __restrict__ o1,
+    float* __restrict__ o2, float* __restrict__ o3, float* __restrict__ o4, float* __restrict__ o5,
+    int fix_gamma, int training, float momentum, float* __restrict__ mm_upd, float* __restrict__ mv_upd,
+    int accum) {
+  const int lane = threadIdx.x & 63;
+  const int c = blockIdx.x * kFinPerBlock + (threadIdx.x >> 6);
+  if (c >= C) return;
+  bn_finalize_channel<MODE>(c, lane, part1, part2, nblk, R, center, gamma, beta, invstd_in, eps, o0, o1, o2, o3, o4,
+                            fix_gamma, training, momentum, mm_upd, mv_upd, accum);
+}
+
+struct BnFinFwd {
+  const float* part1;
+  const float* part2;
+  const float* center;
+  const float* gamma;
+  const float* beta;
+  float* mean;
+  float* invstd;
+  float* var;
+  float* scale;
+  float* shift;
+  float* mm_upd;
+  float* mv_upd;
+  int64_t R;
+  int nblk, C, fix_gamma;
+  float eps, momentum;
+};
+
+__global__ void __launch_bounds__(kFinThreads) bn_finalize_pair_kernel(BnFinFwd a, BnFinFwd b, int blocks_a) {
+  const bool first = static_cast<int>(blockIdx.x) < blocks_a;
+  const BnFinFwd f = first ? a : b;
+  const int lane = threadIdx.x & 63;
+  const int c = (static_cast<int>(blockIdx.x) - (first ? 0 : blocks_a)) * kFinPerBlock + (threadIdx.x >> 6);
+  if (c >= f.C) return;
+  bn_finalize_channel<0>(c, lane, f.part1, f.part2, f.nblk, f.R, f.center, f.gamma, f.beta, nullptr, f.eps, f.mean,
+                         f.invstd, f.var, f.scale, f.shift, f.fix_gamma, 1, f.momentum, f.mm_upd, f.mv_upd, 0);
+}
+
 typedef unsigned int bn_u32x4 __attribute__((ext_vector_type(4)));
 
 template <typename T>
@@ -480,6 +517,18 @@
 }
 
 template <typename T>
+static int bn_forward_reduce(const void* x, const float* center, float* part, int64_t R, int C, const BnGeom& g,
+                             hipStream_t s) {
+  int nblk;
+  int64_t rpb = bn_rows_per_block(R, C, g, &nblk);
+  dim3 grid(nblk, C / g.cb);
+  float* p2r = part + static_cast<int64_t>(nblk) * C;
+  hipLaunchKernelGGL((bn_reduce_kernel<T, 0, kReluNone>), grid, dim3(kBnThreads), 0, s, static_cast<const T*>(x),
+                     nullptr, nullptr, nullptr, center, nullptr, nullptr, part, p2r, R, C, g.tpr, g.rpi, rpb);
+  return nblk;
+}
+
+template <typename T>
 static void bn_forward_impl(const void* x, const void* addend, void* y, uint8_t* mask, const float* gamma,
                             const float* beta, const float* center, float* part, float* mean, float* invstd,
                             float* var, float* scale, float* shift, int64_t R, int C, float eps, int training,
@@ -494,12 +543,7 @@
     if (ext_nblk > 0) {
       nblk = ext_nblk;
     } else {
-      int64_t rpb = bn_rows_per_block(R, C, g, &nblk);
-      dim3 grid(nblk, C / g.cb);
-      float* p2r = part + static_cast<int64_t>(nblk) * C;
-      hipLaunchKernelGGL((bn_reduce_kernel<T, 0, kReluNone>), grid, dim3(kBnThreads), 0, s,
-                         static_cast<const T*>(x), nullptr, nullptr, nullptr, center, nullptr, nullptr, p1, p2r, R, C,
-                         g.tpr, g.rpi, rpb);
+      nblk = bn_forward_reduce<T>(x, center, part, R, C, g, s);
     }
     float* p2 = part + static_cast<int64_t>(nblk) * C;
     hipLaunchKernelGGL((bn_finalize_kernel<0>), dim3((C + kFinPerBlock - 1) / kFinPerBlock), dim3(kFinThreads), 0, s, p1, p2, nblk, C, R, center, gamma,
@@ -752,6 +796,48 @@
   }
 }
 
+template <typename T>
+static void bn_forward_dual_impl(const void* x, const void* z, void* y, uint8_t* mask, float* const* xs, int x_ext_nblk,
+                                 float* const* zs, int z_ext_nblk, int64_t R, int C, float eps, int fix_gamma,
+                                 float momentum, hipStream_t s) {
+  MXAMD_HOST_CHECK(C % 8 == 0, "bn_nhwc: channels must be a multiple of 8");
+  BnGeom g = bn_geom(C);
+  MXAMD_HOST_CHECK(C % g.cb == 0, "bn_nhwc: unsupported channel count");
+  BnFinFwd f[2];
+  const void* src[2] = {x, z};
+  float* const* set[2] = {xs, zs};
+  const int ext[2] = {x_ext_nblk, z_ext_nblk};
+  for (int i = 1; i >= 0; --i) {
+    float* const* a = set[i];
+    const int nblk = ext[i] > 0 ? ext[i] : bn_forward_reduce<T>(src[i], a[2], a[3], R, C, g, s);
+    f[i] = BnFinFwd{a[3], a[3] + static_cast<int64_t>(nblk) * C, a[2], a[0], a[1], a[4], a[5], a[6], a[7], a[8],
+                    a[9], a[10], R, nblk, C, fix_gamma, eps, momentum};
+  }
+  const int blocks = (C + kFinPerBlock - 1) / kFinPerBlock;
+  hipLaunchKernelGGL(bn_finalize_pair_kernel, dim3(2 * blocks), dim3(kFinThreads), 0, s, f[1], f[0], blocks);
+  bn_forward_impl<T>(x, z, y, mask, xs[0], xs[1], xs[2], xs[3], xs[4], xs[5], xs[6], xs[7], xs[8], R, C, eps, 0, 1,
+                     fix_gamma, momentum, nullptr, nullptr, 0, s, zs[7], zs[8]);
+}
+
+void bn_nhwc_forward_dual(int dtype, const void* x, const void* z, void* y, uint8_t* mask, float* const* xs,
+                          int x_ext_nblk, float* const* zs, int z_ext_nblk, int64_t R, int C, float eps,
+                          int fix_gamma, float momentum, hipStream_t s) {
+  MXAMD_HOST_CHECK(x && z && y && mask, "bn_nhwc_forward_dual: x, z, y and the mask are required");
+  for (int i = 0; i < 9; ++i)
+    MXAMD_HOST_CHECK(xs[i] && zs[i], "bn_nhwc_forward_dual: null statistics buffer");
+  switch (dtype) {
+    case kF16:
+      bn_forward_dual_impl<__half>(x, z, y, mask, xs, x_ext_nblk, zs, z_ext_nblk, R, C, eps, fix_gamma, momentum, s);
+      break;
+    case kBF16:
+      bn_forward_dual_impl<__hip_bfloat16>(x, z, y, mask, xs, x_ext_nblk, zs, z_ext_nblk, R, C, eps, fix_gamma,
+                                           momentum, s);
+      break;
+    default:
+      bn_forward_dual_impl<float>(x, z, y, mask, xs, x_ext_nblk, zs, z_ext_nblk, R, C, eps, fix_gamma, momentum, s);
+  }
+}
+
 void bn_finalize_backward(const float* part, int nblk, int C, int64_t R, const float* mean, const float* gamma,
                           const float* invstd, float* dgamma, float* dbeta, float* coef, int fix_gamma, int training,
                           int accum, hipStream_t s) {
diff --git a/src/kernels/pointwise.hip b/src/kernels/pointwise.hip
--- a/src/kernels/pointwise.hip
+++ b/src/kernels/pointwise.hip
@@ -1,4 +1,5 @@
 #include <stdexcept>
+#include <vector>
 
 #include "common.h"
 
@@ -195,19 +196,14 @@
 };
 
 template <typename E>
-__global__ void __launch_bounds__(256) weight_taps_t_kernel(const E* __restrict__ w, E* __restrict__ out, int K, int RS,
-                                                            int C, TapTable tt) {
-  __shared__ E tile[64][65];
-  const int z = blockIdx.z;
-  const int k0 = blockIdx.y * 64, c0 = blockIdx.x * 64;
-  const int src = tt.src[z];
+__device__ __forceinline__ void taps_t_tile(E (*tile)[65], const E* __restrict__ w, E* __restrict__ out, int K, int RS,
+                                            int C, int src, int64_t base, int64_t rs, int k0, int c0) {
   for (int i = threadIdx.x; i < 64 * 64; i += 256) {
     const int kk = i >> 6, cc = i & 63;
     const int k = k0 + kk, c = c0 + cc;
     if (k < K && c < C) tile[kk][cc] = w[(static_cast<int64_t>(k) * RS + src) * C + c];
   }
   __syncthreads();
-  const int64_t base = tt.base[z], rs = tt.rstride[z];
   for (int i = threadIdx.x; i < 64 * 64; i += 256) {
     const int cc = i >> 6, kk = i & 63;
     const int k = k0 + kk, c = c0 + cc;
@@ -215,13 +211,9 @@
   }
 }
 
-__global__ void __launch_bounds__(256) weight_taps_t_vec_kernel(const uint16_t* __restrict__ w,
-                                                                uint16_t* __restrict__ out, int K, int RS, int C,
-                                                                TapTable tt) {
-  __shared__ __attribute__((aligned(16))) uint16_t tile[64][72];
-  const int z = blockIdx.z;
-  const int k0 = blockIdx.y * 64, c0 = blockIdx.x * 64;
-  const int src = tt.src[z];
+__device__ __forceinline__ void taps_t_tile_vec(uint16_t (*tile)[72], const uint16_t* __restrict__ w,
+                                                uint16_t* __restrict__ out, int K, int RS, int C, int src,
+                                                int64_t base, int64_t rs, int k0, int c0) {
   const int tid = threadIdx.x;
   uint4 r[2];
 #pragma unroll
@@ -237,7 +229,6 @@
     *reinterpret_cast<uint4*>(&tile[v >> 3][(v & 7) * 8]) = r[i];
   }
   __syncthreads();
-  const int64_t base = tt.base[z], rs = tt.rstride[z];
 #pragma unroll
   for (int i = 0; i < 2; ++i) {
     const int v = tid + i * 256;
@@ -251,6 +242,81 @@
       *reinterpret_cast<uint4*>(out + base + static_cast<int64_t>(c) * rs + k) = uint4{q[0], q[1], q[2], q[3]};
     }
   }
+}
+
+template <typename E>
+__global__ void __launch_bounds__(256) weight_taps_t_kernel(const E* __restrict__ w, E* __restrict__ out, int K, int RS,
+                                                            int C, TapTable tt) {
+  __shared__ E tile[64][65];
+  const int z = blockIdx.z;
+  taps_t_tile<E>(tile, w, out, K, RS, C, tt.src[z], tt.base[z], tt.rstride[z], blockIdx.y * 64, blockIdx.x * 64);
+}
+
+__global__ void __launch_bounds__(256) weight_taps_t_vec_kernel(const uint16_t* __restrict__ w,
+                                                                uint16_t* __restrict__ out, int K, int RS, int C,
+                                                                TapTable tt) {
+  __shared__ __attribute__((aligned(16))) uint16_t tile[64][72];
+  const int z = blockIdx.z;
+  taps_t_tile_vec(tile, w, out, K, RS, C, tt.src[z], tt.base[z], tt.rstride[z], blockIdx.y * 64, blockIdx.x * 64);
+}
+
+enum { kTapsVec16 = 0, kTapsScalar16 = 1, kTapsScalar32 = 2 };
+struct TapsJob {
+  const void* w;
+  void* out;
+  int K, RS, C;
+  int path;
+  int tap0, ntaps;
+  int block0;
+  int tiles_c, tiles_k;
+  int pad_;
+};
+struct TapsEntry {
+  int64_t base, rstride;
+  int src, pad_;
+};
+struct TapsHeader {
+  int njobs, ntaps, total_blocks, pad_;
+};
+static_assert(sizeof(TapsJob) == 56 && sizeof(TapsEntry) == 24 && sizeof(TapsHeader) == 16, "taps table layout");
+
+__global__ void __launch_bounds__(256) weight_taps_t_multi_kernel(const unsigned char* __restrict__ table) {
+  __shared__ __attribute__((aligned(16))) uint32_t smem[64 * 65];
+  const TapsHeader* hd = reinterpret_cast<const TapsHeader*>(table);
+  const TapsJob* jobs = reinterpret_cast<const TapsJob*>(table + sizeof(TapsHeader));
+  const int njobs = hd->njobs;
+  const int blk = static_cast<int>(blockIdx.x);
+  if (blk >= hd->total_blocks) return;
+  int lo = 0, hi = njobs - 1;
+  while (lo < hi) {
+    const int mid = (lo + hi + 1) >> 1;
+    if (jobs[mid].block0 <= blk) lo = mid; else hi = mid - 1;
+  }
+  const TapsJob j = jobs[lo];
+  const int local = blk - j.block0;
+  const int ct = local % j.tiles_c;
+  const int kt = (local / j.tiles_c) % j.tiles_k;
+  const int z = local / (j.tiles_c * j.tiles_k);
+  if (z >= j.ntaps) return;
+  const TapsEntry* taps = reinterpret_cast<const TapsEntry*>(table + sizeof(TapsHeader) + sizeof(TapsJob) * njobs);
+  const TapsEntry t = taps[j.tap0 + z];
+  if (j.path == kTapsVec16)
+    taps_t_tile_vec(reinterpret_cast<uint16_t(*)[72]>(smem), static_cast<const uint16_t*>(j.w),
+                    static_cast<uint16_t*>(j.out), j.K, j.RS, j.C, t.src, t.base, t.rstride, kt * 64, ct * 64);
+  else if (j.path == kTapsScalar16)
+    taps_t_tile<uint16_t>(reinterpret_cast<uint16_t(*)[65]>(smem), static_cast<const uint16_t*>(j.w),
+                          static_cast<uint16_t*>(j.out), j.K, j.RS, j.C, t.src, t.base, t.rstride, kt * 64, ct * 64);
+  else
+    taps_t_tile<uint32_t>(reinterpret_cast<uint32_t(*)[65]>(smem), static_cast<const uint32_t*>(j.w),
+                          static_cast<uint32_t*>(j.out), j.K, j.RS, j.C, t.src, t.base, t.rstride, kt * 64, ct * 64);
+}
+
+bool taps_vec_ok(int elem_bytes, const void* w, const void* out, int K, int C, int n, const int64_t* base,
+                 const int64_t* rstride) {
+  bool vec = elem_bytes == 2 && K % 8 == 0 && C % 8 == 0 && reinterpret_cast<uintptr_t>(w) % 16 == 0 &&
+             reinterpret_cast<uintptr_t>(out) % 16 == 0;
+  for (int z = 0; z < n && vec; ++z) vec = base[z] % 8 == 0 && rstride[z] % 8 == 0;
+  return vec;
 }
 
 }
@@ -266,9 +332,7 @@
     tt.rstride[z] = rstride[z];
   }
   const dim3 grid((C + 63) / 64, (K + 63) / 64, n);
-  bool vec = elem_bytes == 2 && K % 8 == 0 && C % 8 == 0 && reinterpret_cast<uintptr_t>(w) % 16 == 0 &&
-             reinterpret_cast<uintptr_t>(out) % 16 == 0;
-  for (int z = 0; z < n && vec; ++z) vec = base[z] % 8 == 0 && rstride[z] % 8 == 0;
+  const bool vec = taps_vec_ok(elem_bytes, w, out, K, C, n, base, rstride);
   if (vec)
     hipLaunchKernelGGL(weight_taps_t_vec_kernel, grid, dim3(256), 0, s, static_cast<const uint16_t*>(w),
                        static_cast<uint16_t*>(out), K, RS, C, tt);
@@ -280,6 +344,60 @@
                        static_cast<uint32_t*>(out), K, RS, C, tt);
   else
     throw std::runtime_error("weight_taps_t: 2- or 4-byte elements");
+}
+
+int weight_taps_t_multi_table(int njobs, const int* elem_bytes, const uintptr_t* w, const uintptr_t* out,
+                              const int64_t* out_elems, const int* K, const int* RS, const int* C,
+                              const int* tap_begin, const int* src, const int64_t* base, const int64_t* rstride,
+                              std::vector<unsigned char>* image) {
+  MXAMD_HOST_CHECK(njobs >= 1, "weight_taps_t_multi: no jobs");
+  const int ntaps = tap_begin[njobs];
+  image->assign(sizeof(TapsHeader) + sizeof(TapsJob) * njobs + sizeof(TapsEntry) * ntaps, 0);
+  TapsHeader* hd = reinterpret_cast<TapsHeader*>(image->data());
+  TapsJob* jobs = reinterpret_cast<TapsJob*>(image->data() + sizeof(TapsHeader));
+  TapsEntry* taps = reinterpret_cast<TapsEntry*>(image->data() + sizeof(TapsHeader) + sizeof(TapsJob) * njobs);
+  int64_t blocks = 0;
+  for (int i = 0; i < njobs; ++i) {
+    const int t0 = tap_begin[i], n = tap_begin[i + 1] - t0;
+    MXAMD_HOST_CHECK(n >= 1 && K[i] >= 1 && RS[i] >= 1 && C[i] >= 1, "weight_taps_t_multi: empty job");
+    MXAMD_HOST_CHECK(elem_bytes[i] == 2 || elem_bytes[i] == 4, "weight_taps_t_multi: 2- or 4-byte elements");
+    MXAMD_HOST_CHECK(w[i] != 0 && out[i] != 0, "weight_taps_t_multi: null tensor");
+    for (int z = t0; z < t0 + n; ++z) {
+      MXAMD_HOST_CHECK(src[z] >= 0 && src[z] < RS[i], "weight_taps_t_multi: tap index out of range");
+      MXAMD_HOST_CHECK(base[z] >= 0 && rstride[z] >= 0 &&
+                           base[z] + static_cast<int64_t>(C[i] - 1) * rstride[z] + K[i] <= out_elems[i],
+                       "weight_taps_t_multi: a tap slot writes past its output");
+      taps[z].src = src[z];
+      taps[z].base = base[z];
+      taps[z].rstride = rstride[z];
+    }
+    TapsJob& j = jobs[i];
+    j.w = reinterpret_cast<const void*>(w[i]);
+    j.out = reinterpret_cast<void*>(out[i]);
+    j.K = K[i];
+    j.RS = RS[i];
+    j.C = C[i];
+    j.path = taps_vec_ok(elem_bytes[i], j.w, j.out, K[i], C[i], n, base + t0, rstride + t0)
+                 ? kTapsVec16
+                 : (elem_bytes[i] == 2 ? kTapsScalar16 : kTapsScalar32);
+    j.tap0 = t0;
+    j.ntaps = n;
+    j.tiles_c = (C[i] + 63) / 64;
+    j.tiles_k = (K[i] + 63) / 64;
+    j.block0 = static_cast<int>(blocks);
+    blocks += static_cast<int64_t>(j.tiles_c) * j.tiles_k * n;
+    MXAMD_HOST_CHECK(blocks < (int64_t{1} << 31), "weight_taps_t_multi: too many blocks");
+  }
+  hd->njobs = njobs;
+  hd->ntaps = ntaps;
+  hd->total_blocks = static_cast<int>(blocks);
+  return static_cast<int>(blocks);
+}
+
+void weight_taps_t_multi(const void* table, int total_blocks, hipStream_t s) {
+  MXAMD_HOST_CHECK(table != nullptr && total_blocks >= 1, "weight_taps_t_multi: empty table");
+  hipLaunchKernelGGL(weight_taps_t_multi_kernel, dim3(total_blocks), dim3(256), 0, s,
+                     static_cast<const unsigned char*>(table));
 }
 
 void relu_forward(int dtype, const void* x, void* y, int64_t n, hipStream_t s) {
```

Result: no change. 12640 images/sec, median of 4 (-0.0%).
